# anibali/dsnt-pose2d

Hardware: AMD Instinct MI355X
Metric: images/sec (train step, 256x256, 16 joints) (higher is better)
Workload: dtype f32; 1 GPU; hg2 + DSNT + JS reg, 256x256 -> 64x64x16, batch 32 per GPU, RMSprop lr 2.5e-4, train step fwd+loss+bwd+optim; global_batch=32, parallelism=dp1, launches_fwd=210

## Files before the change

### dsnt-pose2d_amd/csrc/api.cpp

```cpp
#include "common.h"
#include <string.h>

static thread_local char g_err[512] = "";

int dsnt_set_error(int code, const char* fmt, ...) {
    va_list ap;
    va_start(ap, fmt);
    vsnprintf(g_err, sizeof(g_err), fmt, ap);
    va_end(ap);
    return code;
}

int dsnt_device_id(void) {
    int d = 0;
    if (hipGetDevice(&d) != hipSuccess || d < 0) d = 0;
    return d < DSNT_MAX_DEVICES ? d : DSNT_MAX_DEVICES - 1;
}

int dsnt_device_cus(void) {
    static std::atomic<int> cus[DSNT_MAX_DEVICES];
    const int d = dsnt_device_id();
    int c = cus[d].load(std::memory_order_acquire);
    if (!c) {
        hipDeviceProp_t prop;
        int dev = 0;
        c = (hipGetDevice(&dev) == hipSuccess && hipGetDeviceProperties(&prop, dev) == hipSuccess && prop.multiProcessorCount > 0)
                ? prop.multiProcessorCount : 256;
        cus[d].store(c, std::memory_order_release);
    }
    return c;
}

extern "C" int dsnt_version(void) { return 132; }
extern "C" const char* dsnt_last_error(void) { return g_err; }

#include <vector>
#include <new>

struct dsnt_list {
    struct Entry {
        int kind;
        int lane, src, dst;
        mutable hipEvent_t ev;
        std::function<void(hipStream_t)> fn;
    };
    std::vector<Entry> entries;
    std::vector<size_t> seg_start;
    dsnt_list() { seg_start.push_back(0); }
};

static thread_local dsnt_list* g_rec = nullptr;

dsnt_list* dsnt_recording(void) { return g_rec; }

void dsnt_record_launch(dsnt_list* l, int lane, std::function<void(hipStream_t)>&& fn) {
    dsnt_list::Entry e;
    e.kind = 0; e.lane = lane; e.src = e.dst = 0; e.ev = nullptr; e.fn = std::move(fn);
    l->entries.push_back(std::move(e));
}

extern "C" dsnt_list* dsnt_list_create(void) { return new (std::nothrow) dsnt_list(); }

extern "C" void dsnt_list_destroy(dsnt_list* l) {
    if (!l) return;
    if (g_rec == l) g_rec = nullptr;
    for (auto& e : l->entries)
        if (e.ev) (void)hipEventDestroy(e.ev);
    delete l;
}

extern "C" int dsnt_list_begin(dsnt_list* l) {
    DSNT_REQUIRE(l && !g_rec, DSNT_ERR_ARG, "dsnt_list_begin: null list, or this thread is already recording");
    g_rec = l;
    return DSNT_OK;
}

extern "C" int dsnt_list_end(void) {
    DSNT_REQUIRE(g_rec, DSNT_ERR_ARG, "dsnt_list_end: this thread is not recording");
    g_rec = nullptr;
    return DSNT_OK;
}

extern "C" int dsnt_list_sync(dsnt_list* l, int src_lane, int dst_lane) {
    DSNT_REQUIRE(l && src_lane >= 0 && dst_lane >= 0 && src_lane < DSNT_MAX_LANES && dst_lane < DSNT_MAX_LANES, DSNT_ERR_ARG,
                 "dsnt_list_sync: bad argument");
    dsnt_list::Entry e;
    e.kind = 1; e.lane = 0; e.src = src_lane; e.dst = dst_lane; e.ev = nullptr;
    l->entries.push_back(std::move(e));
    return DSNT_OK;
}

extern "C" int dsnt_list_mark(dsnt_list* l) {
    DSNT_REQUIRE(l, DSNT_ERR_ARG, "dsnt_list_mark: null list");
    l->seg_start.push_back(l->entries.size());
    return (int)l->seg_start.size() - 1;
}

extern "C" int dsnt_list_segments(const dsnt_list* l) { return l ? (int)l->seg_start.size() : 0; }
extern "C" int dsnt_list_size(const dsnt_list* l) { return l ? (int)l->entries.size() : 0; }

extern "C" int dsnt_list_replay(const dsnt_list* l, int segment, void* const* streams, int nstreams) {
    DSNT_REQUIRE(l && streams && nstreams > 0 && nstreams <= DSNT_MAX_LANES, DSNT_ERR_ARG, "dsnt_list_replay: bad argument");
    DSNT_REQUIRE(!g_rec, DSNT_ERR_ARG, "dsnt_list_replay: this thread is recording");
    const int nseg = (int)l->seg_start.size();
    DSNT_REQUIRE(segment >= -1 && segment < nseg, DSNT_ERR_ARG, "dsnt_list_replay: segment %d of %d", segment, nseg);
    const size_t a = segment < 0 ? 0 : l->seg_start[segment];
    const size_t b = (segment < 0 || segment + 1 == nseg) ? l->entries.size() : l->seg_start[segment + 1];
    for (size_t i = a; i < b; ++i) {
        const dsnt_list::Entry& e = l->entries[i];
        if (e.kind == 0) {
            DSNT_REQUIRE(e.lane >= 0 && e.lane < nstreams, DSNT_ERR_ARG, "dsnt_list_replay: entry %zu wants lane %d of %d", i, e.lane, nstreams);
            e.fn((hipStream_t)streams[e.lane]);
        } else {
            DSNT_REQUIRE(e.src < nstreams && e.dst < nstreams, DSNT_ERR_ARG, "dsnt_list_replay: lane out of range");
            if (!e.ev && hipEventCreateWithFlags(&e.ev, hipEventDisableTiming) != hipSuccess)
                return dsnt_set_error(DSNT_ERR_HIP, "dsnt_list_replay: hipEventCreate");
            if (hipEventRecord(e.ev, (hipStream_t)streams[e.src]) != hipSuccess ||
                hipStreamWaitEvent((hipStream_t)streams[e.dst], e.ev, 0) != hipSuccess)
                return dsnt_set_error(DSNT_ERR_HIP, "dsnt_list_replay: event record / wait failed");
        }
    }
    hipError_t e_ = hipGetLastError();
    if (e_ != hipSuccess) return dsnt_set_error(DSNT_ERR_HIP, "dsnt_list_replay: %s", hipGetErrorString(e_));
    return DSNT_OK;
}
```

### dsnt-pose2d_amd/csrc/bn.hip

```cpp
#include "common.h"
#include <string.h>
#include "bn_pro.h"
#include "ew_bodies.h"

template <int MODE>
__global__ __launch_bounds__(256) void tile_reduce_kernel(
    const float* __restrict__ a, const float* __restrict__ x, const float* __restrict__ scale,
    const float* __restrict__ shift, const float* __restrict__ mean,
    const float* __restrict__ invstd, int relu, float* __restrict__ partial, long M, int C, int cgs,
    const float* __restrict__ ymask = nullptr, float* __restrict__ dz_out = nullptr) {
    __shared__ float red[256 * 8];
    const int tid = threadIdx.x;
    const int C4 = C >> 2;
    const int rpar = 256 / cgs;
    const int cg_l = tid % cgs, rl = tid / cgs;
    const bool active = rl < rpar;
    const long row0 = (long)blockIdx.x * TILE_ROWS;
    const long row1 = row0 + TILE_ROWS < M ? row0 + TILE_ROWS : M;
    for (int cg0 = blockIdx.y * cgs; cg0 < C4; cg0 += cgs * gridDim.y) {
        const int cg = cg0 + cg_l;
        float4 s1 = make_float4(0.f, 0.f, 0.f, 0.f), s2 = s1;
        if (active && cg < C4) {
            float4 sc, sh, mu, is;
            if (MODE == 1) {
                sc = reinterpret_cast<const float4*>(scale)[cg];
                sh = reinterpret_cast<const float4*>(shift)[cg];
            }
            if (MODE >= 1) {
                mu = reinterpret_cast<const float4*>(mean)[cg];
                is = reinterpret_cast<const float4*>(invstd)[cg];
            }
            for (long r = row0 + rl; r < row1; r += rpar) {
                const float4 v = reinterpret_cast<const float4*>(a + r * C)[cg];
                if (MODE == 0) {
                    s1.x += v.x; s1.y += v.y; s1.z += v.z; s1.w += v.w;
                    s2.x = fmaf(v.x, v.x, s2.x); s2.y = fmaf(v.y, v.y, s2.y);
                    s2.z = fmaf(v.z, v.z, s2.z); s2.w = fmaf(v.w, v.w, s2.w);
                } else {
                    const float4 xv = reinterpret_cast<const float4*>(x + r * C)[cg];
                    float4 dz = v;
                    if (MODE == 2) {
                        if (relu) {
                            const float4 yv = reinterpret_cast<const float4*>(ymask + r * C)[cg];
                            if (yv.x <= 0.f) dz.x = 0.f;
                            if (yv.y <= 0.f) dz.y = 0.f;
                            if (yv.z <= 0.f) dz.z = 0.f;
                            if (yv.w <= 0.f) dz.w = 0.f;
                        }
                        reinterpret_cast<float4*>(dz_out + r * C)[cg] = dz;
                    } else if (relu) {
                        if (fmaf(xv.x, sc.x, sh.x) <= 0.f) dz.x = 0.f;
                        if (fmaf(xv.y, sc.y, sh.y) <= 0.f) dz.y = 0.f;
                        if (fmaf(xv.z, sc.z, sh.z) <= 0.f) dz.z = 0.f;
                        if (fmaf(xv.w, sc.w, sh.w) <= 0.f) dz.w = 0.f;
                    }
                    s1.x += dz.x; s1.y += dz.y; s1.z += dz.z; s1.w += dz.w;
                    s2.x = fmaf(dz.x, (xv.x - mu.x) * is.x, s2.x);
                    s2.y = fmaf(dz.y, (xv.y - mu.y) * is.y, s2.y);
                    s2.z = fmaf(dz.z, (xv.z - mu.z) * is.z, s2.z);
                    s2.w = fmaf(dz.w, (xv.w - mu.w) * is.w, s2.w);
                }
            }
        }
        __syncthreads();
        float* mine = red + tid * 8;
        mine[0] = s1.x; mine[1] = s1.y; mine[2] = s1.z; mine[3] = s1.w;
        mine[4] = s2.x; mine[5] = s2.y; mine[6] = s2.z; mine[7] = s2.w;
        __syncthreads();
        if (tid < cgs && cg0 + tid < C4) {
            float acc[8] = {0, 0, 0, 0, 0, 0, 0, 0};
            for (int j = 0; j < rpar; ++j)
#pragma unroll
                for (int e = 0; e < 8; ++e) acc[e] += red[(j * cgs + tid) * 8 + e];
            float* p0 = partial + ((size_t)blockIdx.x * 2 + 0) * C + (size_t)(cg0 + tid) * 4;
            float* p1 = partial + ((size_t)blockIdx.x * 2 + 1) * C + (size_t)(cg0 + tid) * 4;
            *reinterpret_cast<float4*>(p0) = make_float4(acc[0], acc[1], acc[2], acc[3]);
            *reinterpret_cast<float4*>(p1) = make_float4(acc[4], acc[5], acc[6], acc[7]);
        }
    }
}

extern "C" int dsnt_bn_stats(const float* x, float* partial, int64_t M, int C, void* stream) {
    DSNT_REQUIRE(x && partial && M > 0 && C > 0, DSNT_ERR_ARG, "dsnt_bn_stats: bad argument");
    DSNT_REQUIRE(C % 4 == 0 && dsnt_aligned16(x) && dsnt_aligned16(partial), DSNT_ERR_ALIGN,
                 "dsnt_bn_stats: C %% 4 and 16-byte alignment required");
    const int tiles = (int)((M + TILE_ROWS - 1) / TILE_ROWS);
    DSNT_LAUNCH(tile_reduce_kernel<0>, dim3(tiles, tile_grid_y(tiles, C / 4)), dim3(256), 0, (hipStream_t)stream, x,
                       nullptr, nullptr, nullptr, nullptr, nullptr, 0, partial, (long)M, C, tile_cgs(tiles, C / 4));
    DSNT_CHECK_LAUNCH("dsnt_bn_stats");
}

extern "C" int dsnt_bn_act_fwd_stats(const float* x, const float* scale, const float* shift, int relu, float* y,
                                     float* partial, int64_t M, int C, const dsnt_out_bounds* g_tail, void* stream) {
    OutBoundsP tail;
    if (int e = out_bounds_fill(tail, g_tail, "dsnt_bn_act_fwd_stats")) return e;
    DSNT_REQUIRE(x && scale && shift && y && M > 0 && C > 0, DSNT_ERR_ARG, "dsnt_bn_act_fwd_stats: bad argument");
    DSNT_REQUIRE(C % 4 == 0 && dsnt_aligned16(x) && dsnt_aligned16(y) && dsnt_aligned16(scale) && dsnt_aligned16(shift) &&
                 dsnt_aligned16(partial), DSNT_ERR_ALIGN, "dsnt_bn_act_fwd_stats: alignment");
    const long tiles = ((long)M + TILE_ROWS - 1) / TILE_ROWS;
    DSNT_REQUIRE(M < (1ll << 31), DSNT_ERR_SHAPE, "dsnt_bn_act_fwd_stats: M too large");
    const TileOpP q{x, nullptr, y, nullptr, partial, 1, 1, (int)M, C, tile_cgs(tiles, C / 4), tail, scale, shift, relu};
    DSNT_LAUNCH(tile_op_stats_kernel<2>, dim3((unsigned)tiles, tile_grid_y(tiles, C / 4)), dim3(256), 0, stream, q);
    DSNT_CHECK_LAUNCH("dsnt_bn_act_fwd_stats");
}

extern "C" int dsnt_bn_act_bwd_reduce(const float* da, const float* x, const float* scale,
                                      const float* shift, const float* mean, const float* invstd,
                                      int relu, float* partial, int64_t M, int C, void* stream) {
    DSNT_REQUIRE(da && x && scale && shift && mean && invstd && partial && M > 0 && C > 0,
                 DSNT_ERR_ARG, "dsnt_bn_act_bwd_reduce: bad argument");
    DSNT_REQUIRE(C % 4 == 0 && dsnt_aligned16(x) && dsnt_aligned16(da) && dsnt_aligned16(partial) &&
                 dsnt_aligned16(scale) && dsnt_aligned16(shift) && dsnt_aligned16(mean) &&
                 dsnt_aligned16(invstd), DSNT_ERR_ALIGN,
                 "dsnt_bn_act_bwd_reduce: C %% 4 and 16-byte alignment required");
    const int tiles = (int)((M + TILE_ROWS - 1) / TILE_ROWS);
    DSNT_LAUNCH(tile_reduce_kernel<1>, dim3(tiles, tile_grid_y(tiles, C / 4)), dim3(256), 0, (hipStream_t)stream, da, x,
                       scale, shift, mean, invstd, relu, partial, (long)M, C, tile_cgs(tiles, C / 4));
    DSNT_CHECK_LAUNCH("dsnt_bn_act_bwd_reduce");
}

extern "C" int dsnt_bn_add_act_bwd_reduce(const float* da, const float* y, const float* x, const float* mean, const float* invstd,
                                          int relu, float* dz, float* partial, int64_t M, int C, void* stream) {
    DSNT_REQUIRE(da && y && x && mean && invstd && dz && partial && M > 0 && C > 0, DSNT_ERR_ARG, "dsnt_bn_add_act_bwd_reduce: bad argument");
    DSNT_REQUIRE(C % 4 == 0 && dsnt_aligned16(x) && dsnt_aligned16(da) && dsnt_aligned16(y) && dsnt_aligned16(dz) && dsnt_aligned16(partial) &&
                 dsnt_aligned16(mean) && dsnt_aligned16(invstd), DSNT_ERR_ALIGN, "dsnt_bn_add_act_bwd_reduce: C %% 4 and 16-byte alignment required");
    const int tiles = (int)((M + TILE_ROWS - 1) / TILE_ROWS);
    DSNT_LAUNCH(tile_reduce_kernel<2>, dim3(tiles, tile_grid_y(tiles, C / 4)), dim3(256), 0, (hipStream_t)stream, da, x,
                       nullptr, nullptr, mean, invstd, relu, partial, (long)M, C, tile_cgs(tiles, C / 4), y, dz);
    DSNT_CHECK_LAUNCH("dsnt_bn_add_act_bwd_reduce");
}

#define FIN_T 1024
#define FIN_P (FIN_T / 16)
struct BnBoundP { const float* scale; const float* dz_amax; float sqrtM; unsigned* out; };
struct BnFinP {
    const float* partial; int ntiles; double invM, unbias; int C;
    const float* gamma; const float* beta; float* running_mean; float* running_var;
    float momentum, eps; int training; float* o0; float* o1; float* o2; float* o3; int accumulate; BnBoundP bp;
};
template <int MODE>
__global__ __launch_bounds__(FIN_T) void bn_finalize_kernel(BnFinP q) {
    __shared__ double r0[256], r1[256];
    const float* __restrict__ partial = q.partial; const int ntiles = q.ntiles; const double invM = q.invM, unbias = q.unbias;
    const int C = q.C; const float* __restrict__ gamma = q.gamma; const float* __restrict__ beta = q.beta;
    float* running_mean = q.running_mean; float* running_var = q.running_var; const float momentum = q.momentum, eps = q.eps;
    const int training = q.training; float* o0 = q.o0; float* o1 = q.o1; float* o2 = q.o2; float* o3 = q.o3;
    const int accumulate = q.accumulate; const BnBoundP bp = q.bp;
    const int tid = threadIdx.x, cl = tid & 15;
    const int wg = blockIdx.x;
    const int c = wg * 16 + cl;
    const bool lead = tid < 16 && c < C;
    float pg = 1.f, pb = 0.f, prm = 0.f, prv = 0.f, po0 = 0.f, po1 = 0.f, psc = 0.f, pdz = 0.f;
    if (MODE == 0 && lead) {
        if (gamma) pg = gamma[c];
        if (beta) pb = beta[c];
        if (running_mean) { prm = running_mean[c]; prv = running_var[c]; }
    }
    if (MODE == 1) {
        if (lead && accumulate) { if (o0) po0 = o0[c]; if (o1) po1 = o1[c]; }
        if (bp.out) { pdz = bp.dz_amax[tid & 63]; if (lead) psc = bp.scale[c]; }
    }
    constexpr int VP = 1;
    double a0[VP], a1[VP];
#pragma unroll
    for (int v = 0; v < VP; ++v) {
        a0[v] = 0.0; a1[v] = 0.0;
        const int part = (tid + v * FIN_T) >> 4;
        if (c < C && (MODE == 1 || training)) {
#pragma unroll 4
            for (int t = part; t < ntiles; t += FIN_P) {
                a0[v] += (double)partial[((size_t)t * 2 + 0) * C + c];
                a1[v] += (double)partial[((size_t)t * 2 + 1) * C + c];
            }
        }
    }
#pragma unroll
    for (int v = 0; v < VP; ++v) {
        a0[v] += __shfl_xor(a0[v], 16, 64); a1[v] += __shfl_xor(a1[v], 16, 64);
        a0[v] += __shfl_xor(a0[v], 32, 64); a1[v] += __shfl_xor(a1[v], 32, 64);
        if ((tid & 63) < 16) { r0[((tid + v * FIN_T) >> 6) * 16 + cl] = a0[v]; r1[((tid + v * FIN_T) >> 6) * 16 + cl] = a1[v]; }
    }
    __syncthreads();
    double s0 = 0.0, s1 = 0.0;
    if (tid < 16) {
#pragma unroll
        for (int w = 0; w < FIN_T / 64; ++w) { s0 += r0[w * 16 + cl]; s1 += r1[w * 16 + cl]; }
    }
    if (tid < 16 && c < C) {
        if (MODE == 0) {
            double mean, var;
            if (training) {
                mean = s0 * invM;
                var = s1 * invM - mean * mean;
                if (var < 0.0) var = 0.0;
                if (running_mean) {
                    running_mean[c] = (float)((1.0 - momentum) * prm + momentum * mean);
                    running_var[c] = (float)((1.0 - momentum) * prv + momentum * var * unbias);
                }
            } else {
                mean = prm;
                var = prv;
            }
            const float is = (float)(1.0 / sqrt(var + (double)eps));
            const float mu = (float)mean;
            const float sc = gamma ? pg * is : is;
            o0[c] = mu; o1[c] = is; o2[c] = sc;
            o3[c] = (beta ? pb : 0.f) - mu * sc;
        } else {
            const float sdz = (float)s0, sdzx = (float)s1;
            if (o0) o0[c] = accumulate ? po0 + sdzx : sdzx;
            if (o1) o1[c] = accumulate ? po1 + sdz : sdz;
            o2[c] = (float)(s0 * invM);
            o2[C + c] = (float)(s1 * invM);
        }
    }
    if (MODE == 1 && bp.out) {
        float dzmax = pdz;
#pragma unroll
        for (int o = 32; o > 0; o >>= 1) dzmax = fmaxf(dzmax, __shfl_xor(dzmax, o, 64));
        float b = 0.f;
        if (tid < 16 && c < C)
            b = fabsf(psc) * (dzmax + fabsf((float)(s0 * invM)) + fabsf((float)(s1 * invM)) * bp.sqrtM);
#pragma unroll
        for (int o = 8; o > 0; o >>= 1) b = fmaxf(b, __shfl_xor(b, o, 64));
        if (tid == 0 && b > 0.f) atomicMax(bp.out + (wg & 63), __float_as_uint(b));
    }
}

extern "C" int dsnt_bn_finalize(const float* partial, int ntiles, int64_t M, int C,
                                const float* gamma, const float* beta, float* running_mean,
                                float* running_var, float momentum, float eps, int training,
                                float* mean, float* invstd, float* scale, float* shift,
                                void* stream) {
    DSNT_REQUIRE(mean && invstd && scale && shift && C > 0 && M > 0, DSNT_ERR_ARG,
                 "dsnt_bn_finalize: bad argument");
    DSNT_REQUIRE(training ? (partial != nullptr && ntiles > 0) : (running_mean && running_var),
                 DSNT_ERR_ARG, "dsnt_bn_finalize: missing statistics source");
    DSNT_REQUIRE((running_mean == nullptr) == (running_var == nullptr), DSNT_ERR_ARG,
                 "dsnt_bn_finalize: running_mean/var must be given together");
    const double unbias = M > 1 ? (double)M / (double)(M - 1) : 1.0;
    const BnFinP q{partial, ntiles, 1.0 / (double)M, unbias, C, gamma, beta, running_mean, running_var, momentum, eps, training,
                   mean, invstd, scale, shift, 0, BnBoundP{nullptr, nullptr, 0.f, nullptr}};
    DSNT_LAUNCH(bn_finalize_kernel<0>, dim3((C + 15) / 16), dim3(FIN_T), 0, stream, q);
    DSNT_CHECK_LAUNCH("dsnt_bn_finalize");
}

__global__ __launch_bounds__(256) void bn_eval_prep_kernel(const long long* __restrict__ table) {
    const long long* t = table + (size_t)blockIdx.x * 10;
    const float* gamma = reinterpret_cast<const float*>(t[0]);
    const float* beta = reinterpret_cast<const float*>(t[1]);
    const float* rm = reinterpret_cast<const float*>(t[2]);
    const float* rv = reinterpret_cast<const float*>(t[3]);
    float* mean = reinterpret_cast<float*>(t[4]);
    float* invstd = reinterpret_cast<float*>(t[5]);
    float* scale = reinterpret_cast<float*>(t[6]);
    float* shift = reinterpret_cast<float*>(t[7]);
    const int C = (int)t[8];
    const float eps = __uint_as_float((unsigned)t[9]);
    for (int c = threadIdx.x; c < C; c += 256) {
        const double var = rv[c];
        const float is = (float)(1.0 / sqrt(var + (double)eps));
        const float mu = rm[c];
        const float sc = gamma ? gamma[c] * is : is;
        mean[c] = mu; invstd[c] = is; scale[c] = sc;
        shift[c] = (beta ? beta[c] : 0.f) - mu * sc;
    }
}

extern "C" int dsnt_bn_eval_prep(const int64_t* table, int rows, void* stream) {
    DSNT_REQUIRE(table && rows > 0, DSNT_ERR_ARG, "dsnt_bn_eval_prep: bad argument");
    DSNT_LAUNCH(bn_eval_prep_kernel, dim3(rows), dim3(256), 0, (hipStream_t)stream, (const long long*)table);
    DSNT_CHECK_LAUNCH("dsnt_bn_eval_prep");
}

extern "C" int dsnt_bn_bwd_finalize(const float* partial, int ntiles, int64_t M, int C,
                                    float* dgamma, float* dbeta, int accumulate, float* coef,
                                    void* stream) {
    DSNT_REQUIRE(partial && coef && ntiles > 0 && C > 0 && M > 0, DSNT_ERR_ARG,
                 "dsnt_bn_bwd_finalize: bad argument");
    const double invM = (accumulate & DSNT_BN_FROZEN) ? 0.0 : 1.0 / (double)M;
    const BnFinP q{partial, ntiles, invM, 1.0, C, nullptr, nullptr, nullptr, nullptr, 0.f, 0.f, 1, dgamma, dbeta, coef, nullptr,
                   accumulate & 1, BnBoundP{nullptr, nullptr, 0.f, nullptr}};
    DSNT_LAUNCH(bn_finalize_kernel<1>, dim3((C + 15) / 16), dim3(FIN_T), 0, stream, q);
    DSNT_CHECK_LAUNCH("dsnt_bn_bwd_finalize");
}

extern "C" int dsnt_bn_bwd_finalize_bound(const float* partial, int ntiles, int64_t M, int C, float* dgamma, float* dbeta,
                                          int accumulate, float* coef, const float* scale, const float* dz_amax,
                                          float* bound_out, void* stream) {
    DSNT_REQUIRE(partial && coef && scale && dz_amax && bound_out && ntiles > 0 && C > 0 && M > 0, DSNT_ERR_ARG,
                 "dsnt_bn_bwd_finalize_bound: bad argument");
    DSNT_REQUIRE(!(accumulate & DSNT_BN_FROZEN), DSNT_ERR_ARG, "dsnt_bn_bwd_finalize_bound: DSNT_BN_FROZEN has no bound form");
    const BnFinP q{partial, ntiles, 1.0 / (double)M, 1.0, C, nullptr, nullptr, nullptr, nullptr, 0.f, 0.f, 1, dgamma, dbeta, coef, nullptr,
                   accumulate & 1, BnBoundP{scale, dz_amax, sqrtf((float)M), reinterpret_cast<unsigned*>(bound_out)}};
    DSNT_LAUNCH(bn_finalize_kernel<1>, dim3((C + 15) / 16), dim3(FIN_T), 0, stream, q);
    DSNT_CHECK_LAUNCH("dsnt_bn_bwd_finalize_bound");
}

__global__ void bn_act_fwd_kernel(const float4* __restrict__ x, const float4* __restrict__ scale,
                                  const float4* __restrict__ shift, int relu, float4* __restrict__ y,
                                  long n4, int C4) {
    for (long i = (long)blockIdx.x * blockDim.x + threadIdx.x; i < n4;
         i += (long)gridDim.x * blockDim.x) {
        const int cg = (int)(i % C4);
        const float4 v = x[i], sc = scale[cg], sh = shift[cg];
        float4 o = make_float4(fmaf(v.x, sc.x, sh.x), fmaf(v.y, sc.y, sh.y), fmaf(v.z, sc.z, sh.z),
                               fmaf(v.w, sc.w, sh.w));
        if (relu) { o.x = fmaxf(o.x, 0.f); o.y = fmaxf(o.y, 0.f); o.z = fmaxf(o.z, 0.f); o.w = fmaxf(o.w, 0.f); }
        y[i] = o;
    }
}

extern "C" int dsnt_bn_act_fwd(const float* x, const float* scale, const float* shift, int relu,
                               float* y, int64_t M, int C, void* stream) {
    DSNT_REQUIRE(x && scale && shift && y && M > 0 && C > 0, DSNT_ERR_ARG, "dsnt_bn_act_fwd: bad argument");
    DSNT_REQUIRE(C % 4 == 0 && dsnt_aligned16(x) && dsnt_aligned16(y) && dsnt_aligned16(scale) &&
                 dsnt_aligned16(shift), DSNT_ERR_ALIGN, "dsnt_bn_act_fwd: alignment");
    const long n4 = (long)M * C / 4;
    DSNT_LAUNCH(bn_act_fwd_kernel, dim3(flat_grid(n4, 256)), dim3(256), 0, (hipStream_t)stream,
                       (const float4*)x, (const float4*)scale, (const float4*)shift, relu, (float4*)y,
                       n4, C / 4);
    DSNT_CHECK_LAUNCH("dsnt_bn_act_fwd");
}

__global__ void bn_add_act_fwd_kernel(const float4* __restrict__ x, const float4* __restrict__ scale,
                                      const float4* __restrict__ shift, const float4* __restrict__ res, int relu,
                                      float4* __restrict__ y, long n4, int C4) {
    for (long i = (long)blockIdx.x * blockDim.x + threadIdx.x; i < n4; i += (long)gridDim.x * blockDim.x) {
        const int cg = (int)(i % C4);
        const float4 v = x[i], sc = scale[cg], sh = shift[cg], r = res[i];
        float4 o = make_float4(fmaf(v.x, sc.x, sh.x) + r.x, fmaf(v.y, sc.y, sh.y) + r.y, fmaf(v.z, sc.z, sh.z) + r.z,
                               fmaf(v.w, sc.w, sh.w) + r.w);
        if (relu) { o.x = fmaxf(o.x, 0.f); o.y = fmaxf(o.y, 0.f); o.z = fmaxf(o.z, 0.f); o.w = fmaxf(o.w, 0.f); }
        y[i] = o;
    }
}

extern "C" int dsnt_bn_add_act_fwd(const float* x, const float* scale, const float* shift, const float* res,
                                   int relu, float* y, int64_t M, int C, void* stream) {
    DSNT_REQUIRE(x && scale && shift && res && y && M > 0 && C > 0, DSNT_ERR_ARG, "dsnt_bn_add_act_fwd: bad argument");
    DSNT_REQUIRE(C % 4 == 0 && dsnt_aligned16(x) && dsnt_aligned16(y) && dsnt_aligned16(res) && dsnt_aligned16(scale) &&
                 dsnt_aligned16(shift), DSNT_ERR_ALIGN, "dsnt_bn_add_act_fwd: alignment");
    const long n4 = (long)M * C / 4;
    DSNT_LAUNCH(bn_add_act_fwd_kernel, dim3(flat_grid(n4, 256)), dim3(256), 0, (hipStream_t)stream,
                       (const float4*)x, (const float4*)scale, (const float4*)shift, (const float4*)res, relu,
                       (float4*)y, n4, C / 4);
    DSNT_CHECK_LAUNCH("dsnt_bn_add_act_fwd");
}

__global__ void relu_bwd_kernel(const float4* __restrict__ dy, const float4* __restrict__ y, float4* __restrict__ dz,
                                long n4) {
    for (long i = (long)blockIdx.x * blockDim.x + threadIdx.x; i < n4; i += (long)gridDim.x * blockDim.x) {
        const float4 g = dy[i], v = y[i];
        dz[i] = make_float4(v.x > 0.f ? g.x : 0.f, v.y > 0.f ? g.y : 0.f, v.z > 0.f ? g.z : 0.f, v.w > 0.f ? g.w : 0.f);
    }
}

extern "C" int dsnt_relu_bwd(const float* dy, const float* y, float* dz, int64_t n, void* stream) {
    DSNT_REQUIRE(dy && y && dz && n > 0 && n % 4 == 0, DSNT_ERR_ARG, "dsnt_relu_bwd: bad argument");
    DSNT_REQUIRE(dsnt_aligned16(dy) && dsnt_aligned16(y) && dsnt_aligned16(dz), DSNT_ERR_ALIGN, "dsnt_relu_bwd: alignment");
    DSNT_LAUNCH(relu_bwd_kernel, dim3(flat_grid(n / 4, 256)), dim3(256), 0, (hipStream_t)stream,
                       (const float4*)dy, (const float4*)y, (float4*)dz, (long)(n / 4));
    DSNT_CHECK_LAUNCH("dsnt_relu_bwd");
}

struct BnApplyVec { float4 sc, sh, mu, is, c0, c1; };
__device__ __forceinline__ float4 bn_apply_one(const float4 g, const float4 xv, const BnApplyVec& v, int relu) {
    float4 dz = g;
    if (relu) {
        if (fmaf(xv.x, v.sc.x, v.sh.x) <= 0.f) dz.x = 0.f;
        if (fmaf(xv.y, v.sc.y, v.sh.y) <= 0.f) dz.y = 0.f;
        if (fmaf(xv.z, v.sc.z, v.sh.z) <= 0.f) dz.z = 0.f;
        if (fmaf(xv.w, v.sc.w, v.sh.w) <= 0.f) dz.w = 0.f;
    }
    float4 o;
    o.x = v.sc.x * (dz.x - v.c0.x - (xv.x - v.mu.x) * v.is.x * v.c1.x);
    o.y = v.sc.y * (dz.y - v.c0.y - (xv.y - v.mu.y) * v.is.y * v.c1.y);
    o.z = v.sc.z * (dz.z - v.c0.z - (xv.z - v.mu.z) * v.is.z * v.c1.z);
    o.w = v.sc.w * (dz.w - v.c0.w - (xv.w - v.mu.w) * v.is.w * v.c1.w);
    return o;
}
struct BnApplyP {
    const float4* da; const float4* x; const float4* scale; const float4* shift; const float4* mean; const float4* invstd;
    const float4* coef; int relu; float4* dx; const float4* base; long n4; int C4; unsigned* amax; BnBwdProP pro;
};
template <bool FIXED>
__global__ void bn_act_bwd_apply_kernel(BnApplyP q) {
    __shared__ double pro_sh[512];
    const float4* __restrict__ da = q.da; const float4* __restrict__ x = q.x; const float4* __restrict__ scale = q.scale;
    const float4* __restrict__ shift = q.shift; const float4* __restrict__ mean = q.mean; const float4* __restrict__ invstd = q.invstd;
    const float4* coef = q.coef; const int relu = q.relu; float4* dx = q.dx; const float4* base = q.base;
    const long n4 = q.n4; const int C4 = q.C4; unsigned* __restrict__ amax = q.amax; const BnBwdProP pro = q.pro;
    const bool accumulate = base != nullptr;
    const int wg = blockIdx.x, nwg = gridDim.x;
    if (pro.partial) {
        bn_pro_backward<256>(pro, pro_sh, wg == 0);
        __syncthreads();
    }
    float am = 0.f;
    const long stride = (long)nwg * 256;
    long i = threadIdx.x < 256 ? (long)wg * 256 + threadIdx.x : n4;
    auto vec = [&](int cg) {
        BnApplyVec v;
        v.sc = scale[cg]; v.sh = shift[cg]; v.mu = mean[cg]; v.is = invstd[cg]; v.c0 = coef[cg]; v.c1 = coef[C4 + cg];
        return v;
    };
    auto amx = [&](const float4 o) { am = fmaxf(fmaxf(fmaxf(fabsf(o.x), fabsf(o.y)), fmaxf(fabsf(o.z), fabsf(o.w))), am); };
    if (FIXED) {
        const BnApplyVec v = vec((int)((i < n4 ? i : 0) % C4));
        for (; i + stride < n4; i += 2 * stride) {
            const float4 g0 = da[i], x0 = x[i], g1 = da[i + stride], x1 = x[i + stride];
            float4 p0 = make_float4(0.f, 0.f, 0.f, 0.f), p1 = p0;
            if (accumulate) { p0 = base[i]; p1 = base[i + stride]; }
            float4 o0 = bn_apply_one(g0, x0, v, relu), o1 = bn_apply_one(g1, x1, v, relu);
            if (accumulate) {
                o0.x += p0.x; o0.y += p0.y; o0.z += p0.z; o0.w += p0.w;
                o1.x += p1.x; o1.y += p1.y; o1.z += p1.z; o1.w += p1.w;
            }
            dx[i] = o0; dx[i + stride] = o1;
            amx(o0); amx(o1);
        }
        if (i < n4) {
            float4 o = bn_apply_one(da[i], x[i], v, relu);
            if (accumulate) { const float4 p = base[i]; o.x += p.x; o.y += p.y; o.z += p.z; o.w += p.w; }
            dx[i] = o;
            amx(o);
        }
    } else {
        for (; i < n4; i += stride) {
            float4 o = bn_apply_one(da[i], x[i], vec((int)(i % C4)), relu);
            if (accumulate) { const float4 p = base[i]; o.x += p.x; o.y += p.y; o.z += p.z; o.w += p.w; }
            dx[i] = o;
            amx(o);
        }
    }
    if (amax) amax_commit(am, amax);
}

static int bn_act_bwd_apply_impl(const float* da, const float* x, const float* scale, const float* shift,
                                 const float* mean, const float* invstd, const float* coef, int relu, float* dx,
                                 int accumulate, int64_t M, int C, float* amax, void* stream, const BnBwdProP* pro, const float* base) {
    DSNT_REQUIRE(da && x && scale && shift && mean && invstd && coef && dx && M > 0 && C > 0,
                 DSNT_ERR_ARG, "dsnt_bn_act_bwd_apply: bad argument");
    DSNT_REQUIRE(C % 4 == 0 && dsnt_aligned16(da) && dsnt_aligned16(x) && dsnt_aligned16(dx) &&
                 dsnt_aligned16(coef) && dsnt_aligned16(base), DSNT_ERR_ALIGN, "dsnt_bn_act_bwd_apply: alignment");
    if (!base && accumulate) base = dx;
    const long n4 = (long)M * C / 4;
    int grid = flat_grid(n4, 256);
    BnBwdProP q;
    memset(&q, 0, sizeof(q));
    if (pro) {
        q = *pro;
        if (grid > 128) grid = 128;
    }
    const BnApplyP ap{(const float4*)da, (const float4*)x, (const float4*)scale, (const float4*)shift, (const float4*)mean,
                      (const float4*)invstd, (const float4*)coef, relu, (float4*)dx, (const float4*)base, n4, C / 4, (unsigned*)amax, q};
    if (((long)grid * 256) % (C / 4) == 0)
        DSNT_LAUNCH(bn_act_bwd_apply_kernel<true>, dim3(grid), dim3(256), 0, stream, ap);
    else
        DSNT_LAUNCH(bn_act_bwd_apply_kernel<false>, dim3(grid), dim3(256), 0, stream, ap);
    DSNT_CHECK_LAUNCH("dsnt_bn_act_bwd_apply");
}

extern "C" int dsnt_bn_act_bwd_apply_amax(const float* da, const float* x, const float* scale,
                                          const float* shift, const float* mean, const float* invstd,
                                          const float* coef, int relu, float* dx, int accumulate,
                                          int64_t M, int C, float* amax, void* stream) {
    return bn_act_bwd_apply_impl(da, x, scale, shift, mean, invstd, coef, relu, dx, accumulate, M, C, amax, stream, nullptr, nullptr);
}

extern "C" int dsnt_bn_act_bwd_apply(const float* da, const float* x, const float* scale,
                                     const float* shift, const float* mean, const float* invstd,
                                     const float* coef, int relu, float* dx, int accumulate,
                                     int64_t M, int C, void* stream) {
    return bn_act_bwd_apply_impl(da, x, scale, shift, mean, invstd, coef, relu, dx, accumulate, M, C, nullptr, stream, nullptr, nullptr);
}

static int bn_bwd_pro_fill(BnBwdProP& q, const char* who, const float* partial, int ntiles, float* dgamma, float* dbeta,
                           int accumulate_params, float* coef, int64_t M, int C) {
    DSNT_REQUIRE(partial && ntiles > 0 && coef && C <= 256 && (long)ntiles * C <= 16384, DSNT_ERR_ARG,
                 "%s: needs partial sums of at most 256 channels / 128 KB and a coef buffer", who);
    q.partial = partial; q.tiles = ntiles; q.C = C; q.invM = 1.0 / (double)M;
    q.dgamma = dgamma; q.dbeta = dbeta; q.accumulate = accumulate_params; q.coef = coef;
    return DSNT_OK;
}

extern "C" int dsnt_bn_act_bwd_apply_pro(const float* da, const float* x, const float* scale, const float* shift,
                                         const float* mean, const float* invstd, const float* partial, int ntiles,
                                         float* dgamma, float* dbeta, int accumulate_params, float* coef, int relu,
                                         float* dx, int accumulate, int64_t M, int C, float* amax, void* stream) {
    BnBwdProP q;
    if (int e = bn_bwd_pro_fill(q, "dsnt_bn_act_bwd_apply_pro", partial, ntiles, dgamma, dbeta, accumulate_params, coef, M, C)) return e;
    return bn_act_bwd_apply_impl(da, x, scale, shift, mean, invstd, coef, relu, dx, accumulate, M, C, amax, stream, &q, nullptr);
}
extern "C" int dsnt_bn_act_bwd_apply_base(const float* da, const float* x, const float* scale, const float* shift,
                                          const float* mean, const float* invstd, const float* coef, int relu,
                                          const float* base, float* dx, int64_t M, int C, float* amax, void* stream) {
    DSNT_REQUIRE(base && base != dx, DSNT_ERR_ARG, "dsnt_bn_act_bwd_apply_base: `base` must be a second tensor");
    return bn_act_bwd_apply_impl(da, x, scale, shift, mean, invstd, coef, relu, dx, 1, M, C, amax, stream, nullptr, base);
}
extern "C" int dsnt_bn_act_bwd_apply_pro_base(const float* da, const float* x, const float* scale, const float* shift,
                                              const float* mean, const float* invstd, const float* partial, int ntiles,
                                              float* dgamma, float* dbeta, int accumulate_params, float* coef, int relu,
                                              const float* base, float* dx, int64_t M, int C, float* amax, void* stream) {
    DSNT_REQUIRE(base && base != dx, DSNT_ERR_ARG, "dsnt_bn_act_bwd_apply_pro_base: `base` must be a second tensor");
    BnBwdProP q;
    if (int e = bn_bwd_pro_fill(q, "dsnt_bn_act_bwd_apply_pro_base", partial, ntiles, dgamma, dbeta, accumulate_params, coef, M, C)) return e;
    return bn_act_bwd_apply_impl(da, x, scale, shift, mean, invstd, coef, relu, dx, 1, M, C, amax, stream, &q, base);
}
```

### dsnt-pose2d_amd/csrc/bn_pro.h

```cpp
#pragma once
#include "common.h"

struct OutBoundsP {
    unsigned* amax;
    unsigned* amax_bn;
    const float* amax_scale;
    const float* amax_shift;
    int amax_relu, pad_;
};

__device__ __forceinline__ void tail_store(float* p, float v) { *p = v; }

struct BnProP {
    const float* partial; int tiles, C;
    double invM, unbias;
    const float* gamma; const float* beta; float* rmean; float* rvar;
    float momentum, eps;
    float* mean; float* invstd; float* scale; float* shift;
};
struct BnBwdProP {
    const float* partial; int tiles, C;
    double invM;
    float* dgamma; float* dbeta; int accumulate;
    float* coef;
};

template <int NT>
__device__ __forceinline__ void bn_pro_sums(const float* __restrict__ partial, int tiles, int C, double* sh, double& a0, double& a1) {
    const int tid = threadIdx.x;
    const int ncol = 2 * C;
    a0 = 0.0; a1 = 0.0;
    for (int cb = 0; cb < ncol; cb += NT) {
        const int nc = ncol - cb < NT ? ncol - cb : NT;
        const int L = NT / nc;
        const int col = tid % nc, lane = tid / nc;
        double a = 0.0;
        if (lane < L) {
            const float* q = partial + cb + col;
            for (int r0 = lane; r0 < tiles; r0 += 16 * L) {
                float v[16];
#pragma unroll
                for (int u = 0; u < 16; ++u) {
                    const int r = r0 + u * L;
                    v[u] = r < tiles ? q[(size_t)r * ncol] : 0.f;
                }
#pragma unroll
                for (int u = 0; u < 16; ++u) a += (double)v[u];
            }
        }
        __syncthreads();
        sh[tid] = a;
        __syncthreads();
        for (int st = 0; st < 2; ++st) {
            const int c = st * C + tid - cb;
            if (tid < C && c >= 0 && c < nc) {
                double t = 0.0;
                for (int l = 0; l < L; ++l) t += sh[l * nc + c];
                if (st == 0) a0 = t; else a1 = t;
            }
        }
    }
}

template <int NT>
__device__ __forceinline__ void bn_pro_forward(const BnProP& q, double* sh, bool writer) {
    const int c = threadIdx.x;
    float pg = 1.f, pb = 0.f, prm = 0.f, prv = 0.f;
    if (c < q.C) {
        if (q.gamma) pg = q.gamma[c];
        if (q.beta) pb = q.beta[c];
        if (writer && q.rmean) { prm = q.rmean[c]; prv = q.rvar[c]; }
    }
    double a0, a1;
    bn_pro_sums<NT>(q.partial, q.tiles, q.C, sh, a0, a1);
    if (c < q.C) {
        const double mean = a0 * q.invM;
        double var = a1 * q.invM - mean * mean;
        if (var < 0.0) var = 0.0;
        if (writer && q.rmean) {
            q.rmean[c] = (float)((1.0 - q.momentum) * prm + q.momentum * mean);
            q.rvar[c] = (float)((1.0 - q.momentum) * prv + q.momentum * var * q.unbias);
        }
        const float is = (float)(1.0 / sqrt(var + (double)q.eps));
        const float mu = (float)mean;
        const float sc = q.gamma ? pg * is : is;
        q.mean[c] = mu; q.invstd[c] = is; q.scale[c] = sc;
        q.shift[c] = (q.beta ? pb : 0.f) - mu * sc;
    }
    __builtin_amdgcn_fence(__ATOMIC_RELEASE, "workgroup");
}
template <int NT>
__device__ __forceinline__ void bn_pro_backward(const BnBwdProP& q, double* sh, bool writer) {
    const int c = threadIdx.x;
    float pdg = 0.f, pdb = 0.f;
    if (c < q.C && writer && q.accumulate) { if (q.dgamma) pdg = q.dgamma[c]; if (q.dbeta) pdb = q.dbeta[c]; }
    double a0, a1;
    bn_pro_sums<NT>(q.partial, q.tiles, q.C, sh, a0, a1);
    if (c < q.C) {
        if (writer) {
            const float sdz = (float)a0, sdzx = (float)a1;
            if (q.dgamma) q.dgamma[c] = q.accumulate ? pdg + sdzx : sdzx;
            if (q.dbeta) q.dbeta[c] = q.accumulate ? pdb + sdz : sdz;
        }
        q.coef[c] = (float)(a0 * q.invM);
        q.coef[q.C + c] = (float)(a1 * q.invM);
    }
    __builtin_amdgcn_fence(__ATOMIC_RELEASE, "workgroup");
}

static inline int out_bounds_fill(OutBoundsP& out, const dsnt_out_bounds* in, const char* who) {
    static_assert(sizeof(OutBoundsP) == sizeof(dsnt_out_bounds), "dsnt_out_bounds layout");
    out.amax = in ? reinterpret_cast<unsigned*>(in->amax) : nullptr;
    out.amax_bn = in ? reinterpret_cast<unsigned*>(in->amax_bn) : nullptr;
    out.amax_scale = in ? in->amax_scale : nullptr; out.amax_shift = in ? in->amax_shift : nullptr;
    out.amax_relu = in ? in->amax_relu : 0; out.pad_ = 0;
    DSNT_REQUIRE(!out.amax_bn || (out.amax_scale && out.amax_shift && dsnt_aligned16(out.amax_scale) && dsnt_aligned16(out.amax_shift)),
                 DSNT_ERR_ARG, "%s: dsnt_out_bounds.amax_bn needs 16-byte aligned amax_scale / amax_shift", who);
    return DSNT_OK;
}
```

### dsnt-pose2d_amd/csrc/conv_f32.hip

```cpp
#include "conv_epilogue.h"
#include <string.h>
#include <stdlib.h>

#define BK 32
#define PITCH 36

template <int WM, int WN, int TM, int TN, bool PRO, bool FAST>
__global__ __launch_bounds__(512, 4) void conv_fwd_kernel(ConvP p) {
    constexpr int BM = WM * TM * 32, BN = WN * TN * 32;
    constexpr int APASS = BM / 32, BPASS = BN / 32;
    extern __shared__ __attribute__((aligned(16))) float smem[];
    float* As = smem;
    float* Bs = smem + 2 * BM * PITCH;

    int tile;
    xcd_remap(blockIdx.x, p.mtiles * p.ntiles, tile);
    const int ntile = tile % p.ntiles, mtile = tile / p.ntiles;

    const int tid = threadIdx.x, lane = tid & 63;
    const int wave = __builtin_amdgcn_readfirstlane(tid >> 6);
    const int nsteps = (p.K + BK - 1) / BK;
    const int lr = lane & 31, lh = lane >> 5;
    const int cw = wave & 3;
    const int wm = cw / WN, wn = cw % WN;
    if (PRO && p.pro.partial) {
        bn_pro_forward<512>(p.pro, reinterpret_cast<double*>(smem), blockIdx.x == 0);
        __syncthreads();
    }

    f32x16 acc[TM][TN];
#pragma unroll
    for (int a = 0; a < TM; ++a)
#pragma unroll
        for (int b = 0; b < TN; ++b)
#pragma unroll
            for (int e = 0; e < 16; ++e) acc[a][b][e] = 0.f;

    if (FAST && wave >= 4) {
        typedef unsigned u32x4 __attribute__((ext_vector_type(4)));
        const int ltid = tid - 256;
        const int lrow = ltid >> 3, kc = ltid & 7;
        const int HoWo = p.Ho * p.Wo;
        const int RS = p.R * p.S;
        unsigned apix[APASS];
        unsigned long long vmask = 0ull;
#pragma unroll
        for (int i = 0; i < APASS; ++i) {
            const int m = mtile * BM + lrow + 32 * i;
            const bool vm = m < p.M;
            const int mm = vm ? m : 0;
            const int n = mm / HoWo, rem = mm - n * HoWo;
            const int oh = rem / p.Wo, ow = rem - oh * p.Wo;
            const int ih0 = oh * p.stride - p.pad, iw0 = ow * p.stride - p.pad;
            apix[i] = (unsigned)(((n * p.H + ih0) * p.W + iw0) * p.Cin + kc * 4) * 4u;
            for (int t = 0; t < RS; ++t) {
                const int r = t / p.S, s_ = t - r * p.S;
                const int ih = ih0 + r * p.dil, iw = iw0 + s_ * p.dil;
                if (vm && ih >= 0 && ih < p.H && iw >= 0 && iw < p.W)
                    vmask |= 1ull << (t * APASS + i);
            }
        }
        unsigned bpix[BPASS];
#pragma unroll
        for (int j = 0; j < BPASS; ++j) {
            const int n = ntile * BN + lrow + 32 * j;
            bpix[j] = n < p.Cout ? (unsigned)(n * p.K + kc * 4) * 4u : 0xF0000000u;
        }
        const __amdgpu_buffer_rsrc_t xr = __builtin_amdgcn_make_buffer_rsrc(
            const_cast<float*>(p.x), 0, (int)((size_t)p.N * p.H * p.W * p.Cin * 4u), 0x00020000);
        const __amdgpu_buffer_rsrc_t wr = __builtin_amdgcn_make_buffer_rsrc(
            const_cast<float*>(p.w), 0, (int)((size_t)p.Cout * p.K * 4u), 0x00020000);
        struct Stage {
            u32x4 ra[APASS], rb[BPASS];
            float4 sc, sh;
            unsigned ok;
        };
        Stage S0, S1;
        auto gload = [&](Stage& st, int step) {
            const int kb = step * BK;
            const int tap = kb / p.Cin, cb = kb - tap * p.Cin;
            const int r = tap / p.S, s_ = tap - r * p.S;
            const unsigned toff = (unsigned)(((r * p.dil) * p.W + s_ * p.dil) * p.Cin + cb) * 4u;
            if (PRO) {
                st.sc = *reinterpret_cast<const float4*>(p.in_scale + cb + kc * 4);
                st.sh = *reinterpret_cast<const float4*>(p.in_shift + cb + kc * 4);
            }
            st.ok = (unsigned)(vmask >> (tap * APASS));
#pragma unroll
            for (int i = 0; i < APASS; ++i)
                st.ra[i] = __builtin_amdgcn_raw_buffer_load_b128(xr, apix[i] + toff, 0, 0);
            const unsigned koff = (unsigned)kb * 4u;
#pragma unroll
            for (int j = 0; j < BPASS; ++j)
                st.rb[j] = __builtin_amdgcn_raw_buffer_load_b128(wr, bpix[j] + koff, 0, 0);
        };
        auto lstore = [&](const Stage& st, int buf) {
#pragma unroll
            for (int i = 0; i < APASS; ++i) {
                float4 v = make_float4(__uint_as_float(st.ra[i].x), __uint_as_float(st.ra[i].y),
                                       __uint_as_float(st.ra[i].z), __uint_as_float(st.ra[i].w));
                float* dst = As + (buf * BM + lrow + 32 * i) * PITCH + kc * 4;
                if (PRO) {
                    v.x = fmaf(v.x, st.sc.x, st.sh.x); v.y = fmaf(v.y, st.sc.y, st.sh.y);
                    v.z = fmaf(v.z, st.sc.z, st.sh.z); v.w = fmaf(v.w, st.sc.w, st.sh.w);
                    if (p.in_relu) {
                        v.x = fmaxf(v.x, 0.f); v.y = fmaxf(v.y, 0.f);
                        v.z = fmaxf(v.z, 0.f); v.w = fmaxf(v.w, 0.f);
                    }
                }
                const bool ok = (st.ok >> i) & 1u;
                v.x = ok ? v.x : 0.f; v.y = ok ? v.y : 0.f; v.z = ok ? v.z : 0.f; v.w = ok ? v.w : 0.f;
                *reinterpret_cast<float4*>(dst) = v;
            }
#pragma unroll
            for (int j = 0; j < BPASS; ++j)
                *reinterpret_cast<u32x4*>(Bs + (buf * BN + lrow + 32 * j) * PITCH + kc * 4) = st.rb[j];
        };
        const int last = nsteps - 1;
        gload(S0, 0);
        gload(S1, min(1, last));
        lstore(S0, 0);
        gload(S0, min(2, last));
        __syncthreads();
        int s = 0;
        for (; s + 1 < nsteps; s += 2) {
            lstore(S1, 1);
            gload(S1, min(s + 3, last));
            __syncthreads();
            lstore(S0, 0);
            gload(S0, min(s + 4, last));
            __syncthreads();
        }
        if (s < nsteps) __syncthreads();
    } else if (wave >= 4) {
        const int ltid = tid - 256;
        const int lrow = ltid >> 3, kc = ltid & 7;
        int abase[APASS], aih0[APASS], aiw0[APASS];
        const int HoWo = p.Ho * p.Wo;
#pragma unroll
        for (int i = 0; i < APASS; ++i) {
            const int m = mtile * BM + lrow + 32 * i;
            if (m < p.M) {
                const int n = m / HoWo, rem = m - n * HoWo;
                const int oh = rem / p.Wo, ow = rem - oh * p.Wo;
                abase[i] = n * p.H * p.W * p.Cin;
                aih0[i] = oh * p.stride - p.pad;
                aiw0[i] = ow * p.stride - p.pad;
            } else {
                abase[i] = 0; aih0[i] = -(1 << 28); aiw0[i] = 0;
            }
        }
        int boff[BPASS];
        bool bok[BPASS];
#pragma unroll
        for (int j = 0; j < BPASS; ++j) {
            const int n = ntile * BN + lrow + 32 * j;
            bok[j] = n < p.Cout;
            boff[j] = bok[j] ? n * p.K : 0;
        }
        struct Stage {
            float4 ra[APASS], rb[BPASS];
            float4 sc, sh;
            unsigned okmask;
        };
        Stage S0, S1;
        auto gload = [&](Stage& st, int step) {
            const int k0 = step * BK + kc * 4;
            const bool vk = k0 < p.K;
            const int tap = k0 / p.Cin, c = k0 - tap * p.Cin;
            const int r = tap / p.S, s = tap - r * p.S;
            const int dh = r * p.dil, dw = s * p.dil;
            if (PRO) {
                const int cc = vk ? c : 0;
                st.sc = *reinterpret_cast<const float4*>(p.in_scale + cc);
                st.sh = *reinterpret_cast<const float4*>(p.in_shift + cc);
            }
            st.okmask = 0;
#pragma unroll
            for (int i = 0; i < APASS; ++i) {
                const int ih = aih0[i] + dh, iw = aiw0[i] + dw;
                const bool ok = vk && ih >= 0 && ih < p.H && iw >= 0 && iw < p.W;
                const int off = ok ? abase[i] + (ih * p.W + iw) * p.Cin + c : 0;
                st.ra[i] = *reinterpret_cast<const float4*>(p.x + off);
                st.okmask |= (ok ? 1u : 0u) << i;
            }
#pragma unroll
            for (int j = 0; j < BPASS; ++j) {
                const bool ok = vk && bok[j];
                st.rb[j] = *reinterpret_cast<const float4*>(p.w + (ok ? boff[j] + k0 : 0));
                st.okmask |= (ok ? 1u : 0u) << (8 + j);
            }
        };
        auto lstore = [&](const Stage& st, int buf) {
#pragma unroll
            for (int i = 0; i < APASS; ++i) {
                float4 v = st.ra[i];
                if (PRO) {
                    v.x = fmaf(v.x, st.sc.x, st.sh.x); v.y = fmaf(v.y, st.sc.y, st.sh.y);
                    v.z = fmaf(v.z, st.sc.z, st.sh.z); v.w = fmaf(v.w, st.sc.w, st.sh.w);
                    if (p.in_relu) {
                        v.x = fmaxf(v.x, 0.f); v.y = fmaxf(v.y, 0.f);
                        v.z = fmaxf(v.z, 0.f); v.w = fmaxf(v.w, 0.f);
                    }
                }
                if (!((st.okmask >> i) & 1u)) v = make_float4(0.f, 0.f, 0.f, 0.f);
                *reinterpret_cast<float4*>(As + (buf * BM + lrow + 32 * i) * PITCH + kc * 4) = v;
            }
#pragma unroll
            for (int j = 0; j < BPASS; ++j) {
                float4 v = st.rb[j];
                if (!((st.okmask >> (8 + j)) & 1u)) v = make_float4(0.f, 0.f, 0.f, 0.f);
                *reinterpret_cast<float4*>(Bs + (buf * BN + lrow + 32 * j) * PITCH + kc * 4) = v;
            }
        };
        const int last = nsteps - 1;
        gload(S0, 0);
        gload(S1, min(1, last));
        lstore(S0, 0);
        gload(S0, min(2, last));
        __syncthreads();
        int s = 0;
        for (; s + 1 < nsteps; s += 2) {
            lstore(S1, 1);
            gload(S1, min(s + 3, last));
            __syncthreads();
            lstore(S0, 0);
            gload(S0, min(s + 4, last));
            __syncthreads();
        }
        if (s < nsteps) __syncthreads();
    } else {
        __builtin_amdgcn_s_setprio(1);
        struct Frag { float4 a[TM], b[TN]; };
        Frag F0, F1;
        auto rd = [&](Frag& f, int buf, int ks) {
            const float* Ab = As + (buf * BM + (wm * TM) * 32 + lr) * PITCH + 4 * lh + ks * 8;
            const float* Bb = Bs + (buf * BN + (wn * TN) * 32 + lr) * PITCH + 4 * lh + ks * 8;
#pragma unroll
            for (int a = 0; a < TM; ++a) f.a[a] = *reinterpret_cast<const float4*>(Ab + a * 32 * PITCH);
#pragma unroll
            for (int b = 0; b < TN; ++b) f.b[b] = *reinterpret_cast<const float4*>(Bb + b * 32 * PITCH);
        };
        auto mm = [&](const Frag& f) {
#pragma unroll
            for (int a = 0; a < TM; ++a)
#pragma unroll
                for (int b = 0; b < TN; ++b) {
                    acc[a][b] = __builtin_amdgcn_mfma_f32_32x32x2f32(f.a[a].x, f.b[b].x, acc[a][b], 0, 0, 0);
                    acc[a][b] = __builtin_amdgcn_mfma_f32_32x32x2f32(f.a[a].y, f.b[b].y, acc[a][b], 0, 0, 0);
                    acc[a][b] = __builtin_amdgcn_mfma_f32_32x32x2f32(f.a[a].z, f.b[b].z, acc[a][b], 0, 0, 0);
                    acc[a][b] = __builtin_amdgcn_mfma_f32_32x32x2f32(f.a[a].w, f.b[b].w, acc[a][b], 0, 0, 0);
                }
        };
        __syncthreads();
        rd(F0, 0, 0);
        for (int s = 0; s < nsteps; ++s) {
            const int buf = s & 1;
            rd(F1, buf, 1);
            __builtin_amdgcn_sched_barrier(0);
            mm(F0);
            __builtin_amdgcn_sched_barrier(0);
            rd(F0, buf, 2);
            __builtin_amdgcn_sched_barrier(0);
            mm(F1);
            __builtin_amdgcn_sched_barrier(0);
            rd(F1, buf, 3);
            __builtin_amdgcn_sched_barrier(0);
            mm(F0);
            __builtin_amdgcn_sched_barrier(0);
            __syncthreads();
            if (s + 1 < nsteps) rd(F0, buf ^ 1, 0);
            __builtin_amdgcn_sched_barrier(0);
            mm(F1);
            __builtin_amdgcn_sched_barrier(0);
        }
        __builtin_amdgcn_s_setprio(0);
    }

    conv_epilogue<WM, WN, TM, TN>(p, acc, smem, mtile, ntile, tid, wave, lane);
}

static void pick_cfg(const dsnt_conv_geom* g, int& BM, int& BN) {
    const long M = (long)g->N * g->Ho * g->Wo;
    if (g->Cout <= 32) { BM = 128; BN = 32; }
    else if (g->Cout <= 64) { BM = 128; BN = 64; }
    else { BM = 128; BN = 128; }
    const long tiles = ((M + BM - 1) / BM) * ((g->Cout + BN - 1) / BN);
    if (tiles < 256 && g->Cout >= 128) { BM = 32; BN = 128; }
}

extern "C" int dsnt_conv_fwd_bm(const dsnt_conv_geom* g) {
    int BM, BN;
    pick_cfg(g, BM, BN);
    return BM;
}

template <int WM, int WN, int TM, int TN>
static int launch_fwd(const ConvP& p, bool pro, hipStream_t st) {
    constexpr int BM = WM * TM * 32, BN = WN * TN * 32;
    const size_t lds = (size_t)2 * (BM + BN) * PITCH * sizeof(float);
    const int grid = p.mtiles * p.ntiles;
    if (lds > 65536) {
        DSNT_SET_MAX_LDS((conv_fwd_kernel<WM, WN, TM, TN, true, true>), lds);
        DSNT_SET_MAX_LDS((conv_fwd_kernel<WM, WN, TM, TN, false, true>), lds);
        DSNT_SET_MAX_LDS((conv_fwd_kernel<WM, WN, TM, TN, true, false>), lds);
        DSNT_SET_MAX_LDS((conv_fwd_kernel<WM, WN, TM, TN, false, false>), lds);
    }
    const bool fast = (p.Cin % BK == 0) && (p.R * p.S * (BM / 32) <= 64) &&
                      ((size_t)p.N * p.H * p.W * p.Cin * 4u < (1ull << 31)) &&
                      ((size_t)p.Cout * p.K * 4u < (1ull << 31));
    dim3 gr(grid), bl(512);
    if (pro && fast) DSNT_LAUNCH((conv_fwd_kernel<WM, WN, TM, TN, true, true>), gr, bl, lds, st, p);
    else if (pro) DSNT_LAUNCH((conv_fwd_kernel<WM, WN, TM, TN, true, false>), gr, bl, lds, st, p);
    else if (fast) DSNT_LAUNCH((conv_fwd_kernel<WM, WN, TM, TN, false, true>), gr, bl, lds, st, p);
    else DSNT_LAUNCH((conv_fwd_kernel<WM, WN, TM, TN, false, false>), gr, bl, lds, st, p);
    return 0;
}

int conv_check_geom(const dsnt_conv_geom* g, const char* who) {
    DSNT_REQUIRE(g != nullptr, DSNT_ERR_ARG, "%s: null geometry", who);
    DSNT_REQUIRE(g->N > 0 && g->H > 0 && g->W > 0 && g->Cin > 0 && g->Cout > 0 && g->R > 0 &&
                 g->S > 0 && g->stride > 0 && g->dil > 0 && g->pad >= 0, DSNT_ERR_SHAPE,
                 "%s: non-positive dimension", who);
    DSNT_REQUIRE(g->Cin % 4 == 0, DSNT_ERR_ALIGN, "%s: Cin=%d must be a multiple of 4", who, g->Cin);
    DSNT_REQUIRE(g->Cout % 4 == 0, DSNT_ERR_ALIGN, "%s: Cout=%d must be a multiple of 4", who, g->Cout);
    const int ho = (g->H + 2 * g->pad - g->dil * (g->R - 1) - 1) / g->stride + 1;
    const int wo = (g->W + 2 * g->pad - g->dil * (g->S - 1) - 1) / g->stride + 1;
    DSNT_REQUIRE(ho == g->Ho && wo == g->Wo, DSNT_ERR_SHAPE,
                 "%s: output %dx%d inconsistent with input/filter (expected %dx%d)", who, g->Ho,
                 g->Wo, ho, wo);
    DSNT_REQUIRE((long)g->N * g->H * g->W * g->Cin < (1L << 31) &&
                 (long)g->N * g->Ho * g->Wo * g->Cout < (1L << 31), DSNT_ERR_SHAPE,
                 "%s: tensor exceeds 2^31 elements", who);
    return DSNT_OK;
}

template <bool PRO, int CW>
__device__ __forceinline__ void conv_ksplit_body(const ConvP& p, float (*part)[32][33]) {
    typedef unsigned u32x4 __attribute__((ext_vector_type(4)));
    constexpr int NL = CW / 8;
    const int nt32 = (p.Cout + 31) >> 5;
    const int tile = blockIdx.x;
    const int ntile = tile % nt32, mtile = tile / nt32;
    const int tid = threadIdx.x, lane = tid & 63;
    const int wave = __builtin_amdgcn_readfirstlane(tid >> 6);
    const int i = lane & 31, h = lane >> 5;
    const unsigned OOB = 0xF0000000u;
    if (PRO && p.pro.partial) {
        bn_pro_forward<512>(p.pro, reinterpret_cast<double*>(&part[0][0][0]), tile == 0);
        __syncthreads();
    }
    float* const ssc = &part[0][0][0];
    if (PRO) {
        for (int c = tid; c < p.Cin; c += 512) { ssc[c] = p.in_scale[c]; ssc[p.Cin + c] = p.in_shift[c]; }
        __syncthreads();
    }
    const int m = mtile * 32 + i;
    const bool vm = m < p.M;
    const int HoWo = p.Ho * p.Wo;
    const int mm = vm ? m : 0;
    const int img = mm / HoWo, rem = mm - img * HoWo;
    const int oh = rem / p.Wo, ow = rem - oh * p.Wo;
    const int ih0 = oh * p.stride - p.pad, iw0 = ow * p.stride - p.pad;
    const int nb = ntile * 32 + i;
    const int kl = (CW / 2) * h;
    const unsigned boff = nb < p.Cout ? (unsigned)((size_t)nb * p.K + kl) * 4u : OOB;
    const __amdgpu_buffer_rsrc_t xr = __builtin_amdgcn_make_buffer_rsrc(
        const_cast<float*>(p.x), 0, (int)((size_t)p.N * p.H * p.W * p.Cin * 4u), 0x00020000);
    const __amdgpu_buffer_rsrc_t wr = __builtin_amdgcn_make_buffer_rsrc(
        const_cast<float*>(p.w), 0, (int)((size_t)p.Cout * p.K * 4u), 0x00020000);
    const int nch = p.K / CW;
    const int c0 = wave * nch / 8, c1 = (wave + 1) * nch / 8;
    const float lo_valid = p.in_relu ? 0.f : -__builtin_inff();
    struct Frag { u32x4 a[NL], b[NL]; bool ok; int cb; };
    int pos = c0, pr, ps, pcb;
    {
        const int kb = c0 * CW, tap = kb / p.Cin;
        pcb = kb - tap * p.Cin; pr = tap / p.S; ps = tap - pr * p.S;
    }
    auto load_next = [&]() {
        Frag f;
        const int ih = ih0 + pr * p.dil, iw = iw0 + ps * p.dil;
        f.ok = vm && (unsigned)ih < (unsigned)p.H && (unsigned)iw < (unsigned)p.W;
        f.cb = pcb;
        const unsigned aoff = f.ok ? (unsigned)(((img * p.H + ih) * p.W + iw) * p.Cin + pcb + kl) * 4u : OOB;
        const int kb4 = ((pr * p.S + ps) * p.Cin + pcb) * 4;
#pragma unroll
        for (int q = 0; q < NL; ++q) f.a[q] = __builtin_amdgcn_raw_buffer_load_b128(xr, aoff + 16u * q, 0, 0);
#pragma unroll
        for (int q = 0; q < NL; ++q) f.b[q] = __builtin_amdgcn_raw_buffer_load_b128(wr, boff + 16u * q, kb4, 0);
        if (pos < c1 - 1) {
            ++pos;
            pcb += CW;
            if (pcb == p.Cin) { pcb = 0; if (++ps == p.S) { ps = 0; ++pr; } }
        }
        return f;
    };
    f32x16 acc;
#pragma unroll
    for (int e = 0; e < 16; ++e) acc[e] = 0.f;
    auto mma = [&](const Frag& f) {
        const float lo = f.ok ? lo_valid : 0.f, hi = f.ok ? __builtin_inff() : 0.f;
#pragma unroll
        for (int q = 0; q < NL; ++q) {
            float4 a = make_float4(__uint_as_float(f.a[q].x), __uint_as_float(f.a[q].y), __uint_as_float(f.a[q].z),
                                   __uint_as_float(f.a[q].w));
            if (PRO) {
                const float4 sc = *reinterpret_cast<const float4*>(ssc + f.cb + kl + 4 * q);
                const float4 sh = *reinterpret_cast<const float4*>(ssc + p.Cin + f.cb + kl + 4 * q);
                a.x = __builtin_amdgcn_fmed3f(fmaf(a.x, sc.x, sh.x), lo, hi);
                a.y = __builtin_amdgcn_fmed3f(fmaf(a.y, sc.y, sh.y), lo, hi);
                a.z = __builtin_amdgcn_fmed3f(fmaf(a.z, sc.z, sh.z), lo, hi);
                a.w = __builtin_amdgcn_fmed3f(fmaf(a.w, sc.w, sh.w), lo, hi);
            }
            acc = __builtin_amdgcn_mfma_f32_32x32x2f32(a.x, __uint_as_float(f.b[q].x), acc, 0, 0, 0);
            acc = __builtin_amdgcn_mfma_f32_32x32x2f32(a.y, __uint_as_float(f.b[q].y), acc, 0, 0, 0);
            acc = __builtin_amdgcn_mfma_f32_32x32x2f32(a.z, __uint_as_float(f.b[q].z), acc, 0, 0, 0);
            acc = __builtin_amdgcn_mfma_f32_32x32x2f32(a.w, __uint_as_float(f.b[q].w), acc, 0, 0, 0);
        }
    };
    const int col = tid & 31, rg = tid >> 5;
    const int n = ntile * 32 + col;
    const bool vn = n < p.Cout;
    const bool bnb = p.bnb_scale != nullptr;
    float bias = 0.f, bsc = 0.f, bsh = 0.f, bmu = 0.f, bis = 0.f;
    if (!PRO) {
        bias = (p.bias && vn) ? p.bias[n] : 0.f;
        if (bnb && vn) { bsc = p.bnb_scale[n]; bsh = p.bnb_shift[n]; bmu = p.bnb_mean[n]; bis = p.bnb_invstd[n]; }
    }
    float r1v[2] = {0.f, 0.f};
    if (!PRO) {
#pragma unroll
        for (int j = 0; j < 2; ++j) {
            const int mo = mtile * 32 + rg + 16 * j;
            if (vn && mo < p.M && p.res1) r1v[j] = p.res1[(size_t)mo * p.Cout + n];
        }
    }
    if (c0 < c1) {
        Frag f0 = load_next(), f1 = load_next(), f2;
        for (int ch = c0;;) {
            f2 = load_next(); mma(f0); if (++ch >= c1) break;
            f0 = load_next(); mma(f1); if (++ch >= c1) break;
            f1 = load_next(); mma(f2); if (++ch >= c1) break;
        }
    }
    if (PRO) __syncthreads();
#pragma unroll
    for (int e = 0; e < 16; ++e) part[wave][(e & 3) + 8 * (e >> 2) + 4 * h][i] = acc[e];
    __syncthreads();
    if (PRO) {
        bias = (p.bias && vn) ? p.bias[n] : 0.f;
        if (bnb && vn) { bsc = p.bnb_scale[n]; bsh = p.bnb_shift[n]; bmu = p.bnb_mean[n]; bis = p.bnb_invstd[n]; }
    }
    float s1 = 0.f, s2 = 0.f;
#pragma unroll
    for (int j = 0; j < 2; ++j) {
        const int row = rg + 16 * j;
        const int mo = mtile * 32 + row;
        float v = 0.f;
#pragma unroll
        for (int w = 0; w < 8; ++w) v += part[w][row][col];
        if (vn && mo < p.M) {
            const size_t o = (size_t)mo * p.Cout + n;
            if (bnb) {
                const float xv = PRO ? p.res1[o] : r1v[j];
                if (p.bnb_relu && fmaf(xv, bsc, bsh) <= 0.f) v = 0.f;
                p.y[o] = v;
                s1 += v;
                s2 = fmaf(v, (xv - bmu) * bis, s2);
            } else {
                v += bias + (PRO ? (p.res1 ? p.res1[o] : 0.f) : r1v[j]) + (p.res2 ? p.res2[o] : 0.f);
                p.y[o] = v;
                s1 += v;
                s2 = fmaf(v, v, s2);
            }
        }
    }
    if (p.stats) {
        __syncthreads();
        float* red = &part[0][0][0];
        red[(rg * 32 + col) * 2 + 0] = s1;
        red[(rg * 32 + col) * 2 + 1] = s2;
        __syncthreads();
        if (tid < 32 && vn) {
            float a0 = 0.f, a1 = 0.f;
#pragma unroll
            for (int w = 0; w < 16; ++w) { a0 += red[(w * 32 + tid) * 2 + 0]; a1 += red[(w * 32 + tid) * 2 + 1]; }
            tail_store(p.stats + ((size_t)mtile * 2 + 0) * p.Cout + n, a0);
            tail_store(p.stats + ((size_t)mtile * 2 + 1) * p.Cout + n, a1);
        }
    }
}

template <bool PRO, int CW>
__global__ __launch_bounds__(512) void conv_ksplit_kernel(ConvP p) {
    __shared__ __attribute__((aligned(16))) float part[8][32][33];
    conv_ksplit_body<PRO, CW>(p, part);
}

static long ksplit_rows() {
    static long v = -1;
    if (v < 0) {
        const char* e = getenv("DSNT_X_KSPLIT_ROWS");
        v = e ? atol(e) : 2048;
    }
    return v;
}

static bool conv_fwd_pro_ok(const dsnt_conv_geom* g, int tiles, int C) {
    return g && C == g->Cin && C <= 256 && C % 4 == 0 && tiles > 0 && (long)tiles * C <= 16384;
}
extern "C" int dsnt_conv_fwd_pro_ok(const dsnt_conv_geom* g, int tiles, int C) { return conv_fwd_pro_ok(g, tiles, C) ? 1 : 0; }

int conv_fill(ConvP& p, const char* who, const float* x, const void* w, bool planes, int64_t plane_stride, const float* bias,
              float* y, const float* in_scale, const float* in_shift, int in_relu, const float* res1, const float* res2,
              float* stats_partial, const dsnt_conv_geom* g, const dsnt_bn_bwd_epilogue* bnb, const dsnt_out_bounds* tail) {
    if (int e = conv_check_geom(g, who)) return e;
    char who_ex[64];
    snprintf(who_ex, sizeof(who_ex), "%s_ex", who);
    DSNT_REQUIRE(!bnb || (bnb->x && bnb->scale && bnb->shift && bnb->mean && bnb->invstd &&
                          stats_partial && !res1 && !res2 && !bias), DSNT_ERR_ARG,
                 "%s: the batch-norm-backward epilogue needs x/scale/shift/mean/invstd and "
                 "stats_partial, and excludes bias/residuals", who_ex);
    DSNT_REQUIRE(x && w && y, DSNT_ERR_ARG, "%s: null tensor", who);
    DSNT_REQUIRE((in_scale == nullptr) == (in_shift == nullptr), DSNT_ERR_ARG,
                 "%s: in_scale/in_shift must be given together", who);
    DSNT_REQUIRE(!planes || dsnt_conv_bf16x6_ok(g), DSNT_ERR_SHAPE,
                 "%s: geometry not supported (need Cin %% 16 == 0, <= 16 taps, < 2 GiB)", who);
    DSNT_REQUIRE(dsnt_aligned16(x) && dsnt_aligned16(w) && (!in_scale || dsnt_aligned16(in_scale)) &&
                 (!in_shift || dsnt_aligned16(in_shift)), DSNT_ERR_ALIGN,
                 "%s: x/w/scale/shift must be 16-byte aligned", who);
    DSNT_REQUIRE(!planes || (plane_stride >= (int64_t)g->Cout * g->R * g->S * g->Cin && plane_stride % 8 == 0 &&
                             (2 * plane_stride + (int64_t)g->Cout * g->R * g->S * g->Cin) * 2 < (1LL << 31)), DSNT_ERR_SHAPE,
                 "%s: bad plane stride %lld", who, (long long)plane_stride);
    p.x = x; p.bias = bias; p.y = y; p.in_scale = in_scale; p.in_shift = in_shift;
    p.w = planes ? nullptr : (const float*)w;
    p.wq = planes ? (const unsigned short*)w : nullptr; p.wq_stride = planes ? plane_stride : 0;
    p.res1 = res1; p.res2 = res2; p.stats = stats_partial; p.in_relu = in_relu;
    p.bnb_scale = p.bnb_shift = p.bnb_mean = p.bnb_invstd = nullptr; p.bnb_relu = 0;
    p.a_bound = p.w_bound = nullptr;
    p.ap_y = p.ap_scale = p.ap_mean = p.ap_invstd = p.ap_coef = nullptr; p.ap_out = nullptr;
    if (bnb) {
        p.res1 = bnb->x; p.bnb_scale = bnb->scale; p.bnb_shift = bnb->shift;
        p.bnb_mean = bnb->mean; p.bnb_invstd = bnb->invstd; p.bnb_relu = bnb->relu;
    }
    if (int e = out_bounds_fill(p.tail, tail, who_ex)) return e;
    DSNT_REQUIRE(!(p.tail.amax_bn && bnb), DSNT_ERR_ARG, "%s: dsnt_out_bounds.amax_bn excludes the batch-norm-backward epilogue", who_ex);
    memset(&p.pro, 0, sizeof(p.pro));
    conv_geom_fill(p, g);
    return DSNT_OK;
}

static int conv_fwd_impl(const float* x, const float* w, const float* bias, float* y,
                         const float* in_scale, const float* in_shift, int in_relu,
                         const float* res1, const float* res2, float* stats_partial,
                         const dsnt_conv_geom* g, const dsnt_bn_bwd_epilogue* g_bnb, const dsnt_out_bounds* g_tail,
                         void* stream, const dsnt_bn_prologue* g_pro = nullptr) {
    ConvP p;
    if (int e = conv_fill(p, "dsnt_conv_fwd", x, w, false, 0, bias, y, in_scale, in_shift, in_relu, res1, res2, stats_partial, g,
                          g_bnb, g_tail)) return e;
    if (g_pro) {
        DSNT_REQUIRE(g_pro->partial && g_pro->mean && g_pro->invstd && g_pro->scale && g_pro->shift && g_pro->M > 0 &&
                     conv_fwd_pro_ok(g, g_pro->tiles, g_pro->C), DSNT_ERR_ARG,
                     "dsnt_conv_fwd_pro: incomplete dsnt_bn_prologue, or more than 256 channels / 128 KB of partial sums");
        DSNT_REQUIRE((g_pro->running_mean == nullptr) == (g_pro->running_var == nullptr), DSNT_ERR_ARG,
                     "dsnt_conv_fwd_pro: running_mean/var must be given together");
        DSNT_REQUIRE(dsnt_aligned16(g_pro->scale) && dsnt_aligned16(g_pro->shift), DSNT_ERR_ALIGN, "dsnt_conv_fwd_pro: alignment");
        p.pro.partial = g_pro->partial; p.pro.tiles = g_pro->tiles; p.pro.C = g_pro->C;
        p.pro.invM = 1.0 / (double)g_pro->M;
        p.pro.unbias = g_pro->M > 1 ? (double)g_pro->M / (double)(g_pro->M - 1) : 1.0;
        p.pro.gamma = g_pro->gamma; p.pro.beta = g_pro->beta; p.pro.rmean = g_pro->running_mean; p.pro.rvar = g_pro->running_var;
        p.pro.momentum = g_pro->momentum; p.pro.eps = g_pro->eps;
        p.pro.mean = g_pro->mean; p.pro.invstd = g_pro->invstd; p.pro.scale = g_pro->scale; p.pro.shift = g_pro->shift;
    }
    int BM, BN;
    pick_cfg(g, BM, BN);
    p.mtiles = (p.M + BM - 1) / BM; p.ntiles = (p.Cout + BN - 1) / BN;
    hipStream_t st = (hipStream_t)stream;
    const bool pro = in_scale != nullptr;
    if (BM == 32 && p.M <= ksplit_rows() && p.Cin % 8 == 0 && (size_t)p.N * p.H * p.W * p.Cin * 4u < (1ull << 31) &&
        (size_t)p.Cout * p.K * 4u < (1ull << 31) && !p.tail.amax && !p.tail.amax_bn &&
        (!pro || p.Cin <= 4096)) {
        const int grid = p.mtiles * ((p.Cout + 31) / 32);
#ifndef KS_CW
#define KS_CW 16
#endif
        if (p.Cin % KS_CW == 0) {
            if (pro) DSNT_LAUNCH((conv_ksplit_kernel<true, KS_CW>), dim3(grid), dim3(512), 0, st, p);
            else DSNT_LAUNCH((conv_ksplit_kernel<false, KS_CW>), dim3(grid), dim3(512), 0, st, p);
        } else if (pro) DSNT_LAUNCH((conv_ksplit_kernel<true, 8>), dim3(grid), dim3(512), 0, st, p);
        else DSNT_LAUNCH((conv_ksplit_kernel<false, 8>), dim3(grid), dim3(512), 0, st, p);
    } else if (BM == 128 && BN == 128) launch_fwd<2, 2, 2, 2>(p, pro, st);
    else if (BM == 128 && BN == 64) launch_fwd<2, 2, 2, 1>(p, pro, st);
    else if (BM == 128 && BN == 32) launch_fwd<4, 1, 1, 1>(p, pro, st);
    else launch_fwd<1, 4, 1, 1>(p, pro, st);
    DSNT_CHECK_LAUNCH("dsnt_conv_fwd");
}

extern "C" int dsnt_conv_fwd(const float* x, const float* w, const float* bias, float* y,
                             const float* in_scale, const float* in_shift, int in_relu,
                             const float* res1, const float* res2, float* stats_partial,
                             const dsnt_conv_geom* g, void* stream) {
    return conv_fwd_impl(x, w, bias, y, in_scale, in_shift, in_relu, res1, res2, stats_partial, g, nullptr, nullptr, stream);
}

extern "C" int dsnt_conv_fwd_ex(const float* x, const float* w, const float* bias, float* y,
                                const float* in_scale, const float* in_shift, int in_relu,
                                const float* res1, const float* res2, float* stats_partial,
                                const dsnt_conv_geom* g, const dsnt_bn_bwd_epilogue* bnb, const dsnt_out_bounds* tail,
                                void* stream) {
    return conv_fwd_impl(x, w, bias, y, in_scale, in_shift, in_relu, res1, res2, stats_partial, g, bnb, tail, stream);
}

extern "C" int dsnt_conv_fwd_pro(const float* x, const float* w, const float* bias, float* y, const dsnt_bn_prologue* pro,
                                 int in_relu, const float* res1, const float* res2, float* stats_partial,
                                 const dsnt_conv_geom* g, const dsnt_out_bounds* tail, void* stream) {
    DSNT_REQUIRE(pro, DSNT_ERR_ARG, "dsnt_conv_fwd_pro: null dsnt_bn_prologue");
    return conv_fwd_impl(x, w, bias, y, pro->scale, pro->shift, in_relu, res1, res2, stats_partial, g, nullptr, tail, stream, pro);
}
```

### dsnt-pose2d_amd/dsnt/_lib.py

```python
import ctypes as C
import os

import torch

_HERE = os.path.dirname(os.path.abspath(__file__))
LIB_PATH = os.environ.get('DSNT_HIP_LIB') or os.path.join(os.path.dirname(_HERE), 'csrc', 'libdsnt_hip.so')

P = C.c_void_p
I = C.c_int
L = C.c_int64
F = C.c_float
D = C.c_double


class ConvGeom(C.Structure):
    _fields_ = [(n, C.c_int) for n in
                ('N', 'H', 'W', 'Cin', 'Ho', 'Wo', 'Cout', 'R', 'S', 'stride', 'pad', 'dil')]


GP = C.POINTER(ConvGeom)


class BnBwdEpilogue(C.Structure):
    _fields_ = [('x', C.c_void_p), ('scale', C.c_void_p), ('shift', C.c_void_p), ('mean', C.c_void_p),
                ('invstd', C.c_void_p), ('relu', C.c_int)]


BP = C.POINTER(BnBwdEpilogue)


class BnPrologue(C.Structure):
    _fields_ = [('partial', C.c_void_p), ('tiles', C.c_int), ('C', C.c_int), ('M', C.c_int64),
                ('gamma', C.c_void_p), ('beta', C.c_void_p), ('running_mean', C.c_void_p), ('running_var', C.c_void_p),
                ('momentum', C.c_float), ('eps', C.c_float),
                ('mean', C.c_void_p), ('invstd', C.c_void_p), ('scale', C.c_void_p), ('shift', C.c_void_p)]


PP = C.POINTER(BnPrologue)


class BnTail(C.Structure):
    _fields_ = [('amax', C.c_void_p), ('amax_bn', C.c_void_p), ('amax_scale', C.c_void_p), ('amax_shift', C.c_void_p),
                ('amax_relu', C.c_int), ('reserved', C.c_int)]


TP = C.POINTER(BnTail)


class BnBwdApply(C.Structure):
    _fields_ = [('y', C.c_void_p), ('scale', C.c_void_p), ('mean', C.c_void_p), ('invstd', C.c_void_p),
                ('coef', C.c_void_p)]


AP = C.POINTER(BnBwdApply)

SIGNATURES = {
    'dsnt_preact_fwd': [P, P, L, I, I, F, F, P],
    'dsnt_preact_bwd': [P, P, P, P, L, I, I, F, F, P],
    'dsnt_expect_fwd': [P, P, L, I, I, P],
    'dsnt_expect_bwd': [P, P, L, I, I, P],
    'dsnt_make_gauss': [P, P, L, I, I, F, P],
    'dsnt_make_gauss_bwd': [P, P, P, L, I, I, F, P],
    'dsnt_encode_heatmaps': [P, P, L, I, I, F, P],
    'dsnt_heatmap_mse_fwd': [P, P, P, L, I, I, F, P],
    'dsnt_heatmap_mse_bwd': [P, P, P, P, L, I, I, F, P],
    'dsnt_decode_heatmaps': [P, P, L, I, I, I, P],
    'dsnt_fc2_fwd': [P, P, P, P, L, I, P],
    'dsnt_fc2_bwd': [P, P, P, P, P, P, L, I, P],
    'dsnt_reg_fwd': [P, P, P, L, I, I, F, I, P],
    'dsnt_reg_bwd': [P, P, P, P, L, I, I, F, I, P],
    'dsnt_reg_bwd_mu': [P, P, P, P, L, I, I, F, I, P],
    'dsnt_euclid_fwd': [P, P, P, L, I, P],
    'dsnt_euclid_bwd': [P, P, P, P, P, L, I, P],
    'dsnt_masked_avg_fwd': [P, P, P, L, P],
    'dsnt_masked_avg_bwd': [P, P, P, P, L, P],
    'dsnt_head_fwd': [P, P, P, L, I, I, P],
    'dsnt_flip_merge_head': [P, L, I, I, I, P, I, I, F, F, P, P, P, P, P, P],
    'dsnt_flip_merge_head_stats': [P, L, I, I, I, P, I, I, F, F, P, P, P, P, P, P, P, P, P],
    'dsnt_heatmap_stats': [P, L, I, I, P, P, P],
    'dsnt_head_loss_rows': [P, P, P, P, P, L, I, I, F, I, P],
    'dsnt_head_bwd': [P, P, P, P, P, P, P, L, I, I, F, I, P],
    'dsnt_head_loss_grad': [P, P, P, P, P, P, P, P, L, I, I, F, I, F, P],
    'dsnt_mask_denom': [P, P, L, P],
    'dsnt_head_loss_reduce': [P, P, P, P, F, P, P, L, P],
    'dsnt_scale_by_scalar': [P, P, L, P],
    'dsnt_conv_fwd': [P, P, P, P, P, P, I, P, P, P, GP, P],
    'dsnt_conv_fwd_ex': [P, P, P, P, P, P, I, P, P, P, GP, BP, TP, P],
    'dsnt_conv_fwd_bf16x6_ex': [P, P, L, P, P, P, P, I, P, P, P, GP, BP, TP, P],
    'dsnt_conv_pack_dgrad': [P, P, I, I, I, I, P],
    'dsnt_conv_pack_dgrad_all': [P, I, P, P, P, L, P],
    'dsnt_conv_fwd_bf16x6': [P, P, L, P, P, P, P, I, P, P, P, GP, P],
    'dsnt_split_bf16x3': [P, P, L, P],
    'dsnt_conv_fwd_f16x3_ex': [P, P, L, P, P, P, P, P, P, I, P, P, P, GP, BP, TP, P],
    'dsnt_conv_fwd_f16x3_stream': [P, P, L, P, P, P, P, P, P, I, P, P, P, GP, BP, TP, P],
    'dsnt_amax': [P, L, P, P],
    'dsnt_split_f16x2': [P, P, L, L, P, P],
    'dsnt_f16_prep_weights': [P, I, I, P],
    'dsnt_f16_prep_bn_bounds': [P, I, P],
    'dsnt_conv_wgrad': [P, P, P, I, P, P, P, P, I, GP, P],
    'dsnt_conv_wgrad_bf16x6': [P, P, P, I, P, P, P, P, I, GP, P],
    'dsnt_conv_wgrad_f16x3': [P, P, P, I, P, P, P, P, I, P, P, GP, P],
    'dsnt_conv1x1_fwd_f16x3': [P, P, L, P, P, P, P, P, P, I, P, P, GP, TP, P],
    'dsnt_conv1x1_bwd_f16x3': [BP, P, AP, P, L, P, P, P, P, P, P, P, I, GP, P],
    'dsnt_conv1x1_fwd_ds_f16x3': [P, P, P, P, L, P, P, P, P, P, P, P, P, P, I, P, GP, GP, TP, P],
    'dsnt_conv_dgrad_f16x3_stream_apply': [P, AP, P, P, L, P, P, P, P, I, GP, BP, TP, P],
    'dsnt_wgrad_reduce_all': [P, I, I, P],
    'dsnt_conv_wgrad_group': [P, I, I, P],
    'dsnt_bn_stats': [P, P, L, I, P],
    'dsnt_bn_finalize': [P, I, L, I, P, P, P, P, F, F, I, P, P, P, P, P],
    'dsnt_bn_act_fwd': [P, P, P, I, P, L, I, P],
    'dsnt_bn_act_bwd_reduce': [P, P, P, P, P, P, I, P, L, I, P],
    'dsnt_bn_bwd_finalize': [P, I, L, I, P, P, I, P, P],
    'dsnt_bn_bwd_finalize_bound': [P, I, L, I, P, P, I, P, P, P, P, P],
    'dsnt_bn_eval_prep': [P, I, P],
    'dsnt_bn_act_bwd_apply': [P, P, P, P, P, P, P, I, P, I, L, I, P],
    'dsnt_bn_act_bwd_apply_amax': [P, P, P, P, P, P, P, I, P, I, L, I, P, P],
    'dsnt_bn_act_bwd_apply_pro': [P, P, P, P, P, P, P, I, P, P, I, P, I, P, I, L, I, P, P],
    'dsnt_stem4_fwd_f16x3': [P, P, L, P, P, P, P, P, GP, TP, P],
    'dsnt_bn_add_act_bwd_reduce': [P, P, P, P, P, I, P, P, L, I, P],
    'dsnt_bn_act_bwd_apply_base': [P, P, P, P, P, P, P, I, P, P, L, I, P, P],
    'dsnt_bn_act_bwd_apply_pro_base': [P, P, P, P, P, P, P, I, P, P, I, P, I, P, P, L, I, P, P],
    'dsnt_conv_fwd_pro': [P, P, P, P, PP, I, P, P, P, GP, TP, P],
    'dsnt_fill_zero': [P, L, P],
    'dsnt_axpy_amax': [P, P, F, I, L, P, P],
    'dsnt_maxpool2_bwd_amax': [P, P, P, I, I, I, I, I, P, P],
    'dsnt_maxpool2_bwd_add': [P, P, P, I, P, I, I, I, I, P, P],
    'dsnt_upsample2_bwd_amax': [P, P, I, I, I, I, I, P, P],
    'dsnt_maxpool2_fwd': [P, P, P, I, I, I, I, P],
    'dsnt_maxpool2_bwd': [P, P, P, I, I, I, I, I, P],
    'dsnt_maxpool2_fwd_stats': [P, P, P, P, I, I, I, I, TP, P],
    'dsnt_upsample2_add_fwd_stats': [P, P, P, P, I, I, I, I, TP, P],
    'dsnt_bn_act_fwd_stats': [P, P, P, I, P, P, L, I, TP, P],
    'dsnt_s2d_input': [P, P, I, I, I, I, TP, P],
    'dsnt_s2d_weights': [P, P, I, I, P],
    'dsnt_s2d_weights_prep': [P, P, P, P, P, I, P],
    'dsnt_maxpool3s2_fwd': [P, P, P, I, I, I, I, P],
    'dsnt_maxpool3s2_bwd': [P, P, P, I, I, I, I, I, P],
    'dsnt_bn_add_act_fwd': [P, P, P, P, I, P, L, I, P],
    'dsnt_relu_bwd': [P, P, P, L, P],
    'dsnt_zero_insert': [P, P, I, I, I, I, I, I, I, P],
    'dsnt_conv_dgrad_strided': [P, P, P, P, P, GP, BP, TP, P],
    'dsnt_upsample2_add_fwd': [P, P, P, I, I, I, I, P],
    'dsnt_upsample2_bwd': [P, P, I, I, I, I, I, P],
    'dsnt_axpy': [P, P, F, I, L, P],
    'dsnt_nchw_to_nhwc': [P, P, I, I, I, I, P],
    'dsnt_nhwc_to_nchw': [P, P, I, I, I, I, P],
    'dsnt_rmsprop_step': [P, P, P, L, F, F, F, F, F, P],
    'dsnt_sgd_step': [P, P, P, L, F, F, F, F, I, P],
    'dsnt_rmsprop_step_guarded': [P, P, P, L, F, F, F, F, F, P, P],
    'dsnt_sgd_step_guarded': [P, P, P, L, F, F, F, F, I, P, P],
    'dsnt_nonfinite_flag': [P, L, P, I, P],
    'dsnt_pckh': [P, P, P, P, P, P, F, P, P, I, I, P],
    'dsnt_pckh_hist': [P, P, P, P, P, P, P, I, P, P, I, I, P],
    'dsnt_error_field': [P, P, P, P, P, P, F, P, I, P, P, I, I, P],
    'dsnt_score_hist': [P, P, P, P, P, P, P, P, I, P, I, P, I, I, P],
    'dsnt_score_lookup': [P, P, I, P, I, P, L, I, P],
    'dsnt_pckh_boot': [P, P, P, P, P, P, P, P, I, C.c_uint64, I, P, I, I, P],
    'dsnt_joint_confusion': [P, P, P, P, P, P, F, P, P, P, I, I, P],
    'dsnt_target_mass': [P, P, P, P, P, P, F, P, P, I, I, I, I, P],
    'dsnt_map_modes': [P, L, I, I, I, I, I, P, P, P, P, P, P, P],
    'dsnt_augment_fwd': [P, I, I, I, P, P, P, P, I, C.c_uint64, C.c_uint64, P, P, P, P],
    'dsnt_augment_fwd_pair': [P, I, I, I, P, P, P, P, I, C.c_uint64, C.c_uint64, P, P, P, P],
    'dsnt_augment_keypoints': [P, P, P, I, I, P, P, P, P, I, P, P, P, P, P],
    'dsnt_pool_normalize': [P, I, I, I, I, I, P, P, P, P],
    'dsnt_augment_fwd_gather': [P, L, P, I, I, I, P, P, P, P, I, C.c_uint64, C.c_uint64, C.c_uint32, P, P, P, P],
    'dsnt_augment_fwd_pair_gather': [P, L, P, I, I, I, P, P, P, P, I, C.c_uint64, C.c_uint64, C.c_uint32, P, P, P, P],
    'dsnt_augment_keypoints_gather': [P, P, P, P, L, P, I, I, P, P, P, P, I, P, P, P, P, P, P],
    'dsnt_epoch_indices': [L, C.c_uint64, C.c_uint64, L, L, I, P, P],
    'dsnt_sample_cdf': [P, L, P, P, P],
    'dsnt_sample_indices': [P, L, C.c_uint64, C.c_uint64, L, L, P, P],
    'dsnt_example_scores': [P, P, P, P, P, P, P, L, C.c_uint32, P, P, I, I, P],
    'dsnt_occlude': [P, P, I, I, I, I, I, C.c_uint32, I, I, P, P, P, P, P, I, P, P, P, I, C.c_uint64, C.c_uint64, C.c_uint32, P],
    'dsnt_crop_affine': [P, L, P, P, L, P, P, I, I, P, P, P],
    'dsnt_render_pose': [P, I, P, P, I, I, I, I, P, I, I, P, L, P, F, P, P, I, P, P, I, F, F, P, P],
}
PLAIN = {
    'dsnt_version': (I, []),
    'dsnt_last_error': (C.c_char_p, []),
    'dsnt_conv_fwd_bm': (I, [GP]),
    'dsnt_list_create': (P, []),
    'dsnt_list_destroy': (None, [P]),
    'dsnt_list_begin': (I, [P]),
    'dsnt_list_end': (I, []),
    'dsnt_list_sync': (I, [P, I, I]),
    'dsnt_list_mark': (I, [P]),
    'dsnt_list_segments': (I, [P]),
    'dsnt_list_size': (I, [P]),
    'dsnt_list_replay': (I, [P, I, C.POINTER(C.c_void_p), I]),
    'dsnt_conv_bf16x6_ok': (I, [GP]),
    'dsnt_conv_wgrad_bf16x6_ok': (I, [GP]),
    'dsnt_conv_wgrad_splits': (I, [GP]),
    'dsnt_conv_wgrad_halo_ok': (I, [GP]),
    'dsnt_conv_f16x3_route': (I, [GP, I]),
    'dsnt_conv_fwd_stream_ok': (I, [GP]),
    'dsnt_conv_fwd_stream_form': (I, [GP, I]),
    'dsnt_conv_dgrad_strided_ok': (I, [GP]),
    'dsnt_conv_dgrad_strided_tiles': (I, [GP]),
    'dsnt_conv_fwd_pro_ok': (I, [GP, I, I]),
    'dsnt_conv_wgrad_f16x3_splits': (I, [GP, I]),
    'dsnt_conv_wgrad_f16x3_ws_floats': (L, [GP, I]),
    'dsnt_conv_wgrad_ws_floats': (L, [GP]),
    'dsnt_conv1x1_fwd_ok': (I, [GP]),
    'dsnt_conv1x1_fwd_stats_rows': (I, [GP, I]),
    'dsnt_stem4_fwd_ok': (I, [GP]),
    'dsnt_stem4_fwd_stats_rows': (I, [GP]),
    'dsnt_conv1x1_bwd_ok': (I, [GP]),
    'dsnt_conv1x1_bwd_splits': (I, [GP, I]),
    'dsnt_conv1x1_bwd_ws_floats': (L, [GP, I]),
    'dsnt_conv_wgrad_desc_bytes': (I, []),
    'dsnt_conv_wgrad_desc': (I, [P, P, P, I, P, P, GP, P]),
    'dsnt_conv_wgrad_desc_f16x3': (I, [P, P, P, I, P, P, P, P, GP, P]),
}

_lib = None


def load():
    global _lib
    if _lib is None:
        if not os.path.exists(LIB_PATH):
            raise RuntimeError(
                'libdsnt_hip.so not found at %s — build it with `python dsnt-pose2d_amd/build.py` '
                '(there is no CPU fallback for the dsnt hot path)' % LIB_PATH)
        lib = C.CDLL(LIB_PATH)
        for name, argtypes in SIGNATURES.items():
            fn = getattr(lib, name)
            fn.argtypes = argtypes
            fn.restype = I
        for name, (res, argtypes) in PLAIN.items():
            fn = getattr(lib, name)
            fn.argtypes = argtypes
            fn.restype = res
        _lib = lib
    return _lib


def fn(name):
    return getattr(load(), name)


def stream_ptr():
    return torch.cuda.current_stream().cuda_stream


def call(name, *args):
    lib = load()
    rc = getattr(lib, name)(*args, stream_ptr())
    if rc != 0:
        raise RuntimeError('%s failed (%d): %s' % (name, rc, lib.dsnt_last_error().decode()))


def ptr(t):
    if t is None:
        return None
    if not t.is_cuda:
        raise RuntimeError('dsnt: tensor is on %s; the dsnt hot path runs on the HIP device only '
                           '(no CPU fallback)' % t.device)
    if not t.is_contiguous():
        raise RuntimeError('dsnt: tensor must be contiguous')
    return t.data_ptr()


def f32(t):
    if t.dtype != torch.float32:
        raise RuntimeError('dsnt: expected float32, got %s (the HIP path computes in fp32)' % t.dtype)
    return t
```

### dsnt-pose2d_amd/dsnt/convop.py

```python
import ctypes as C

import torch

from . import _lib
from ._lib import ConvGeom, BnBwdEpilogue, BnTail, BnPrologue, BnBwdApply


def use6(tape, g):
    return (tape.use_bf16x6 and g.N * g.Ho * g.Wo >= tape.bf16x6_min_rows and
            bool(tape.lib.dsnt_conv_bf16x6_ok(C.byref(g))))


def stream_ok(tape, p, g, res2):
    return (tape.conv3s and p.R == 3 and p.S == 3 and res2 is None and
            bool(tape.lib.dsnt_conv_fwd_stream_ok(C.byref(g))))


def share(tape, persistent=True):
    return 2 if (persistent and tape.lane != 0) else 0


def stats_tiles(tape, g, big):
    bm = 128 if big else tape.lib.dsnt_conv_fwd_bm(C.byref(g))
    return (g.N * g.Ho * g.Wo + bm - 1) // bm


def tail_at(slot):
    tl = BnTail()
    tl.amax = slot.data_ptr()
    return tl


def bn_epilogue(x, n):
    vectors = (n.scale, n.shift, n.mean, n.invstd) if n is not None else (None,) * 4
    return BnBwdEpilogue(_lib.ptr(x.buf), *(_lib.ptr(v) for v in vectors), 1 if (n is not None and n.relu) else 0)


def bn_apply(y, ap):
    n = ap.n
    return (BnBwdApply(_lib.ptr(y.buf), _lib.ptr(n.scale), _lib.ptr(n.mean), _lib.ptr(n.invstd), _lib.ptr(ap.coef)),
            dict(dz=ap.dz, y=y.buf, scale=n.scale, mean=n.mean, invstd=n.invstd, coef=ap.coef))


def ds_fuse_ok(tape, x, p_ds, p3):
    if not (tape.ds_fuse and tape.training and tape.record and tape.use_f16x3 and tape.fwd1):
        return False
    if not (p_ds.R == 1 and p_ds.S == 1 and p_ds.stride == 1 and p3.R == 1 and p3.S == 1 and p3.stride == 1 and
            (p_ds.Cin, p_ds.Cout) == (p3.Cin, p3.Cout) and (p3.Cin, p3.Cout) in ((64, 128), (128, 256)) and
            x.M >= tape.ds_fuse_rows and p_ds.post_reduce is None and p3.post_reduce is None):
        return False
    if any(p.wq is None or p.wq16 is None for p in (p_ds, p3)) or p_ds.wq_stride != p3.wq_stride:
        return False
    g = tape.geom(x, p_ds)
    if not (use6(tape, g) and tape.lib.dsnt_conv1x1_fwd_ok(C.byref(g))):
        return False
    return tape.bounds.operand_amax(x) is not None


class _Dgrad:
    __slots__ = ('native', 'gd', 'gsrc', 'wd', 'wq', 'wq_stride', 'wq16', 'wbd', 'g_amax', 'd6', 'd16', 'd_stream')

    def __init__(self, native, gd, gsrc, wd, wq, wq_stride, d6, g_amax, d16, d_stream, wq16, wbd):
        self.native, self.gd, self.gsrc = native, gd, gsrc
        self.wd, self.wq, self.wq_stride, self.d6 = wd, wq, wq_stride, d6
        self.g_amax, self.d16, self.d_stream, self.wq16, self.wbd = g_amax, d16, d_stream, wq16, wbd


class ConvOp:
    __slots__ = ('tape', 'src', 'x', 'y', 'p', 'g', 'res1', 'res2', 'name', 'normed', 'sc', 'sh', 'relu', 'need_input_grad', 'bucket',
                 'x_amax', 'use6', 'use16', 'slot', 'slot_k', 'fuse1', 'fold3_ok', 'gd')

    def __init__(self, tape, src, p, res1, res2, name, need_input_grad):
        from .engine import Normed
        self.tape, self.src, self.p, self.res1, self.res2, self.name = tape, src, p, res1, res2, name
        self.need_input_grad = need_input_grad
        self.normed = isinstance(src, Normed)
        self.x = src.x if self.normed else src
        self.g = tape.geom(self.x, p)
        self.sc, self.sh, self.relu = (src.scale, src.shift, 1 if src.relu else 0) if self.normed else (None, None, 0)
        self.bucket = tape.cur_bucket
        self.y = None
        self.x_amax, self.use6, self.use16 = None, False, False
        self.slot, self.slot_k, self.fuse1, self.fold3_ok, self.gd = None, None, False, False, None

    def operand_bound(self):
        bd = self.tape.bounds
        return bd.operand_amax_bn(self.src) if self.normed else bd.operand_amax(self.x)

    def dz_buffer(self, private):
        t, n = self.tape, self.x.M * self.x.C
        return t.empty(n) if private else t.scratch('da', n).view(-1)[:n]

    def a_operand(self, a_bound):
        return dict(x=self.x.buf, sc=self.sc, sh=self.sh, relu=self.relu, a_bound=a_bound)

    def use(self, e, kind, **operands):
        u = dict(kind=kind, name=self.name, **operands)
        if e is not None:
            self.tape.f16_uses.append((e, u))
        return u

    def forward(self, want_stats):
        t, lib, bd = self.tape, self.tape.lib, self.tape.bounds
        src, x, y, p, g, normed, res2 = self.src, self.x, self.y, self.p, self.g, self.normed, self.res2
        sc, sh, relu = self.sc, self.sh, self.relu
        if normed:
            t.check_lane(src)
        part, tail = None, None
        big = self.use6 = use6(t, g) and p.wq is not None
        can16 = big and p.wq16 is not None
        early = can16 and p.R == 1 and res2 is None and t.fwd1
        x_amax = self.operand_bound() if early else None
        f1 = bool(early and t.use_f16x3 and ((t.training and normed) or x_amax is not None) and
                  lib.dsnt_conv1x1_fwd_ok(C.byref(g)))
        f1_shr = share(t, f1)
        s4 = bool(can16 and t.use_f16x3 and t.stem4 and not normed and self.res1 is None and res2 is None and
                  lib.dsnt_stem4_fwd_ok(C.byref(g)))
        if want_stats and t.training:
            tiles = (lib.dsnt_conv1x1_fwd_stats_rows(C.byref(g), f1_shr) if f1 else
                     lib.dsnt_stem4_fwd_stats_rows(C.byref(g)) if s4 else stats_tiles(t, g, big))
            part = t.empty(tiles, 2, p.Cout)
            y.stats = (part, tiles)
        if big and t.use_f16x3:
            y.amax_tail = tail = BnTail()
        r1 = self.res1.buf if self.res1 is not None else None
        r2 = res2.buf if res2 is not None else None
        if t.use_f16x3 and t.training and normed:
            bd.f16_bn_bound(src)
        if can16 and not early:
            x_amax = self.operand_bound()
        self.x_amax = x_amax
        use16 = self.use16 = can16 and t.use_f16x3 and ((t.training and normed) or x_amax is not None)
        if normed and (use16 or big):
            t.materialize(src)
        if use16:
            st = stream_ok(t, p, g, res2)
            bd.f16_weights(p, stream=st)
            ab = bd.f16_bn_bound(src) if (normed and t.training) else x_amax
            if f1:
                e = t.f('dsnt_conv1x1_fwd_f16x3', x.buf, p.wq16, p.wq_stride, p.wb, ab, p.b, y.buf, sc, sh, relu | f1_shr, r1,
                        part, g, tail)
            elif s4:
                e = t.f('dsnt_stem4_fwd_f16x3', x.buf, p.wq16, p.wq_stride, p.wb, ab, p.b, y.buf, part, g, tail)
            else:
                e = t.f('dsnt_conv_fwd_f16x3_stream' if st else 'dsnt_conv_fwd_f16x3_ex', x.buf, p.wq16, p.wq_stride, p.wb, ab,
                        p.b, y.buf, sc, sh, relu | share(t, st or p.R == 1), r1, r2, part, g, None, tail)
            self.use(e, 'fwd', **self.a_operand(ab), w=p.w, w_bound=p.wb)
        elif big:
            t.f('dsnt_conv_fwd_bf16x6_ex', x.buf, p.wq, p.wq_stride, p.b, y.buf, sc, sh, relu, r1, r2, part, g,
                None, tail)
        elif normed and src.pending is not None and lib.dsnt_conv_fwd_pro_ok(C.byref(g), src.pending[1], src.bn.C):
            spart, stiles = src.pending
            src.pending = None
            bn = src.bn
            pro = BnPrologue(_lib.ptr(spart), stiles, bn.C, x.M, _lib.ptr(bn.gamma), _lib.ptr(bn.beta), _lib.ptr(bn.rmean),
                             _lib.ptr(bn.rvar), bn.momentum, bn.eps, _lib.ptr(src.mean), _lib.ptr(src.invstd),
                             _lib.ptr(src.scale), _lib.ptr(src.shift))
            t._keep.extend((spart, src.mean, src.invstd, src.scale, src.shift))
            t.f('dsnt_conv_fwd_pro', x.buf, p.w, p.b, y.buf, pro, relu, r1, r2, part, g, tail)
        else:
            if normed:
                t.materialize(src)
            t.f('dsnt_conv_fwd_ex', x.buf, p.w, p.b, y.buf, sc, sh, relu, r1, r2, part, g, None, tail)

    def forward_ds(self, cd, want_stats):
        t, bd = self.tape, self.tape.bounds
        src, x, y, p, g = self.src, self.x, self.y, self.p, self.g
        t.check_lane(src)
        self.use6 = cd.use6 = True
        self.use16 = cd.use16 = True
        shr = share(t)
        part = None
        if want_stats:
            tiles = t.lib.dsnt_conv1x1_fwd_stats_rows(C.byref(g), shr)
            part = t.empty(tiles, 2, p.Cout)
            y.stats = (part, tiles)
        y.amax_tail = tail = BnTail()
        ab = bd.f16_bn_bound(src)
        self.x_amax, cd.x_amax = None, bd.operand_amax(cd.x)
        t.materialize(src)
        for q in (p, cd.p):
            bd.f16_weights(q, stream=False)
        e = t.f('dsnt_conv1x1_fwd_ds_f16x3', x.buf, cd.x.buf, p.wq16, cd.p.wq16, p.wq_stride, p.wb, cd.p.wb, ab, cd.x_amax,
                p.b, cd.p.b, y.buf, self.sc, self.sh, self.relu | shr, part, g, cd.g, tail)
        self.use(e, 'fwd', **self.a_operand(ab), w=p.w, w_bound=p.wb)
        cd.use(e, 'fwd', **cd.a_operand(cd.x_amax), w=cd.p.w, w_bound=cd.p.wb)

    def plan_backward(self):
        t, x, y, p, g = self.tape, self.x, self.y, self.p, self.g
        if self.need_input_grad and t.param_arena is not None:
            self.slot, self.slot_k = t.bounds.dgrad_slot(p)
        one_pass = t.bwd1 and t.use_f16x3 and t.defer_reduce and self.slot is not None
        self.fuse1 = bool(one_pass and (self.normed or self.x_amax is not None) and p.R == 1 and p.S == 1 and
                          p.post_reduce is None and t.lib.dsnt_conv1x1_bwd_ok(C.byref(g)))
        plain = self.normed and self.res1 is None and self.res2 is None
        if p.stride == 1:
            self.gd = ConvGeom(x.N, g.Ho, g.Wo, p.Cout, x.H, x.W, p.Cin, p.R, p.S, 1, p.dil * (p.R - 1) - p.pad, p.dil)
        self.fold3_ok = bool(t.fold3 and one_pass and plain and t.training and p.R == 3 and p.S == 3 and self.gd is not None and
                             self.use16 and y.M >= t.fold3_rows and use6(t, self.gd) and stream_ok(t, p, self.gd, None))
        y.fold_ok = bool(self.fuse1 and plain) or self.fold3_ok

    def backward(self):
        t, y = self.tape, self.y
        gy, ap = y.grad, y.pending_apply
        fused = self.fuse1 and t.bounds.dgrad_planes16 is not None
        fold3 = bool(self.fold3_ok and ap is not None and gy is None and t.bounds.dgrad_planes16 is not None and
                     self.need_input_grad and ap.bound is not None)
        if ap is not None and (not fused or gy is not None) and not fold3:
            t.materialize_apply(y)
            ap, gy = None, y.grad
        assert gy is not None or ap is not None, 'no gradient reached conv output ' + self.name
        if fused and ap is None and y.grad_amax is None:
            fused = False
        wl, defer_res = t.lane, False
        if fused:
            self.backward_fused1(ap, gy)
        elif fold3:
            gy = y._grad = t.empty(y.N, y.H, y.W, y.C)
            y.grad_amax, y.pending_apply = ap.bound, None
            self.dgrad(gy, ap)
            wl, defer_res = self.wgrad(gy)
        else:
            wl, defer_res = self.wgrad(gy)
            self.dgrad(gy, None)
        self.residual_grads(gy, wl, defer_res)

    def backward_ds(self, cd):
        y = self.y
        if y.pending_apply is not None:
            self.tape.materialize_apply(y)
        assert y.grad is not None, 'no gradient reached conv output ' + self.name
        self.backward()
        cd.backward()

    def backward_fused1(self, ap, gy):
        t, lib, bd = self.tape, self.tape.lib, self.tape.bounds
        src, x, y, p, g, name = self.src, self.x, self.y, self.p, self.g, 'dsnt_conv1x1_bwd_f16x3'
        nw = p.w.numel()
        shr = share(t)
        nsp = lib.dsnt_conv1x1_bwd_splits(C.byref(g), shr)
        ws = t.wgrads.slab(p, lib.dsnt_conv1x1_bwd_ws_floats(C.byref(g), shr), nsp)
        wd, wq16, wbd = bd.dgrad_f16(self.slot, self.slot_k, nw)
        total = bd.dgrad_total
        if ap is not None:
            aps, applied = bn_apply(y, ap)
            dy, gb = ap.dz, ap.bound
            y.pending_apply = None
            grad = dict(g_apply=applied, g_bound=gb)
        else:
            aps, dy, gb = None, gy, y.grad_amax
            grad = dict(g=dy, g_bound=gb)
        if self.normed:
            ab = bd.f16_bn_bound_bwd(src)
            fold = t.fold_ok(src)
            dz = self.dz_buffer(fold)
            dz_amax = bd.amax_slot() if fold else None
            part = t.scratch('bnpart', nsp * 2 * x.C).view(-1)
            e = t.b(name, bn_epilogue(x, src), dy, aps, wq16, total, wbd, ab, gb, dz, part, ws, dz_amax, shr, g)
        else:
            ab = self.x_amax
            buf, acc = t.grad_target(x, amax=True)
            e = t.b(name, bn_epilogue(x, None), dy, None, wq16, total, wbd, ab, gb, buf, None, ws,
                    x.grad_amax, shr | acc, g)
        t.bwd.count(name, 4 * (x.buf.numel() + (y.buf.numel() if ap is not None else 0)))
        self.use(e, 'bwd1', **self.a_operand(ab), w=wd, w_bound=wbd, **grad)
        if self.normed:
            t._norm_backward(src, dz, reduced=(part, nsp), finalised=False, dz_amax=dz_amax)

    def wgrad(self, gy):
        t, p, g = self.tape, self.p, self.g
        cur = t.lane
        w6 = t.use_bf16x6 and bool(t.lib.dsnt_conv_wgrad_bf16x6_ok(C.byref(g)))
        defer_res = False
        with t.wgrads.placed(self, gy) as (wl, shr):
            if t.defer_reduce:
                defer_res = self.wgrad_slab(gy, shr, w6, wl == cur)
            else:
                ws = t.scratch('wgrad', t.lib.dsnt_conv_wgrad_ws_floats(C.byref(g)))
                t.b('dsnt_conv_wgrad_bf16x6' if w6 else 'dsnt_conv_wgrad', self.x.buf, self.sc, self.sh, self.relu, gy, ws, p.gw, p.gb, 0, g)
                if p.post_reduce is not None:
                    t.b(p.post_reduce[0], *p.post_reduce[1])
        return wl, defer_res

    def wgrad_slab(self, gy, shr, w6, on_chain):
        t, lib = self.tape, self.tape.lib
        x, y, p, g, normed, sc, sh, relu = self.x, self.y, self.p, self.g, self.normed, self.sc, self.sh, self.relu
        groupable = (w6 and (normed or t.share_grads) and on_chain and not y.grad_shared and
                     0 < g.N * g.Ho * g.Wo <= t.group_rows)
        residuals = [r for r in (self.res1, self.res2) if r is not None]
        defer_res = bool(groupable and residuals and t.share_grads and t.defer_res and all(r.untouched for r in residuals))
        grouped = groupable and (not residuals or defer_res)
        w16 = w6 and t.use_f16x3 and (normed or self.x_amax is not None) and y.grad_amax is not None
        ab = (t.bounds.f16_bn_bound_bwd(self.src) if normed else self.x_amax) if w16 else None
        if w16 and not grouped:
            nws = lib.dsnt_conv_wgrad_f16x3_ws_floats(C.byref(g), shr)
            splits = lib.dsnt_conv_wgrad_f16x3_splits(C.byref(g), shr)
        else:
            nws, splits = lib.dsnt_conv_wgrad_ws_floats(C.byref(g)), lib.dsnt_conv_wgrad_splits(C.byref(g))
        ws = t.wgrads.slab(p, nws, splits)
        if grouped:
            desc = C.create_string_buffer(lib.dsnt_conv_wgrad_desc_bytes())
            gsc, gsh = (sc, sh) if normed else t.identity_bn(x.C)
            if w16:
                nblk = lib.dsnt_conv_wgrad_desc_f16x3(_lib.ptr(x.buf), _lib.ptr(gsc), _lib.ptr(gsh), relu, _lib.ptr(gy),
                                                      _lib.ptr(ws), _lib.ptr(ab), _lib.ptr(y.grad_amax), C.byref(g), desc)
            else:
                nblk = lib.dsnt_conv_wgrad_desc(_lib.ptr(x.buf), _lib.ptr(gsc), _lib.ptr(gsh), relu, _lib.ptr(gy),
                                                _lib.ptr(ws), C.byref(g), desc)
            if nblk <= 0:
                raise RuntimeError('dsnt_conv_wgrad_desc failed: %s' % lib.dsnt_last_error().decode())
            t.wgrads.group(desc.raw, nblk, self.use(None, 'wgrad', **self.a_operand(ab), g=gy, g_bound=y.grad_amax) if w16 else None)
        elif w16:
            e = t.b('dsnt_conv_wgrad_f16x3', x.buf, sc, sh, relu, gy, ws, None, None, shr, ab, y.grad_amax, g)
            self.use(e, 'wgrad', **self.a_operand(ab), g=gy, g_bound=y.grad_amax)
        else:
            t.b('dsnt_conv_wgrad_bf16x6' if w6 else 'dsnt_conv_wgrad', x.buf, sc, sh, relu, gy, ws, None, None,
                shr if w6 else 0, g)
        return defer_res

    def dgrad_operands(self, gy):
        t, x, p, g, bd = self.tape, self.x, self.p, self.g, self.tape.bounds
        nw = p.w.numel()
        pad_d = p.dil * (p.R - 1) - p.pad
        assert pad_d >= 0, 'data gradient needs pad <= dil * (R - 1)'
        native = p.stride != 1 and self.slot is not None and t.lib.dsnt_conv_dgrad_strided_ok(C.byref(g))
        gd, gsrc = self.gd, gy
        if p.stride != 1 and not native:
            Hs, Ws = x.H + 2 * p.pad - p.dil * (p.R - 1), x.W + 2 * p.pad - p.dil * (p.S - 1)
            gsrc = t.scratch('stuffed', x.N * Hs * Ws * p.Cout).view(-1)[:x.N * Hs * Ws * p.Cout]
            t.b('dsnt_zero_insert', gy, gsrc, x.N, g.Ho, g.Wo, p.Cout, Hs, Ws, p.stride)
            gd = ConvGeom(x.N, Hs, Ws, p.Cout, x.H, x.W, p.Cin, p.R, p.S, 1, pad_d, p.dil)
        wq = wq_stride = None
        if self.slot is not None:
            wd = bd.dgrad_f32[self.slot:self.slot + nw]
            wq, wq_stride = bd.dgrad_planes[self.slot:self.slot + nw], bd.dgrad_total
            d6 = gd is not None and use6(t, gd)
        else:
            wd = t.scratch('wdgrad', nw)
            t.b('dsnt_conv_pack_dgrad', p.w, wd, p.Cout, p.R, p.S, p.Cin)
            d6 = use6(t, gd) and nw % 8 == 0
            if d6:
                wq, wq_stride = t.scratch('wdgrad6', 3 * nw, torch.bfloat16, 8), nw
                t.b('dsnt_split_bf16x3', wd, wq, nw)
        g_amax = self.y.grad_amax if (t.use_f16x3 and p.stride == 1) else None
        d16 = d6 and g_amax is not None and self.slot is not None and bd.dgrad_planes16 is not None
        d_stream = wq16 = wbd = None
        if d16:
            d_stream = stream_ok(t, p, gd, None)
            _, wq16, wbd = bd.dgrad_f16(self.slot, self.slot_k, nw, (p.Cin, p.Cout) if d_stream else (0, 0))
        return _Dgrad(native, gd, gsrc, wd, wq, wq_stride, d6, g_amax, d16, d_stream, wq16, wbd)

    def dgrad_launch(self, d, out, res, part=None, bnb=None, tail=None):
        t = self.tape
        if d.native:
            t.b('dsnt_conv_dgrad_strided', d.gsrc, d.wd, out, res, part, self.g, bnb, tail)
        elif d.d16:
            e = t.b('dsnt_conv_fwd_f16x3_stream' if d.d_stream else 'dsnt_conv_fwd_f16x3_ex', d.gsrc, d.wq16, t.bounds.dgrad_total,
                    d.wbd, d.g_amax, None, out, None, None, share(t, d.d_stream or self.p.R == 1), res, None, part, d.gd, bnb, tail)
            self.use(e, 'dgrad', g=d.gsrc, g_bound=d.g_amax, w=d.wd, w_bound=d.wbd)
        elif d.d6:
            t.b('dsnt_conv_fwd_bf16x6_ex', d.gsrc, d.wq, d.wq_stride, None, out, None, None, 0, res, None, part, d.gd, bnb, tail)
        else:
            t.b('dsnt_conv_fwd_ex', d.gsrc, d.wd, None, out, None, None, 0, res, None, part, d.gd, bnb, tail)

    def dgrad(self, gy, ap):
        if not self.need_input_grad:
            return
        t, src, x, y = self.tape, self.src, self.x, self.y
        d = self.dgrad_operands(gy)
        if not self.normed:
            buf, acc, base = t.grad_target_base(x, amax=bool(d.d6 or d.native))
            tl = tail_at(x.grad_amax) if x.grad_amax is not None else None
            self.dgrad_launch(d, buf, base if base is not None else (buf if acc else None), tail=tl)
            return
        fold = not d.native and t.fold_ok(src)
        dz = self.dz_buffer(fold)
        tiles = t.lib.dsnt_conv_dgrad_strided_tiles(C.byref(self.g)) if d.native else stats_tiles(t, d.gd, d.d6)
        part = t.scratch('bnpart', tiles * 2 * x.C).view(-1)
        bnb = bn_epilogue(x, src)
        tl, dz_amax = None, None
        if fold:
            dz_amax = t.bounds.amax_slot()
            tl = tail_at(dz_amax)
        if ap is not None:
            assert d.d16 and d.d_stream and not d.native
            name = 'dsnt_conv_dgrad_f16x3_stream_apply'
            aps, applied = bn_apply(y, ap)
            e = t.b(name, ap.dz, aps, gy, d.wq16, t.bounds.dgrad_total, d.wbd, ap.bound, dz, part, share(t), d.gd, bnb, tl)
            t.bwd.count(name, 4 * y.buf.numel())
            self.use(e, 'dgrad', w=d.wd, w_bound=d.wbd, g_bound=ap.bound, g_apply=applied)
        else:
            self.dgrad_launch(d, dz, None, part, bnb, tl)
        t._norm_backward(src, dz, reduced=(part, tiles), dz_amax=dz_amax)

    def residual_grads(self, gy, wl, defer_res):
        t, y = self.tape, self.y
        if self.res1 is not None or self.res2 is not None:
            t.sync_bwd(wl, t.lane)
        donated = False
        for r in (self.res1, self.res2):
            if r is None:
                continue
            if defer_res:
                r.base, r.base_amax = gy, y.grad_amax
            elif (donated and t.share_grads and r.grad is None and r.pending_apply is None and r.uses == 1 and
                    not r.gives_away and not r.is_branch):
                r.grad, r.grad_amax, r.grad_shared = gy, y.grad_amax, True
            else:
                donated = t.grad_identity(r, gy, donate=not donated, g_amax=y.grad_amax) or donated
```

### dsnt-pose2d_amd/dsnt/engine.py

```python
import os

import torch

from . import _lib, convop
from ._lib import ConvGeom, BnTail
from .bounds import Bounds
from .launchlist import Lanes, LaunchList
from .wgrad_queue import WgradQueue

BN_EPS = 1e-5
BN_MOMENTUM = 0.1


class Act:
    __slots__ = ('buf', 'N', 'H', 'W', 'C', '_grad', 'stats', 'name', 'grad_amax', 'amax_tail', 'fold_ok',
                 'pending_apply', 'uses', 'gives_away', 'is_branch', 'grad_shared', 'pending_add', 'base', 'base_amax')

    def __init__(self, buf, name=''):
        self.buf = buf
        self.N, self.H, self.W, self.C = buf.shape
        self._grad = None
        self.base, self.base_amax = None, None
        self.stats = None
        self.amax_tail = None
        self.grad_amax = None
        self.fold_ok = False
        self.pending_apply = None
        self.uses = 0
        self.gives_away = False
        self.is_branch = False
        self.grad_shared = False
        self.pending_add = None
        self.name = name

    @property
    def M(self):
        return self.N * self.H * self.W

    @property
    def untouched(self):
        return self._grad is None and self.base is None and self.pending_apply is None and self.pending_add is None

    @property
    def grad(self):
        if self._grad is None and self.base is not None:
            self._grad, self.grad_amax, self.grad_shared = self.base, self.base_amax, True
        return self._grad

    @grad.setter
    def grad(self, g):
        self._grad = g


class ConvParams:
    __slots__ = ('w', 'b', 'gw', 'gb', 'Cout', 'R', 'S', 'Cin', 'stride', 'pad', 'dil', 'wq', 'wq_stride', 'wq16', 'wb',
                 'post_reduce')

    def __init__(self, w, b, gw, gb, stride=1, pad=0, dil=1):
        self.w, self.b, self.gw, self.gb = w, b, gw, gb
        self.wq, self.wq_stride = None, 0
        self.wq16, self.wb = None, None
        self.post_reduce = None
        self.Cout, self.R, self.S, self.Cin = w.shape
        self.stride, self.pad, self.dil = stride, pad, dil


class BnParams:
    __slots__ = ('gamma', 'beta', 'ggamma', 'gbeta', 'rmean', 'rvar', 'C', 'uses', 'momentum', 'eps')

    def __init__(self, gamma, beta, ggamma, gbeta, rmean, rvar, momentum=BN_MOMENTUM, eps=BN_EPS):
        self.gamma, self.beta, self.ggamma, self.gbeta = gamma, beta, ggamma, gbeta
        self.rmean, self.rvar = rmean, rvar
        self.momentum, self.eps = float(momentum), float(eps)
        self.C = gamma.numel()
        self.uses = 0


class Normed:
    __slots__ = ('x', 'bn', 'mean', 'invstd', 'scale', 'shift', 'relu', 'abound', 'pending', 'lane')


class PendingApply:
    __slots__ = ('dz', 'n', 'coef', 'bound', 'dz_amax')

    def __init__(self, dz, n, coef, bound, dz_amax):
        self.dz, self.n, self.coef, self.bound, self.dz_amax = dz, n, coef, bound, dz_amax


class Tape:
    def __init__(self, device, training, record=None, want_input_grad=False):
        self.device = device
        self.training = training
        self.record = training if record is None else bool(record)
        self.want_input_grad = want_input_grad
        self._bwd_emitters = []
        self._scratch = {}
        self._keep = []
        self.lib = _lib.load()
        self.nbytes = 0
        self._read_switches()
        lanes = Lanes(self.use_lanes, self.n_lanes)
        self.fwd, self.bwd = (LaunchList(self.lib, lanes, self._keep) for _ in range(2))
        self.bounds = Bounds(self)
        self.wgrads = WgradQueue(self)
        self.lane = 0
        self.cur_bucket = 0
        self._ident = None
        self.acts = []
        self.param_arena = None
        self._planar_src = {}
        self.f16_uses = []

    def _read_switches(self):
        self.use_bf16x6 = os.environ.get('DSNT_MFMA', 'bf16x6') != 'f32'
        self.bf16x6_min_rows = int(os.environ.get('DSNT_BF16X6_MIN_ROWS', '4096'))
        self.use_lanes = os.environ.get('DSNT_LANES', '1') != '0'
        self.side_lanes = (1, 3)
        self.n_lanes = 3 + len(self.side_lanes) - 1
        self.chain_lanes = (0,) + self.side_lanes
        self.wgrad_lane = 2 if (self.use_lanes and os.environ.get('DSNT_WGRAD_LANE', '1') != '0') else None
        self.wgrad_lane_rows = int(os.environ.get('DSNT_X_WGRAD_LANE_ROWS', '16000'))
        self.release_rows = int(os.environ.get('DSNT_X_RELEASE_ROWS', '4096'))
        off = set(os.environ.get('DSNT_OFF', '').replace('+', ',').split(','))
        self.conv3s = 'conv3s' not in off
        self.bwd1 = 'bwd1' not in off
        self.fwd1 = 'fwd1' not in off
        self.fold3 = 'fold3' not in off
        self.fold3_rows = int(os.environ.get('DSNT_X_FOLD3_ROWS', '16384'))
        self.stem4 = 'stem4' not in off
        self.ds_fuse = 'dsfuse' not in off
        self.ds_fuse_rows = int(os.environ.get('DSNT_X_DS_FUSE_ROWS', '65536'))
        self._x = dict(kv.split('=') for kv in os.environ.get('DSNT_X', '').split(',') if '=' in kv)
        self.wgrad_narrow = self._x.get('wgrad_narrow', '1')
        self.share_grads = self._x.get('share_grads', '1') != '0'
        self.defer_res = self._x.get('defer_res', '1') != '0'
        self.flush_points = self._x.get('flush_points', '1') != '0'
        self.prep_split = self._x.get('prep_split', '1') != '0'
        self.defer_reduce = os.environ.get('DSNT_DEFER_REDUCE', '1') != '0'
        self.group_rows = int(os.environ.get('DSNT_X_GROUP_ROWS', '8192')) if self.defer_reduce else 0
        self.fuse_finalize = os.environ.get('DSNT_FUSE_FINALIZE', '1') != '0'
        self.fuse_finalize_max = int(os.environ.get('DSNT_X_FUSE_FINALIZE_MAX', '2048'))
        self.use_f16x3 = self.use_bf16x6 and os.environ.get('DSNT_SPLIT', 'f16x3') == 'f16x3'
        if self.record and not self.training:
            self.use_f16x3 = False
        self.no_relu = bool(os.environ.get('DSNT_DEBUG_NO_RELU'))

    def empty(self, *shape, dtype=torch.float32):
        t = torch.empty(*shape, device=self.device, dtype=dtype)
        self.nbytes += t.numel() * t.element_size()
        self._keep.append(t)
        return t

    def scratch(self, key, numel, dtype=torch.float32, least=1):
        key = (key, self.lane)
        t = self._scratch.get(key)
        if t is None or t.numel() < numel:
            if t is not None:
                self._keep.append(t)
            t = torch.empty(max(numel, least), device=self.device, dtype=dtype)
            self.nbytes += t.numel() * t.element_size()
            self._scratch[key] = t
        return t

    def upload(self, rows, dtype=torch.int64):
        t = torch.tensor(rows, dtype=dtype).to(self.device)
        self._keep.append(t)
        return t

    def act(self, N, H, W, Cc, name=''):
        a = Act(self.empty(N, H, W, Cc), name)
        self.acts.append(a)
        return a

    def f(self, name, *args):
        return self.fwd.emit(self.lane, name, *args)

    def b(self, name, *args):
        return self.bwd.emit(self.lane, name, *args)

    def b_amax(self, name, *args, amax):
        return self.b(name, *args) if amax is None else self.b(name + '_amax', *args, amax)

    bytes_fwd = property(lambda self: self.fwd.nbytes)
    bytes_bwd = property(lambda self: self.bwd.nbytes)

    @property
    def bytes_by_name(self):
        both = dict(self.fwd.bytes_by_name)
        for name, nb in self.bwd.bytes_by_name.items():
            both[name] = both.get(name, 0) + nb
        return both

    def on_backward(self, fn):
        lane = self.lane

        def emit():
            saved, self.lane = self.lane, lane
            try:
                fn()
            finally:
                self.lane = saved
        self._bwd_emitters.append(emit)

    def sync(self, src, dst, bwd=True):
        if not self.use_lanes:
            return
        self.fwd.sync(src, dst)
        if self.record and bwd:
            self._bwd_emitters.append(lambda: self.bwd.sync(dst, src))

    def sync_bwd(self, src, dst):
        if self.use_lanes and src != dst:
            self.bwd.sync(src, dst)

    def branch(self, x, join=True):
        if not self.use_lanes:
            return x
        xb = Act(x.buf, x.name + '/branch')
        xb.stats, xb.amax_tail = x.stats, x.amax_tail
        xb.is_branch = True
        x.uses += 1
        if self.record and join:
            def join_grad():
                if xb.grad is not None:
                    self.grad_identity(x, xb.grad, donate=False, g_amax=xb.grad_amax)
            self.on_backward(join_grad)
        return xb

    def finish(self):
        self.bounds.close_dgrad()
        prep_pos = len(self.bwd)
        self.wgrads.begin_backward()
        for fn in reversed(self._bwd_emitters):
            fn()
        self._bwd_emitters = []
        self.bounds.emit_backward_zero(prep_pos)
        if self.wgrads.pending:
            self.wgrads.flush()

    def mark_bucket(self, k):
        self.cur_bucket = k
        if self.record:
            self.on_backward(lambda: self.wgrads.flush(bucket=k))

    def flush_point(self):
        if self.record and self.defer_reduce and self.flush_points:
            self.on_backward(self.wgrads.flush)

    def run(self, lst, bucket_hook=None, probe=None):
        lst.replay(bucket_hook, probe)

    def add_later(self, a, g, g_amax=None):
        assert a.grad is not None and a.pending_add is None
        a.pending_add = (g, g_amax)

    def _flush_add(self, a):
        (g, g_amax), a.pending_add = a.pending_add, None
        self.grad_identity(a, g, donate=False, g_amax=g_amax)

    def identity_bn(self, Cc):
        if self._ident is None or self._ident[0].numel() < Cc:
            n = max(Cc, 2048)
            self._ident = (torch.ones(n, device=self.device), torch.zeros(n, device=self.device))
        return self._ident

    def grad_target(self, a, amax=False, take_add=False):
        buf, acc, base = self.grad_target_base(a, amax, take_add)
        if base is not None:
            self.b_amax('dsnt_axpy', base, buf, 1.0, 0, base.numel(), amax=a.grad_amax)
            acc = 1
        return buf, acc

    def grad_target_base(self, a, amax=False, take_add=False):
        if a.pending_apply is not None:
            self.materialize_apply(a)
        if a.pending_add is not None and not take_add:
            self._flush_add(a)
        if a.base is not None:
            base, a.base, a.base_amax = a.base, None, None
            a._grad, a.grad_shared = self.empty(a.N, a.H, a.W, a.C), False
            a.grad_amax = self.bounds.amax_slot() if (self.use_f16x3 and amax) else None
            return a._grad, 0, base
        acc = 1
        if a.grad is None:
            a.grad = self.empty(a.N, a.H, a.W, a.C)
            acc = 0
        else:
            self.wgrads.before_write(a.grad)
        if self.use_f16x3 and amax:
            if a.grad_amax is None:
                a.grad_amax = self.bounds.amax_slot()
        else:
            a.grad_amax = None
        return a.grad, acc, None

    def grad_identity(self, a, g, donate, g_amax=None):
        if a.pending_apply is not None:
            self.materialize_apply(a)
        if a.pending_add is not None:
            self._flush_add(a)
        if a.grad is None and donate:
            a.grad = g
            a.grad_amax = g_amax
            return True
        buf, acc = self.grad_target(a, amax=True)
        self.b_amax('dsnt_axpy', g, buf, 1.0, acc, g.numel(), amax=a.grad_amax)
        return False

    def geom(self, x, p):
        Ho = (x.H + 2 * p.pad - p.dil * (p.R - 1) - 1) // p.stride + 1
        Wo = (x.W + 2 * p.pad - p.dil * (p.S - 1) - 1) // p.stride + 1
        assert x.C == p.Cin, (x.C, p.Cin)
        return ConvGeom(x.N, x.H, x.W, p.Cin, Ho, Wo, p.Cout, p.R, p.S, p.stride, p.pad, p.dil)

    def ensure_stats(self, a):
        if a.stats is None:
            tiles = (a.M + 127) // 128
            part = self.empty(tiles, 2, a.C)
            self.f('dsnt_bn_stats', a.buf, part, a.M, a.C)
            a.stats = (part, tiles)
        return a.stats

    def finalize_in_consumer(self, bn, tiles):
        return self.fuse_finalize and bn.C <= 256 and tiles * bn.C <= self.fuse_finalize_max

    def norm(self, x, bn, relu=True):
        if self.no_relu:
            relu = False
        n = Normed()
        n.x, n.bn, n.relu = x, bn, relu
        n.abound = None
        n.mean, n.invstd, n.scale, n.shift = (self.empty(bn.C) for _ in range(4))
        n.pending = None
        n.lane = self.lane
        if self.training:
            n.pending = self.ensure_stats(x)
            if not self.finalize_in_consumer(bn, n.pending[1]):
                self.materialize(n)
        else:
            self.bounds.eval_bn(n)
        return n

    def check_lane(self, n):
        if n.pending is not None:
            n.lane = self.lane
        elif n.lane != self.lane:
            raise RuntimeError('dsnt: BatchNorm vectors finalised on lane %d are read on lane %d without a synchronisation '
                               '(trace norm() and its consumers on one lane, or sync the lanes)' % (n.lane, self.lane))

    def materialize(self, n):
        self.check_lane(n)
        if n.pending is not None:
            part, tiles = n.pending
            n.pending = None
            bn = n.bn
            self.f('dsnt_bn_finalize', part, tiles, n.x.M, bn.C, bn.gamma, bn.beta, bn.rmean, bn.rvar,
                   bn.momentum, bn.eps, 1, n.mean, n.invstd, n.scale, n.shift)

    def fold_ok(self, n):
        x = n.x
        return bool(self.bwd1 and x.fold_ok and x.grad is None and x.pending_apply is None)

    def materialize_apply(self, x):
        ap, x.pending_apply = x.pending_apply, None
        n = ap.n
        buf, acc = self.grad_target(x, amax=True)
        self.b_amax('dsnt_bn_act_bwd_apply', ap.dz, x.buf, n.scale, n.shift, n.mean, n.invstd, ap.coef, 0,
                    buf, acc, x.M, n.bn.C, amax=x.grad_amax)

    def _norm_backward(self, n, da, reduced=None, finalised=False, dz_amax=None):
        x, bn = n.x, n.bn
        coef = self.scratch('bncoef', 2 * bn.C)
        relu = 1 if n.relu else 0
        if reduced is not None:
            part, tiles = reduced
            relu = 0
        else:
            tiles = (x.M + 127) // 128
            part = self.scratch('bnpart', tiles * 2 * bn.C).view(-1)
            self.b('dsnt_bn_act_bwd_reduce', da, x.buf, n.scale, n.shift, n.mean, n.invstd, relu, part,
                   x.M, bn.C)
        if dz_amax is not None:
            assert reduced is not None and not finalised and x.grad is None
            acc_p = 1 if bn.uses > 0 else 0
            bn.uses += 1
            coef = self.empty(2 * bn.C)
            bound = self.bounds.amax_slot()
            self.b('dsnt_bn_bwd_finalize_bound', part, tiles, x.M, bn.C, bn.ggamma, bn.gbeta, acc_p, coef, n.scale,
                   dz_amax, bound)
            x.pending_apply = PendingApply(da, n, coef, bound, dz_amax)
            return
        frozen = not self.training
        fused = (not finalised) and self.finalize_in_consumer(bn, tiles) and not frozen
        assert not (frozen and finalised)
        if not finalised:
            acc_p = 1 if bn.uses > 0 else 0
            bn.uses += 1
            if not fused:
                self.b('dsnt_bn_bwd_finalize', part, tiles, x.M, bn.C, bn.ggamma, bn.gbeta, acc_p | (2 if frozen else 0), coef)
        buf, acc, base = self.grad_target_base(x, amax=True)
        if fused:
            coef = self.empty(2 * bn.C)
            if base is not None:
                self.b('dsnt_bn_act_bwd_apply_pro_base', da, x.buf, n.scale, n.shift, n.mean, n.invstd, part, tiles,
                       bn.ggamma, bn.gbeta, acc_p, coef, relu, base, buf, x.M, bn.C, x.grad_amax)
            else:
                self.b('dsnt_bn_act_bwd_apply_pro', da, x.buf, n.scale, n.shift, n.mean, n.invstd, part, tiles,
                       bn.ggamma, bn.gbeta, acc_p, coef, relu, buf, acc, x.M, bn.C, x.grad_amax)
        elif base is not None:
            self.b('dsnt_bn_act_bwd_apply_base', da, x.buf, n.scale, n.shift, n.mean, n.invstd, coef, relu,
                   base, buf, x.M, bn.C, x.grad_amax)
        else:
            self.b_amax('dsnt_bn_act_bwd_apply', da, x.buf, n.scale, n.shift, n.mean, n.invstd, coef, relu,
                        buf, acc, x.M, bn.C, amax=x.grad_amax)

    def conv(self, src, p, res1=None, res2=None, want_stats=False, need_input_grad=True, name=''):
        c = convop.ConvOp(self, src, p, res1, res2, name, need_input_grad)
        c.y = y = self.act(c.x.N, c.g.Ho, c.g.Wo, p.Cout, name)
        c.x.uses += 1
        for r in (res1, res2):
            if r is not None:
                r.uses += 1
                y.gives_away = True
        c.forward(want_stats)
        if self.record:
            c.plan_backward()
            self.on_backward(c.backward)
        return y

    def ds_fuse_ok(self, x, p_ds, p3):
        return convop.ds_fuse_ok(self, x, p_ds, p3)

    def conv_ds(self, src, p, x_ds, p_ds, want_stats=False, name='', name_ds='ds'):
        c, cd = convop.ConvOp(self, src, p, None, None, name, True), convop.ConvOp(self, x_ds, p_ds, None, None, name_ds, True)
        c.y = cd.y = y = self.act(c.x.N, c.g.Ho, c.g.Wo, p.Cout, name)
        c.x.uses += 1
        x_ds.uses += 1
        c.forward_ds(cd, want_stats)
        cd.plan_backward()
        c.plan_backward()
        y.fold_ok = False
        self.on_backward(lambda: c.backward_ds(cd))
        return y

    def _f_with_stats(self, name, y, tensors, dims):
        part = None
        if self.training:
            tiles = (y.M + 127) // 128
            part = self.empty(tiles, 2, y.C)
            y.stats = (part, tiles)
        if self.use_f16x3 and y.M >= self.bf16x6_min_rows:
            y.amax_tail = BnTail()
        if part is None and y.amax_tail is None:
            self.f(name, *tensors, *dims)
        else:
            self.f(name + '_stats', *tensors, part, *dims, y.amax_tail)

    def bn_act(self, x, bn, relu=True, name=''):
        n = self.norm(x, bn, relu)
        self.materialize(n)
        y = self.act(x.N, x.H, x.W, x.C, name)
        x.uses += 1
        self._f_with_stats('dsnt_bn_act_fwd', y, (x.buf, n.scale, n.shift, 1 if n.relu else 0, y.buf), (x.M, x.C))
        if self.record:
            def backward():
                self._norm_backward(n, y.grad)
            self.on_backward(backward)
        return y

    def maxpool2(self, x, name=''):
        y = self.act(x.N, x.H // 2, x.W // 2, x.C, name)
        x.uses += 1
        idx = self.empty(x.N, x.H // 2, x.W // 2, x.C, dtype=torch.uint8)
        self._f_with_stats('dsnt_maxpool2_fwd', y, (x.buf, y.buf, idx), (x.N, x.H, x.W, x.C))
        if self.record:
            def backward():
                add, x.pending_add = x.pending_add, None
                buf, acc = self.grad_target(x, amax=True, take_add=True)
                if add is not None:
                    assert acc == 1
                    self.b('dsnt_maxpool2_bwd_add', y.grad, idx, buf, acc, add[0], x.N, x.H, x.W, x.C, x.grad_amax)
                else:
                    self.b_amax('dsnt_maxpool2_bwd', y.grad, idx, buf, acc, x.N, x.H, x.W, x.C, amax=x.grad_amax)
            self.on_backward(backward)
        return y

    def maxpool3s2(self, x, name=''):
        Ho, Wo = (x.H - 1) // 2 + 1, (x.W - 1) // 2 + 1
        y = self.act(x.N, Ho, Wo, x.C, name)
        x.uses += 1
        idx = self.empty(x.N, Ho, Wo, x.C, dtype=torch.uint8)
        self.f('dsnt_maxpool3s2_fwd', x.buf, y.buf, idx, x.N, x.H, x.W, x.C)
        if self.record:
            def backward():
                buf, acc = self.grad_target(x)
                self.b('dsnt_maxpool3s2_bwd', y.grad, idx, buf, acc, x.N, x.H, x.W, x.C)
            self.on_backward(backward)
        return y

    def bn_add_act(self, x, bn, skip, relu=True, name=''):
        n = self.norm(x, bn, relu=False)
        y = self.act(x.N, x.H, x.W, x.C, name)
        x.uses += 1
        skip.uses += 1
        if self.no_relu:
            relu = False
        self.materialize(n)
        self.f('dsnt_bn_add_act_fwd', x.buf, n.scale, n.shift, skip.buf, 1 if relu else 0, y.buf, x.M, x.C)
        if self.record:
            def backward():
                share = bool(self.share_grads and skip.untouched)
                if relu:
                    dz = (self.empty(x.M * x.C) if share else self.scratch('dz_tail', x.M * x.C).view(-1)[:x.M * x.C])
                    tiles = (x.M + 127) // 128
                    part = self.scratch('bnpart', tiles * 2 * bn.C).view(-1)
                    self.b('dsnt_bn_add_act_bwd_reduce', y.grad, y.buf, x.buf, n.mean, n.invstd, 1, dz, part, x.M, bn.C)
                    self._norm_backward(n, dz, reduced=(part, tiles))
                else:
                    dz = y.grad
                    self._norm_backward(n, dz)
                if share and skip.untouched:
                    skip.base, skip.base_amax = dz, None
                else:
                    self.grad_identity(skip, dz, donate=False)
            self.on_backward(backward)
        return y

    def upsample2_add(self, up, low, name=''):
        out = self.act(up.N, up.H, up.W, up.C, name)
        up.uses += 1
        low.uses += 1
        out.gives_away = True
        self._f_with_stats('dsnt_upsample2_add_fwd', out, (up.buf, low.buf, out.buf), (up.N, up.H, up.W, up.C))
        if self.record:
            point = self.wgrads.release_point(low.M)

            def backward():
                if point:
                    self.wgrads.pass_release_point()
                buf, acc = self.grad_target(low, amax=True)
                self.b_amax('dsnt_upsample2_bwd', out.grad, buf, acc, up.N, up.H, up.W, up.C, amax=low.grad_amax)
                self.grad_identity(up, out.grad, donate=True, g_amax=out.grad_amax)
            self.on_backward(backward)
        return out

    def to_planar(self, x, C_logical, name='', out=None, gin=None):
        out = self.empty(x.N, C_logical, x.H, x.W) if out is None else out
        x.uses += 1
        if gin is None:
            gin = self.empty(x.N, C_logical, x.H, x.W) if self.record else None
        self.f('dsnt_nhwc_to_nchw', x.buf, out, x.N, C_logical, x.H * x.W, x.C)
        if self.record:
            def backward():
                assert x.grad is None, 'planar output must be the first gradient writer'
                buf, _ = self.grad_target(x)
                self.b('dsnt_nchw_to_nhwc', gin, buf, x.N, C_logical, x.H * x.W, x.C)
            self.on_backward(backward)
        return out, gin

    def from_planar(self, src_nchw, Cpad, name=''):
        N, Cc, H, W = src_nchw.shape
        a = self.act(N, H, W, Cpad, name)
        e = self.f('dsnt_nchw_to_nhwc', src_nchw, a.buf, N, Cc, H * W, Cpad)
        self._planar_src[id(a)] = (src_nchw, e)
        return a

    def stem_s2d(self, x, p, name='stem'):
        got = self._planar_src.get(id(x))
        if (got is None or not self.use_f16x3 or p.R != 7 or p.S != 7 or p.stride != 2 or p.pad != 3
                or p.dil != 1 or x.C != 4 or x.H % 2 or x.W % 2 or x.N * (x.H // 2) * (x.W // 2) < self.bf16x6_min_rows):
            return None
        src, entry = got
        self.fwd.remove(entry)
        xs = self.act(x.N, x.H // 2 + 1, x.W // 2 + 1, 16, 'input_s2d')
        xs.amax_tail = BnTail()
        self.f('dsnt_s2d_input', src, xs.buf, x.N, src.shape[1], x.H, x.W, xs.amax_tail)
        n = p.Cout * 256
        w2, gw2 = self.empty(p.Cout, 4, 4, 16), self.empty(p.Cout, 4, 4, 16)
        p2 = ConvParams(w2, p.b, gw2, p.gb, 1, 1, 1)
        p2.wq, p2.wq_stride = self.empty(3 * n, dtype=torch.bfloat16), n
        p2.wq16, p2.wb = self.empty(2 * n, dtype=torch.float16), self.empty(64)
        p2.post_reduce = ('dsnt_s2d_weights', (gw2, p.gw, p.Cout, 1))
        self.f('dsnt_s2d_weights_prep', p.w, w2, p2.wq16, p2.wq, p2.wb, p.Cout)
        self.bounds.prepared_elsewhere(p2.wq16)
        mark = len(self.fwd)
        y = self.conv(xs, p2, want_stats=True, need_input_grad=False, name=name)
        self.bounds.exempt(self.fwd[mark:])
        return y
```

### include/dsnt_hip.h

```cpp
#ifndef DSNT_HIP_H
#define DSNT_HIP_H

#include <stdint.h>

#ifdef __cplusplus
extern "C" {
#endif

typedef enum {
    DSNT_OK = 0,
    DSNT_ERR_SHAPE = 1,
    DSNT_ERR_ALIGN = 2,
    DSNT_ERR_ARG = 3,
    DSNT_ERR_HIP = 4
} dsnt_status;

typedef struct {
    float* amax;
    float* amax_bn; const float* amax_scale; const float* amax_shift; int amax_relu, reserved;
} dsnt_out_bounds;

typedef struct dsnt_bn_prologue {
    const float* partial; int tiles, C;
    int64_t M;
    const float* gamma; const float* beta;
    float* running_mean; float* running_var;
    float momentum, eps;
    float* mean; float* invstd; float* scale; float* shift;
} dsnt_bn_prologue;

int dsnt_version(void);
const char* dsnt_last_error(void);


int dsnt_preact_fwd(const float* x, float* y, int64_t rows, int hw, int mode,
                    float threshold, float eps, void* stream);
int dsnt_preact_bwd(const float* x, const float* y, const float* gy, float* gx,
                    int64_t rows, int hw, int mode, float threshold, float eps, void* stream);

int dsnt_expect_fwd(const float* hm, float* coords, int64_t rows, int h, int w, void* stream);
int dsnt_expect_bwd(const float* gcoords, float* ghm, int64_t rows, int h, int w, void* stream);

int dsnt_make_gauss(const float* coords, float* out, int64_t rows, int h, int w, float sigma,
                    void* stream);
int dsnt_make_gauss_bwd(const float* coords, const float* g_out, float* g_coords, int64_t rows, int h, int w,
                        float sigma, void* stream);

int dsnt_fc2_fwd(const float* hm, const float* w, const float* b, float* out, int64_t rows, int hw, void* stream);
int dsnt_fc2_bwd(const float* g, const float* hm, const float* w, float* ghm, float* gw, float* gb, int64_t rows,
                 int hw, void* stream);

int dsnt_reg_fwd(const float* hm, const float* target, float* per_row, int64_t rows, int h, int w,
                 float sigma, int kind, void* stream);
int dsnt_reg_bwd(const float* hm, const float* target, const float* g_row, float* ghm,
                 int64_t rows, int h, int w, float sigma, int kind, void* stream);
int dsnt_reg_bwd_mu(const float* hm, const float* target, const float* g_row, float* gmu,
                    int64_t rows, int h, int w, float sigma, int kind, void* stream);

int dsnt_euclid_fwd(const float* actual, const float* target, float* dist, int64_t n, int d,
                    void* stream);
int dsnt_euclid_bwd(const float* actual, const float* target, const float* dist,
                    const float* g_dist, float* g_actual, int64_t n, int d, void* stream);

int dsnt_masked_avg_fwd(const float* losses, const float* mask, float* out2, int64_t n,
                        void* stream);
int dsnt_masked_avg_bwd(const float* g_out, const float* mask, const float* out2,
                        float* g_losses, int64_t n, void* stream);

int dsnt_head_fwd(const float* logits, float* hm, float* coords, int64_t rows, int h, int w,
                  void* stream);
#define DSNT_FLIP_DSNT 0
#define DSNT_FLIP_GAUSS 1
int dsnt_flip_merge_head(const float* logits, int64_t B, int J, int h, int w, const int* perm, int strategy,
                         int preact, float threshold, float eps, const double* transform_m, const double* transform_b,
                         float* hm, float* coords, double* img, void* stream);
int dsnt_heatmap_stats(const float* hm, int64_t rows, int h, int w, float* stats, int* peak_index, void* stream);
int dsnt_flip_merge_head_stats(const float* logits, int64_t B, int J, int h, int w, const int* perm, int strategy,
                               int preact, float threshold, float eps, const double* transform_m,
                               const double* transform_b, float* hm, float* coords, double* img, float* stats,
                               int* peak_index, double* cov_image, void* stream);
int dsnt_head_loss_rows(const float* hm, const float* coords, const float* target,
                        float* dist, float* reg_row, int64_t rows, int h, int w, float sigma,
                        int reg_kind, void* stream);
int dsnt_mask_denom(const float* mask, float* denom2, int64_t n, void* stream);
int dsnt_head_loss_grad(const float* hm, const float* coords, const float* target, const float* mask,
                        const float* denom2, float* dist, float* reg_row, float* g_logits, int64_t rows, int h, int w,
                        float sigma, int reg_kind, float reg_coeff, void* stream);
int dsnt_head_loss_reduce(const float* dist, const float* reg_row, const float* mask, const float* denom2,
                          float reg_coeff, float* loss, float* e2, int64_t rows, void* stream);
int dsnt_scale_by_scalar(float* x, const float* s, int64_t n, void* stream);
int dsnt_head_bwd(const float* hm, const float* coords, const float* target, const float* dist,
                  const float* g_dist, const float* g_reg, float* g_logits, int64_t rows,
                  int h, int w, float sigma, int reg_kind, void* stream);

typedef struct {
    int N, H, W, Cin;
    int Ho, Wo, Cout;
    int R, S;
    int stride, pad, dil;
} dsnt_conv_geom;

int dsnt_conv_fwd(const float* x, const float* w, const float* bias, float* y,
                  const float* in_scale, const float* in_shift, int in_relu,
                  const float* res1, const float* res2, float* stats_partial,
                  const dsnt_conv_geom* g, void* stream);

typedef struct {
    const float* x;
    const float* scale; const float* shift; const float* mean; const float* invstd;
    int relu;
} dsnt_bn_bwd_epilogue;
int dsnt_conv_fwd_ex(const float* x, const float* w, const float* bias, float* y,
                     const float* in_scale, const float* in_shift, int in_relu,
                     const float* res1, const float* res2, float* stats_partial,
                     const dsnt_conv_geom* g, const dsnt_bn_bwd_epilogue* bnb, const dsnt_out_bounds* tail, void* stream);

int dsnt_conv_fwd_pro_ok(const dsnt_conv_geom* g, int tiles, int C);
int dsnt_conv_fwd_pro(const float* x, const float* w, const float* bias, float* y, const dsnt_bn_prologue* pro,
                      int in_relu, const float* res1, const float* res2, float* stats_partial,
                      const dsnt_conv_geom* g, const dsnt_out_bounds* tail, void* stream);

int dsnt_conv_fwd_bm(const dsnt_conv_geom* g);

int dsnt_conv_bf16x6_ok(const dsnt_conv_geom* g);
int dsnt_split_bf16x3(const float* src, void* dst_planes, int64_t n, void* stream);
int dsnt_conv_fwd_bf16x6(const float* x, const void* w_planes, int64_t plane_stride, const float* bias, float* y,
                         const float* in_scale, const float* in_shift, int in_relu,
                         const float* res1, const float* res2, float* stats_partial,
                         const dsnt_conv_geom* g, void* stream);

int dsnt_conv_fwd_bf16x6_ex(const float* x, const void* w_planes, int64_t plane_stride, const float* bias,
                            float* y, const float* in_scale, const float* in_shift, int in_relu,
                            const float* res1, const float* res2, float* stats_partial,
                            const dsnt_conv_geom* g, const dsnt_bn_bwd_epilogue* bnb, const dsnt_out_bounds* tail,
                            void* stream);

int dsnt_conv_fwd_f16x3_ex(const float* x, const void* w_planes, int64_t plane_stride, const float* w_bound,
                           const float* a_bound, const float* bias, float* y, const float* in_scale,
                           const float* in_shift, int in_relu, const float* res1, const float* res2,
                           float* stats_partial, const dsnt_conv_geom* g, const dsnt_bn_bwd_epilogue* bnb,
                           const dsnt_out_bounds* tail, void* stream);
#define DSNT_CONV_SHARE_CHIP 2
int dsnt_conv_fwd_f16x3_stream(const float* x, const void* w_planes, int64_t plane_stride, const float* w_bound,
                               const float* a_bound, const float* bias, float* y, const float* in_scale,
                               const float* in_shift, int in_relu, const float* res1, const float* res2,
                               float* stats_partial, const dsnt_conv_geom* g, const dsnt_bn_bwd_epilogue* bnb,
                               const dsnt_out_bounds* tail, void* stream);
int dsnt_conv_fwd_stream_ok(const dsnt_conv_geom* g);
int dsnt_conv_fwd_stream_form(const dsnt_conv_geom* g, int mode);
int dsnt_amax(const float* src, int64_t n, float* out, void* stream);
int dsnt_split_f16x2(const float* src, void* dst, int64_t n, int64_t plane_stride, const float* bound, void* stream);
int dsnt_f16_prep_weights(const int64_t* table, int rows, int row_ints, void* stream);
int dsnt_f16_prep_bn_bounds(const int64_t* table, int rows, void* stream);

int dsnt_conv_pack_dgrad(const float* w, float* wd, int Cout, int R, int S, int Cin,
                         void* stream);

int dsnt_conv_pack_dgrad_all(const int* table, int nconv, const float* params, float* out,
                             void* planes, int64_t total, void* stream);

#define DSNT_WGRAD_SHARE_CHIP 2
#define DSNT_WGRAD_NARROW 4
int64_t dsnt_conv_wgrad_ws_floats(const dsnt_conv_geom* g);
int dsnt_conv_wgrad(const float* x, const float* in_scale, const float* in_shift, int in_relu,
                    const float* dy, float* ws, float* dw, float* dbias, int accumulate,
                    const dsnt_conv_geom* g, void* stream);

int dsnt_conv_wgrad_bf16x6_ok(const dsnt_conv_geom* g);
int dsnt_conv_wgrad_bf16x6(const float* x, const float* in_scale, const float* in_shift, int in_relu,
                           const float* dy, float* ws, float* dw, float* dbias, int accumulate,
                           const dsnt_conv_geom* g, void* stream);

int dsnt_conv_wgrad_splits(const dsnt_conv_geom* g);
int dsnt_wgrad_reduce_all(const int64_t* table, int rows, int max_blocks, void* stream);

int dsnt_conv_wgrad_desc_bytes(void);
int dsnt_conv_wgrad_desc(const float* x, const float* in_scale, const float* in_shift, int in_relu,
                         const float* dy, float* ws, const dsnt_conv_geom* g, void* desc_out);
int dsnt_conv_wgrad_group(const void* table, int nconv, int max_blocks, void* stream);

int dsnt_conv_wgrad_f16x3(const float* x, const float* in_scale, const float* in_shift, int in_relu,
                          const float* dy, float* ws, float* dw, float* dbias, int accumulate,
                          const float* a_bound, const float* g_bound, const dsnt_conv_geom* g, void* stream);
int dsnt_conv_wgrad_desc_f16x3(const float* x, const float* in_scale, const float* in_shift, int in_relu,
                               const float* dy, float* ws, const float* a_bound, const float* g_bound,
                               const dsnt_conv_geom* g, void* desc_out);
int dsnt_conv_wgrad_halo_ok(const dsnt_conv_geom* g);
int dsnt_conv_f16x3_route(const dsnt_conv_geom* g, int wgrad);
int dsnt_conv_wgrad_f16x3_splits(const dsnt_conv_geom* g, int accumulate);
int64_t dsnt_conv_wgrad_f16x3_ws_floats(const dsnt_conv_geom* g, int accumulate);

int dsnt_conv1x1_fwd_ok(const dsnt_conv_geom* g);
int dsnt_conv1x1_fwd_stats_rows(const dsnt_conv_geom* g, int in_relu);
int dsnt_conv1x1_fwd_f16x3(const float* x, const void* w_planes, int64_t plane_stride, const float* w_bound,
                           const float* a_bound, const float* bias, float* y, const float* in_scale,
                           const float* in_shift, int in_relu, const float* res1, float* stats_partial,
                           const dsnt_conv_geom* g, const dsnt_out_bounds* tail, void* stream);
int dsnt_conv1x1_fwd_ds_f16x3(const float* x, const float* x_ds, const void* w_planes, const void* w_planes_ds,
                              int64_t plane_stride, const float* w_bound, const float* w_bound_ds, const float* a_bound,
                              const float* a_bound_ds, const float* bias, const float* bias_ds, float* y,
                              const float* in_scale, const float* in_shift, int in_relu, float* stats_partial,
                              const dsnt_conv_geom* g, const dsnt_conv_geom* g_ds, const dsnt_out_bounds* tail, void* stream);
int dsnt_stem4_fwd_ok(const dsnt_conv_geom* g);
int dsnt_stem4_fwd_stats_rows(const dsnt_conv_geom* g);
int dsnt_stem4_fwd_f16x3(const float* x, const void* w_planes, int64_t plane_stride, const float* w_bound,
                         const float* a_bound, const float* bias, float* y, float* stats_partial,
                         const dsnt_conv_geom* g, const dsnt_out_bounds* tail, void* stream);


typedef struct {
    const float* y;
    const float* scale; const float* mean; const float* invstd;
    const float* coef;
} dsnt_bn_bwd_apply;
int dsnt_conv1x1_bwd_ok(const dsnt_conv_geom* g);
int dsnt_conv1x1_bwd_splits(const dsnt_conv_geom* g, int flags);
int64_t dsnt_conv1x1_bwd_ws_floats(const dsnt_conv_geom* g, int flags);
int dsnt_conv1x1_bwd_f16x3(const dsnt_bn_bwd_epilogue* xs, const float* dy, const dsnt_bn_bwd_apply* ap,
                           const void* wd_planes, int64_t plane_stride, const float* w_bound, const float* a_bound,
                           const float* g_bound, float* dz_out, float* stats_partial, float* ws, float* dz_amax,
                           int flags, const dsnt_conv_geom* g, void* stream);
int dsnt_conv_dgrad_f16x3_stream_apply(const float* dz, const dsnt_bn_bwd_apply* ap, float* dy_out,
                                       const void* w_planes, int64_t plane_stride, const float* w_bound,
                                       const float* a_bound, float* dx_dz, float* stats_partial, int flags,
                                       const dsnt_conv_geom* g, const dsnt_bn_bwd_epilogue* bnb,
                                       const dsnt_out_bounds* tail, void* stream);

int dsnt_encode_heatmaps(const float* target, float* out, int64_t rows, int h, int w, float sigma, void* stream);
int dsnt_heatmap_mse_fwd(const float* hm, const float* target, float* per_row, int64_t rows, int h, int w,
                         float sigma, void* stream);
int dsnt_heatmap_mse_bwd(const float* hm, const float* target, const float* gscale, float* dhm, int64_t rows,
                         int h, int w, float sigma, void* stream);
int dsnt_decode_heatmaps(const float* hm, float* coords, int64_t rows, int h, int w, int use_neighbours,
                         void* stream);


int dsnt_bn_stats(const float* x, float* partial, int64_t M, int C, void* stream);

int dsnt_bn_finalize(const float* partial, int ntiles, int64_t M, int C,
                     const float* gamma, const float* beta,
                     float* running_mean, float* running_var, float momentum, float eps,
                     int training, float* mean, float* invstd, float* scale, float* shift,
                     void* stream);

int dsnt_bn_act_fwd(const float* x, const float* scale, const float* shift, int relu,
                    float* y, int64_t M, int C, void* stream);

int dsnt_bn_eval_prep(const int64_t* table, int rows, void* stream);
#define DSNT_BN_FROZEN 2
int dsnt_bn_act_bwd_reduce(const float* da, const float* x, const float* scale,
                           const float* shift, const float* mean, const float* invstd,
                           int relu, float* partial, int64_t M, int C, void* stream);
int dsnt_bn_add_act_bwd_reduce(const float* da, const float* y, const float* x, const float* mean, const float* invstd,
                               int relu, float* dz, float* partial, int64_t M, int C, void* stream);
int dsnt_bn_bwd_finalize(const float* partial, int ntiles, int64_t M, int C,
                         float* dgamma, float* dbeta, int accumulate, float* coef,
                         void* stream);
int dsnt_bn_bwd_finalize_bound(const float* partial, int ntiles, int64_t M, int C, float* dgamma, float* dbeta,
                               int accumulate, float* coef, const float* scale, const float* dz_amax, float* bound_out,
                               void* stream);
int dsnt_bn_act_bwd_apply(const float* da, const float* x, const float* scale,
                          const float* shift, const float* mean, const float* invstd,
                          const float* coef, int relu, float* dx, int accumulate,
                          int64_t M, int C, void* stream);
int dsnt_bn_act_bwd_apply_amax(const float* da, const float* x, const float* scale, const float* shift,
                               const float* mean, const float* invstd, const float* coef, int relu, float* dx,
                               int accumulate, int64_t M, int C, float* amax, void* stream);
int dsnt_bn_act_bwd_apply_pro(const float* da, const float* x, const float* scale, const float* shift,
                              const float* mean, const float* invstd, const float* partial, int ntiles,
                              float* dgamma, float* dbeta, int accumulate_params, float* coef, int relu,
                              float* dx, int accumulate, int64_t M, int C, float* amax, void* stream);
int dsnt_bn_act_bwd_apply_base(const float* da, const float* x, const float* scale, const float* shift,
                               const float* mean, const float* invstd, const float* coef, int relu,
                               const float* base, float* dx, int64_t M, int C, float* amax, void* stream);
int dsnt_bn_act_bwd_apply_pro_base(const float* da, const float* x, const float* scale, const float* shift,
                                   const float* mean, const float* invstd, const float* partial, int ntiles,
                                   float* dgamma, float* dbeta, int accumulate_params, float* coef, int relu,
                                   const float* base, float* dx, int64_t M, int C, float* amax, void* stream);
int dsnt_fill_zero(float* p, int64_t n, void* stream);
int dsnt_axpy_amax(const float* x, float* y, float a, int accumulate, int64_t n, float* amax, void* stream);
int dsnt_maxpool2_bwd_amax(const float* dy, const uint8_t* idx, float* dx, int accumulate, int N, int H, int W, int C,
                           float* amax, void* stream);
int dsnt_maxpool2_bwd_add(const float* dy, const uint8_t* idx, float* dx, int accumulate, const float* extra,
                          int N, int H, int W, int C, float* amax, void* stream);
int dsnt_upsample2_bwd_amax(const float* dout, float* dlow, int accumulate, int N, int H, int W, int C, float* amax,
                            void* stream);

int dsnt_maxpool2_fwd(const float* x, float* y, uint8_t* idx, int N, int H, int W, int C,
                      void* stream);
int dsnt_maxpool2_bwd(const float* dy, const uint8_t* idx, float* dx, int accumulate,
                      int N, int H, int W, int C, void* stream);

int dsnt_maxpool3s2_fwd(const float* x, float* y, uint8_t* idx, int N, int H, int W, int C, void* stream);
int dsnt_maxpool3s2_bwd(const float* dy, const uint8_t* idx, float* dx, int accumulate, int N, int H, int W,
                        int C, void* stream);
int dsnt_bn_add_act_fwd(const float* x, const float* scale, const float* shift, const float* res, int relu,
                        float* y, int64_t M, int C, void* stream);
int dsnt_relu_bwd(const float* dy, const float* y, float* dz, int64_t n, void* stream);
int dsnt_zero_insert(const float* dy, float* out, int N, int Ho, int Wo, int C, int Hs, int Ws, int stride,
                     void* stream);

int dsnt_conv_dgrad_strided(const float* dy, const float* wd, float* dx, const float* res1, float* stats_partial,
                            const dsnt_conv_geom* g, const dsnt_bn_bwd_epilogue* bnb, const dsnt_out_bounds* tail, void* stream);
int dsnt_conv_dgrad_strided_ok(const dsnt_conv_geom* g);
int dsnt_conv_dgrad_strided_tiles(const dsnt_conv_geom* g);

int dsnt_upsample2_add_fwd(const float* up, const float* low, float* out,
                           int N, int H, int W, int C, void* stream);
int dsnt_upsample2_bwd(const float* dout, float* dlow, int accumulate,
                       int N, int H, int W, int C, void* stream);

int dsnt_maxpool2_fwd_stats(const float* x, float* y, uint8_t* idx, float* partial, int N, int H, int W, int C,
                            const dsnt_out_bounds* tail, void* stream);
int dsnt_upsample2_add_fwd_stats(const float* up, const float* low, float* out, float* partial, int N, int H, int W,
                                 int C, const dsnt_out_bounds* tail, void* stream);
int dsnt_bn_act_fwd_stats(const float* x, const float* scale, const float* shift, int relu, float* y, float* partial,
                          int64_t M, int C, const dsnt_out_bounds* tail, void* stream);

int dsnt_s2d_input(const float* src_nchw, float* dst, int N, int C, int H, int W, const dsnt_out_bounds* tail, void* stream);
int dsnt_s2d_weights(const float* w, float* w2, int Cout, int back, void* stream);
int dsnt_s2d_weights_prep(const float* w, float* w2, void* planes16, void* planes_bf16, float* bound, int Cout, void* stream);

int dsnt_axpy(const float* x, float* y, float a, int accumulate, int64_t n, void* stream);

int dsnt_nchw_to_nhwc(const float* src, float* dst, int N, int C, int HW, int Cpad, void* stream);
int dsnt_nhwc_to_nchw(const float* src, float* dst, int N, int C, int HW, int Cpad, void* stream);

int dsnt_rmsprop_step(float* p, const float* g, float* square_avg, int64_t n, float lr,
                      float alpha, float eps, float weight_decay, float grad_scale, void* stream);
int dsnt_sgd_step(float* p, const float* g, float* momentum_buf, int64_t n, float lr,
                  float momentum, float weight_decay, float grad_scale, int first_step,
                  void* stream);
#define DSNT_FLAG_LOSS 1
#define DSNT_FLAG_GRAD 2
int dsnt_rmsprop_step_guarded(float* p, const float* g, float* square_avg, int64_t n, float lr, float alpha,
                              float eps, float weight_decay, float grad_scale, int* flag, void* stream);
int dsnt_sgd_step_guarded(float* p, const float* g, float* momentum_buf, int64_t n, float lr, float momentum,
                          float weight_decay, float grad_scale, int first_step, int* flag, void* stream);
int dsnt_nonfinite_flag(const float* x, int64_t n, int* flag, int code, void* stream);

#define DSNT_MAX_LANES 8
typedef struct dsnt_list dsnt_list;
dsnt_list* dsnt_list_create(void);
void dsnt_list_destroy(dsnt_list* l);
int dsnt_list_begin(dsnt_list* l);
int dsnt_list_end(void);
int dsnt_list_sync(dsnt_list* l, int src_lane, int dst_lane);
int dsnt_list_mark(dsnt_list* l);
int dsnt_list_segments(const dsnt_list* l);
int dsnt_list_size(const dsnt_list* l);
int dsnt_list_replay(const dsnt_list* l, int segment, void* const* streams, int nstreams);

int dsnt_pckh(const float* pred, const float* target, const double* m, const double* b,
              const float* mask, const double* head, float threshold, float* hits,
              float* valid, int B, int J, void* stream);
#define DSNT_PCKH_HIST_MAX_T 64
#define DSNT_PCKH_HIST_LDS_CELLS 4096
#define DSNT_PCKH_HIST_BLOCK 256
#define DSNT_PCKH_HIST_MAX_BLOCKS 64
int dsnt_pckh_hist(const float* pred, const float* target, const double* m, const double* b,
                   const float* mask, const double* head, const double* thresholds, int T,
                   unsigned long long* table, double* dist, int B, int J, void* stream);
#define DSNT_ERROR_FIELD_MAX_BINS 32
#define DSNT_ERROR_FIELD_BLOCK 256
int dsnt_error_field(const float* pred, const float* target, const double* m, const double* b,
                     const float* mask, const double* head, float threshold,
                     const double* edges, int bins, int64_t* counts, double* sums,
                     int B, int J, void* stream);
#define DSNT_SCORE_HIST_MAX_S 64
#define DSNT_SCORE_HIST_LDS_CELLS 8192
int dsnt_score_hist(const float* pred, const float* target, const double* m, const double* b,
                    const float* mask, const double* head, const float* score,
                    const double* score_edges, int S, const double* thresholds, int T,
                    unsigned long long* table, int B, int J, void* stream);
#define DSNT_SCORE_LOOKUP_BLOCK 256
#define DSNT_SCORE_LOOKUP_MAX_BLOCKS 1024
int dsnt_score_lookup(const float* score, const double* score_edges, int S, const float* values,
                      int per_joint, float* out, int64_t n, int J, void* stream);
#define DSNT_PCKH_BOOT_DOMAIN 0x424F4F54u
#define DSNT_PCKH_BOOT_CDF { 1580030168u, 3160060337u, 3950075421u, 4213413783u, 4279248373u, 4292415291u, 4294609777u, 4294923276u, 4294962463u, 4294966817u, 4294967252u, 4294967292u }
#define DSNT_PCKH_BOOT_MAX_B 357913941
#define DSNT_PCKH_BOOT_LDS_CELLS 4096
#define DSNT_PCKH_BOOT_BLOCK 256
#define DSNT_PCKH_BOOT_CHUNK 32
#define DSNT_PCKH_BOOT_SPAN 1024
#define DSNT_PCKH_BOOT_MAX_CHUNK_BLOCKS 1024
#define DSNT_PCKH_BOOT_MAX_SPAN_BLOCKS 16
int dsnt_pckh_boot(const float* pred, const float* target, const double* m, const double* b,
                   const float* mask, const double* head, const int64_t* ids,
                   const double* thresholds, int T, uint64_t seed, int R,
                   unsigned long long* table, int B, int J, void* stream);
#define DSNT_CONFUSION_MAX_J 64
#define DSNT_CONFUSION_BLOCK 256
#define DSNT_CONFUSION_MAX_BLOCKS 64
int dsnt_joint_confusion(const float* pred, const float* target, const double* m, const double* b,
                         const float* mask, const double* head, float threshold, const int* mirror,
                         unsigned long long* table, unsigned long long* mutual, int B, int J, void* stream);
#define DSNT_TARGET_MASS_BLOCK 256
int dsnt_target_mass(const float* heatmaps, const float* target, const double* m, const double* b,
                     const float* mask, const double* head, float threshold, const int* mirror, float* out,
                     int B, int J, int h, int w, void* stream);
#define DSNT_MODES_MAX_RADIUS 8
#define DSNT_MODES_MAX_K 4
#define DSNT_MODES_MAX_PIXELS 8192
int dsnt_map_modes(const float* hm, int64_t rows, int J, int h, int w, int radius, int K,
                   const double* transform_m, const double* transform_b,
                   float* coords, float* mass, int* index, double* image, void* stream);

int dsnt_augment_fwd(const uint8_t* src, int B, int R, int S, float* scale, float* rot_deg, uint8_t* hflip,
                     float* gain, int draw, uint64_t seed, uint64_t step, const float* mean, const float* stdv,
                     float* out, void* stream);
int dsnt_augment_fwd_pair(const uint8_t* src, int B, int R, int S, float* scale, float* rot_deg, uint8_t* hflip,
                          float* gain, int draw, uint64_t seed, uint64_t step, const float* mean, const float* stdv,
                          float* out, void* stream);
int dsnt_augment_keypoints(const double* matrix, const double* keypoints, const float* keypoint_mask, int B, int J,
                           const float* scale, const float* rot_deg, const uint8_t* hflip, const int64_t* flip_idx,
                           int train, float* part_coords, float* part_mask, double* trans_m, double* trans_b,
                           void* stream);
int dsnt_augment_fwd_gather(const uint8_t* pool, int64_t N, const int64_t* idx, int B, int R, int S, float* scale,
                            float* rot_deg, uint8_t* hflip, float* gain, int draw, uint64_t seed, uint64_t step,
                            uint32_t draw_offset, const float* mean, const float* stdv, float* out, void* stream);
int dsnt_augment_fwd_pair_gather(const uint8_t* pool, int64_t N, const int64_t* idx, int B, int R, int S, float* scale,
                                 float* rot_deg, uint8_t* hflip, float* gain, int draw, uint64_t seed, uint64_t step,
                                 uint32_t draw_offset, const float* mean, const float* stdv, float* out, void* stream);
int dsnt_augment_keypoints_gather(const double* matrix_pool, const double* kp_pool, const float* mask_pool,
                                  const double* head_len_pool, int64_t N, const int64_t* idx, int B, int J,
                                  const float* scale, const float* rot_deg, const uint8_t* hflip, const int64_t* flip_idx,
                                  int train, float* part_coords, float* part_mask, double* trans_m, double* trans_b,
                                  double* normalize, void* stream);
int dsnt_epoch_indices(int64_t n, uint64_t seed, uint64_t epoch, int64_t first, int64_t count, int shuffle, int64_t* out,
                       void* stream);
#define DSNT_SAMPLE_MAX_N (1 << 24)
#define DSNT_SAMPLE_TILE 1024
#define DSNT_SAMPLE_CDF_SCRATCH_BYTES(n) (8 * (1 + ((int64_t)(n) + DSNT_SAMPLE_TILE - 1) / DSNT_SAMPLE_TILE))
int dsnt_sample_cdf(const float* weights, int64_t n, uint64_t* cdf, void* scratch, void* stream);
#define DSNT_SAMPLE_DOMAIN 0x57534D50u
int dsnt_sample_indices(const uint64_t* cdf, int64_t n, uint64_t seed, uint64_t epoch, int64_t first, int64_t count,
                        int64_t* out, void* stream);
int dsnt_example_scores(const float* pred, const float* target, const double* m, const double* b, const float* mask,
                        const double* head, const int64_t* idx, int64_t N, uint32_t stamp, unsigned long long* table,
                        float* score, int B, int J, void* stream);
#define DSNT_OCCLUDE_DOMAIN 0x4F43434Cu
#define DSNT_OCCLUDE_MAX_RECTS 8
#define DSNT_OCCLUDE_MAX_JOINTS 256
#define DSNT_OCCLUDE_FILL_VALUE 0
#define DSNT_OCCLUDE_FILL_NOISE 1
#define DSNT_OCCLUDE_FILL_PASTE 2
#define DSNT_OCCLUDE_CENTRE_UNIFORM 0
#define DSNT_OCCLUDE_CENTRE_JOINT 1
int dsnt_occlude(const float* in, float* out, int B, int S, int K, int side_min, int side_max, uint32_t p24, int fill,
                 int centre, const float* fill_value, const float* mean, const float* stdv, const float* coords,
                 const float* mask, int J, int32_t* rects, int32_t* donor, uint8_t* occluded, int draw, uint64_t seed,
                 uint64_t step, uint32_t draw_offset, void* stream);
int dsnt_crop_affine(const uint8_t* pool, int64_t pool_bytes, const int64_t* offset, const int32_t* hw, int64_t N,
                     const int64_t* idx, const double* matrix, int B, int R, uint8_t* out, uint8_t* valid, void* stream);
int dsnt_pool_normalize(const float* x, int N, int C, int H, int W, int S, const float* mean, const float* stdv,
                        float* out, void* stream);

#define DSNT_RENDER_CANVAS_BLACK 0
#define DSNT_RENDER_CANVAS_F32 1
#define DSNT_RENDER_CANVAS_U8 2
#define DSNT_RENDER_MAX_JOINTS 64
#define DSNT_RENDER_MAX_BONES 32
#define DSNT_RENDER_MAX_SIDE 16384
int dsnt_render_pose(const void* canvas, int canvas_kind, const float* mean, const float* stdv, int B, int H, int W, int J,
                     const float* heatmaps, int h, int w, const float* peak, int64_t peak_stride, const float* heat_rgb,
                     float heat_alpha, const float* coords, const float* mask, int pixel_coords,
                     const int32_t* bone_joints, const float* bone_rgb, int nbones, float width, float joint_radius,
                     uint8_t* out, void* stream);

#ifdef __cplusplus
}
#endif
#endif
```

Baseline: 2965 images/sec.

## Fold BatchNorm backward apply into f32 k-split dgrad kernel operand load

Adds an APPLY variant of the f32 k-split dgrad kernel that applies the pending BatchNorm backward transform (and optionally its finalize prologue) to the incoming gradient while loading it. The workgroup that owns the centre filter tap writes the materialized gradient out for wgrad. This removes the separate bn_act_bwd_apply pass and its extra read and write of the activation-sized gradient for eligible convolutions. In exchange, the kernel loads an extra operand (y) per fragment, does more ALU work per MFMA, and pipelines only two fragments deep instead of three. It also redoes the apply arithmetic in every tap and N-tile workgroup.

```diff
diff --git a/dsnt-pose2d_amd/csrc/api.cpp b/dsnt-pose2d_amd/csrc/api.cpp
--- a/dsnt-pose2d_amd/csrc/api.cpp
+++ b/dsnt-pose2d_amd/csrc/api.cpp
@@ -31,7 +31,7 @@
     return c;
 }
 
-extern "C" int dsnt_version(void) { return 132; }
+extern "C" int dsnt_version(void) { return 133; }
 extern "C" const char* dsnt_last_error(void) { return g_err; }
 
 #include <vector>
diff --git a/dsnt-pose2d_amd/csrc/bn.hip b/dsnt-pose2d_amd/csrc/bn.hip
--- a/dsnt-pose2d_amd/csrc/bn.hip
+++ b/dsnt-pose2d_amd/csrc/bn.hip
@@ -364,22 +364,6 @@
     DSNT_CHECK_LAUNCH("dsnt_relu_bwd");
 }
 
-struct BnApplyVec { float4 sc, sh, mu, is, c0, c1; };
-__device__ __forceinline__ float4 bn_apply_one(const float4 g, const float4 xv, const BnApplyVec& v, int relu) {
-    float4 dz = g;
-    if (relu) {
-        if (fmaf(xv.x, v.sc.x, v.sh.x) <= 0.f) dz.x = 0.f;
-        if (fmaf(xv.y, v.sc.y, v.sh.y) <= 0.f) dz.y = 0.f;
-        if (fmaf(xv.z, v.sc.z, v.sh.z) <= 0.f) dz.z = 0.f;
-        if (fmaf(xv.w, v.sc.w, v.sh.w) <= 0.f) dz.w = 0.f;
-    }
-    float4 o;
-    o.x = v.sc.x * (dz.x - v.c0.x - (xv.x - v.mu.x) * v.is.x * v.c1.x);
-    o.y = v.sc.y * (dz.y - v.c0.y - (xv.y - v.mu.y) * v.is.y * v.c1.y);
-    o.z = v.sc.z * (dz.z - v.c0.z - (xv.z - v.mu.z) * v.is.z * v.c1.z);
-    o.w = v.sc.w * (dz.w - v.c0.w - (xv.w - v.mu.w) * v.is.w * v.c1.w);
-    return o;
-}
 struct BnApplyP {
     const float4* da; const float4* x; const float4* scale; const float4* shift; const float4* mean; const float4* invstd;
     const float4* coef; int relu; float4* dx; const float4* base; long n4; int C4; unsigned* amax; BnBwdProP pro;
@@ -476,15 +460,6 @@
     return bn_act_bwd_apply_impl(da, x, scale, shift, mean, invstd, coef, relu, dx, accumulate, M, C, nullptr, stream, nullptr, nullptr);
 }
 
-static int bn_bwd_pro_fill(BnBwdProP& q, const char* who, const float* partial, int ntiles, float* dgamma, float* dbeta,
-                           int accumulate_params, float* coef, int64_t M, int C) {
-    DSNT_REQUIRE(partial && ntiles > 0 && coef && C <= 256 && (long)ntiles * C <= 16384, DSNT_ERR_ARG,
-                 "%s: needs partial sums of at most 256 channels / 128 KB and a coef buffer", who);
-    q.partial = partial; q.tiles = ntiles; q.C = C; q.invM = 1.0 / (double)M;
-    q.dgamma = dgamma; q.dbeta = dbeta; q.accumulate = accumulate_params; q.coef = coef;
-    return DSNT_OK;
-}
-
 extern "C" int dsnt_bn_act_bwd_apply_pro(const float* da, const float* x, const float* scale, const float* shift,
                                          const float* mean, const float* invstd, const float* partial, int ntiles,
                                          float* dgamma, float* dbeta, int accumulate_params, float* coef, int relu,
diff --git a/dsnt-pose2d_amd/csrc/bn_pro.h b/dsnt-pose2d_amd/csrc/bn_pro.h
--- a/dsnt-pose2d_amd/csrc/bn_pro.h
+++ b/dsnt-pose2d_amd/csrc/bn_pro.h
@@ -108,6 +108,23 @@
     __builtin_amdgcn_fence(__ATOMIC_RELEASE, "workgroup");
 }
 
+struct BnApplyVec { float4 sc, sh, mu, is, c0, c1; };
+__device__ __forceinline__ float4 bn_apply_one(const float4 g, const float4 xv, const BnApplyVec& v, int relu) {
+    float4 dz = g;
+    if (relu) {
+        if (fmaf(xv.x, v.sc.x, v.sh.x) <= 0.f) dz.x = 0.f;
+        if (fmaf(xv.y, v.sc.y, v.sh.y) <= 0.f) dz.y = 0.f;
+        if (fmaf(xv.z, v.sc.z, v.sh.z) <= 0.f) dz.z = 0.f;
+        if (fmaf(xv.w, v.sc.w, v.sh.w) <= 0.f) dz.w = 0.f;
+    }
+    float4 o;
+    o.x = v.sc.x * (dz.x - v.c0.x - (xv.x - v.mu.x) * v.is.x * v.c1.x);
+    o.y = v.sc.y * (dz.y - v.c0.y - (xv.y - v.mu.y) * v.is.y * v.c1.y);
+    o.z = v.sc.z * (dz.z - v.c0.z - (xv.z - v.mu.z) * v.is.z * v.c1.z);
+    o.w = v.sc.w * (dz.w - v.c0.w - (xv.w - v.mu.w) * v.is.w * v.c1.w);
+    return o;
+}
+
 static inline int out_bounds_fill(OutBoundsP& out, const dsnt_out_bounds* in, const char* who) {
     static_assert(sizeof(OutBoundsP) == sizeof(dsnt_out_bounds), "dsnt_out_bounds layout");
     out.amax = in ? reinterpret_cast<unsigned*>(in->amax) : nullptr;
@@ -118,3 +135,12 @@
                  DSNT_ERR_ARG, "%s: dsnt_out_bounds.amax_bn needs 16-byte aligned amax_scale / amax_shift", who);
     return DSNT_OK;
 }
+
+static inline int bn_bwd_pro_fill(BnBwdProP& q, const char* who, const float* partial, int ntiles, float* dgamma, float* dbeta,
+                           int accumulate_params, float* coef, int64_t M, int C) {
+    DSNT_REQUIRE(partial && ntiles > 0 && coef && C <= 256 && (long)ntiles * C <= 16384, DSNT_ERR_ARG,
+                 "%s: needs partial sums of at most 256 channels / 128 KB and a coef buffer", who);
+    q.partial = partial; q.tiles = ntiles; q.C = C; q.invM = 1.0 / (double)M;
+    q.dgamma = dgamma; q.dbeta = dbeta; q.accumulate = accumulate_params; q.coef = coef;
+    return DSNT_OK;
+}
diff --git a/dsnt-pose2d_amd/csrc/conv_f32.hip b/dsnt-pose2d_amd/csrc/conv_f32.hip
--- a/dsnt-pose2d_amd/csrc/conv_f32.hip
+++ b/dsnt-pose2d_amd/csrc/conv_f32.hip
@@ -335,8 +335,14 @@
     return DSNT_OK;
 }
 
-template <bool PRO, int CW>
-__device__ __forceinline__ void conv_ksplit_body(const ConvP& p, float (*part)[32][33]) {
+struct KsApplyP {
+    BnBwdProP pro;
+    unsigned* amax;
+    int cr, cs;
+};
+template <bool PRO, int CW, bool APPLY = false>
+__device__ __forceinline__ void conv_ksplit_body(const ConvP& p, float (*part)[32][33], const KsApplyP& ka = KsApplyP()) {
+    static_assert(!(PRO && APPLY), "the APPLY form has no BatchNorm prologue on its operand");
     typedef unsigned u32x4 __attribute__((ext_vector_type(4)));
     constexpr int NL = CW / 8;
     const int nt32 = (p.Cout + 31) >> 5;
@@ -353,6 +359,17 @@
     float* const ssc = &part[0][0][0];
     if (PRO) {
         for (int c = tid; c < p.Cin; c += 512) { ssc[c] = p.in_scale[c]; ssc[p.Cin + c] = p.in_shift[c]; }
+        __syncthreads();
+    }
+    if (APPLY) {
+        if (ka.pro.partial) {
+            bn_pro_backward<256>(ka.pro, reinterpret_cast<double*>(&part[0][0][0]), tile == 0);
+            __syncthreads();
+        }
+        for (int c = tid; c < p.Cin; c += 512) {
+            ssc[c] = p.ap_scale[c]; ssc[p.Cin + c] = p.ap_mean[c]; ssc[2 * p.Cin + c] = p.ap_invstd[c];
+            ssc[3 * p.Cin + c] = p.ap_coef[c]; ssc[4 * p.Cin + c] = p.ap_coef[p.Cin + c];
+        }
         __syncthreads();
     }
     const int m = mtile * 32 + i;
@@ -369,10 +386,16 @@
         const_cast<float*>(p.x), 0, (int)((size_t)p.N * p.H * p.W * p.Cin * 4u), 0x00020000);
     const __amdgpu_buffer_rsrc_t wr = __builtin_amdgcn_make_buffer_rsrc(
         const_cast<float*>(p.w), 0, (int)((size_t)p.Cout * p.K * 4u), 0x00020000);
+    const __amdgpu_buffer_rsrc_t yr = __builtin_amdgcn_make_buffer_rsrc(
+        const_cast<float*>(APPLY ? p.ap_y : p.x), 0, (int)((size_t)p.N * p.H * p.W * p.Cin * 4u), 0x00020000);
+    const __amdgpu_buffer_rsrc_t dor = __builtin_amdgcn_make_buffer_rsrc(
+        APPLY ? p.ap_out : const_cast<float*>(p.x), 0, (int)((size_t)p.N * p.H * p.W * p.Cin * 4u), 0x00020000);
+    const bool writer = APPLY && ntile == 0;
+    float am = 0.f;
     const int nch = p.K / CW;
     const int c0 = wave * nch / 8, c1 = (wave + 1) * nch / 8;
     const float lo_valid = p.in_relu ? 0.f : -__builtin_inff();
-    struct Frag { u32x4 a[NL], b[NL]; bool ok; int cb; };
+    struct Frag { u32x4 a[NL], b[NL], y[APPLY ? NL : 1]; bool ok; int cb; unsigned aoff; bool own; };
     int pos = c0, pr, ps, pcb;
     {
         const int kb = c0 * CW, tap = kb / p.Cin;
@@ -387,6 +410,12 @@
         const int kb4 = ((pr * p.S + ps) * p.Cin + pcb) * 4;
 #pragma unroll
         for (int q = 0; q < NL; ++q) f.a[q] = __builtin_amdgcn_raw_buffer_load_b128(xr, aoff + 16u * q, 0, 0);
+        if (APPLY) {
+#pragma unroll
+            for (int q = 0; q < NL; ++q) f.y[q] = __builtin_amdgcn_raw_buffer_load_b128(yr, aoff + 16u * q, 0, 0);
+            f.aoff = aoff;
+            f.own = writer && pr == ka.cr && ps == ka.cs;
+        }
 #pragma unroll
         for (int q = 0; q < NL; ++q) f.b[q] = __builtin_amdgcn_raw_buffer_load_b128(wr, boff + 16u * q, kb4, 0);
         if (pos < c1 - 1) {
@@ -413,6 +442,25 @@
                 a.z = __builtin_amdgcn_fmed3f(fmaf(a.z, sc.z, sh.z), lo, hi);
                 a.w = __builtin_amdgcn_fmed3f(fmaf(a.w, sc.w, sh.w), lo, hi);
             }
+            if (APPLY) {
+                const int ch = f.cb + kl + 4 * q;
+                BnApplyVec v;
+                v.sc = *reinterpret_cast<const float4*>(ssc + ch);
+                v.mu = *reinterpret_cast<const float4*>(ssc + p.Cin + ch);
+                v.is = *reinterpret_cast<const float4*>(ssc + 2 * p.Cin + ch);
+                v.c0 = *reinterpret_cast<const float4*>(ssc + 3 * p.Cin + ch);
+                v.c1 = *reinterpret_cast<const float4*>(ssc + 4 * p.Cin + ch);
+                v.sh = v.sc;
+                a = bn_apply_one(a, make_float4(__uint_as_float(f.y[q].x), __uint_as_float(f.y[q].y), __uint_as_float(f.y[q].z),
+                                                __uint_as_float(f.y[q].w)), v, 0);
+                a.x = f.ok ? a.x : 0.f; a.y = f.ok ? a.y : 0.f; a.z = f.ok ? a.z : 0.f; a.w = f.ok ? a.w : 0.f;
+                if (f.own) {
+                    u32x4 o;
+                    o.x = __float_as_uint(a.x); o.y = __float_as_uint(a.y); o.z = __float_as_uint(a.z); o.w = __float_as_uint(a.w);
+                    __builtin_amdgcn_raw_buffer_store_b128(o, dor, f.ok ? f.aoff + 16u * q : OOB, 0, 0);
+                    am = fmaxf(fmaxf(fmaxf(fabsf(a.x), fabsf(a.y)), fmaxf(fabsf(a.z), fabsf(a.w))), am);
+                }
+            }
             acc = __builtin_amdgcn_mfma_f32_32x32x2f32(a.x, __uint_as_float(f.b[q].x), acc, 0, 0, 0);
             acc = __builtin_amdgcn_mfma_f32_32x32x2f32(a.y, __uint_as_float(f.b[q].y), acc, 0, 0, 0);
             acc = __builtin_amdgcn_mfma_f32_32x32x2f32(a.z, __uint_as_float(f.b[q].z), acc, 0, 0, 0);
@@ -436,7 +484,13 @@
             if (vn && mo < p.M && p.res1) r1v[j] = p.res1[(size_t)mo * p.Cout + n];
         }
     }
-    if (c0 < c1) {
+    if (APPLY && c0 < c1) {
+        Frag f0 = load_next(), f1;
+        for (int ch = c0;;) {
+            f1 = load_next(); mma(f0); if (++ch >= c1) break;
+            f0 = load_next(); mma(f1); if (++ch >= c1) break;
+        }
+    } else if (c0 < c1) {
         Frag f0 = load_next(), f1 = load_next(), f2;
         for (int ch = c0;;) {
             f2 = load_next(); mma(f0); if (++ch >= c1) break;
@@ -444,7 +498,8 @@
             f1 = load_next(); mma(f2); if (++ch >= c1) break;
         }
     }
-    if (PRO) __syncthreads();
+    if (PRO || APPLY) __syncthreads();
+    if (APPLY && ka.amax && writer) amax_commit(am, ka.amax);
 #pragma unroll
     for (int e = 0; e < 16; ++e) part[wave][(e & 3) + 8 * (e >> 2) + 4 * h][i] = acc[e];
     __syncthreads();
@@ -496,6 +551,11 @@
 __global__ __launch_bounds__(512) void conv_ksplit_kernel(ConvP p) {
     __shared__ __attribute__((aligned(16))) float part[8][32][33];
     conv_ksplit_body<PRO, CW>(p, part);
+}
+template <int CW>
+__global__ __launch_bounds__(512) void conv_ksplit_apply_kernel(ConvP p, KsApplyP q) {
+    __shared__ __attribute__((aligned(16))) float part[8][32][33];
+    conv_ksplit_body<false, CW, true>(p, part, q);
 }
 
 static long ksplit_rows() {
@@ -618,3 +678,52 @@
     DSNT_REQUIRE(pro, DSNT_ERR_ARG, "dsnt_conv_fwd_pro: null dsnt_bn_prologue");
     return conv_fwd_impl(x, w, bias, y, pro->scale, pro->shift, in_relu, res1, res2, stats_partial, g, nullptr, tail, stream, pro);
 }
+
+static bool dgrad_apply_tap(const dsnt_conv_geom* g, int& cr, int& cs) {
+    if (g->stride != 1 || g->dil <= 0 || g->H != g->Ho || g->W != g->Wo || g->pad % g->dil != 0) return false;
+    cr = cs = g->pad / g->dil;
+    return cr < g->R && cs < g->S;
+}
+
+extern "C" int dsnt_conv_dgrad_apply_ok(const dsnt_conv_geom* g) {
+    if (!g || g->N <= 0 || g->H <= 0 || g->W <= 0 || g->Ho <= 0 || g->Wo <= 0 || g->R <= 0 || g->S <= 0 || g->Cin <= 0 || g->Cout <= 0)
+        return 0;
+    if (g->Cin % 8 != 0 || g->Cin > 1024 || g->Cout % 4 != 0) return 0;
+    const long M = (long)g->N * g->Ho * g->Wo;
+    if (M > ksplit_rows()) return 0;
+    if ((size_t)g->N * g->H * g->W * g->Cin * 4u >= (1ull << 31) || (size_t)g->Cout * g->R * g->S * g->Cin * 4u >= (1ull << 31)) return 0;
+    int cr, cs;
+    return dgrad_apply_tap(g, cr, cs) ? 1 : 0;
+}
+
+extern "C" int dsnt_conv_dgrad_apply(const float* dz, const dsnt_bn_bwd_apply* ap, float* dy_out, float* dy_amax,
+                                     const float* partial, int ntiles, float* dgamma, float* dbeta, int accumulate_params,
+                                     const float* wd, float* dx_dz, float* stats_partial, const dsnt_conv_geom* g,
+                                     const dsnt_bn_bwd_epilogue* bnb, void* stream) {
+    const char* who = "dsnt_conv_dgrad_apply";
+    ConvP p;
+    if (int e = conv_fill(p, who, dz, wd, false, 0, nullptr, dx_dz, nullptr, nullptr, 0, nullptr, nullptr, stats_partial, g, bnb, nullptr))
+        return e;
+    DSNT_REQUIRE(dsnt_conv_dgrad_apply_ok(g), DSNT_ERR_SHAPE,
+                 "%s: geometry not supported (stride 1, output as large as the input, a filter tap on the output pixel, "
+                 "Cin %% 8 == 0 and <= 1024, at most %ld rows)", who, ksplit_rows());
+    DSNT_REQUIRE(bnb && ap && ap->y && ap->scale && ap->mean && ap->invstd && ap->coef && dy_out, DSNT_ERR_ARG,
+                 "%s: needs a complete dsnt_bn_bwd_apply, dy_out and the BatchNorm-backward epilogue", who);
+    DSNT_REQUIRE(dsnt_aligned16(ap->y) && dsnt_aligned16(dy_out) && dy_out != dz && dy_out != ap->y && dy_out != dx_dz, DSNT_ERR_ALIGN,
+                 "%s: 16-byte alignment; dy_out must not alias dz or y (other workgroups read them again)", who);
+    KsApplyP q;
+    memset(&q, 0, sizeof(q));
+    if (partial) {
+        if (int e = bn_bwd_pro_fill(q.pro, who, partial, ntiles, dgamma, dbeta, accumulate_params, const_cast<float*>(ap->coef), p.M, p.Cin))
+            return e;
+    }
+    q.amax = reinterpret_cast<unsigned*>(dy_amax);
+    dgrad_apply_tap(g, q.cr, q.cs);
+    p.ap_y = ap->y; p.ap_scale = ap->scale; p.ap_mean = ap->mean; p.ap_invstd = ap->invstd; p.ap_coef = ap->coef; p.ap_out = dy_out;
+    p.mtiles = (p.M + 31) / 32; p.ntiles = (p.Cout + 31) / 32;
+    const int grid = p.mtiles * p.ntiles;
+    hipStream_t st = (hipStream_t)stream;
+    if (p.Cin % KS_CW == 0) DSNT_LAUNCH((conv_ksplit_apply_kernel<KS_CW>), dim3(grid), dim3(512), 0, st, p, q);
+    else DSNT_LAUNCH((conv_ksplit_apply_kernel<8>), dim3(grid), dim3(512), 0, st, p, q);
+    DSNT_CHECK_LAUNCH("dsnt_conv_dgrad_apply");
+}
diff --git a/dsnt-pose2d_amd/dsnt/_lib.py b/dsnt-pose2d_amd/dsnt/_lib.py
--- a/dsnt-pose2d_amd/dsnt/_lib.py
+++ b/dsnt-pose2d_amd/dsnt/_lib.py
@@ -104,6 +104,7 @@
     'dsnt_conv1x1_bwd_f16x3': [BP, P, AP, P, L, P, P, P, P, P, P, P, I, GP, P],
     'dsnt_conv1x1_fwd_ds_f16x3': [P, P, P, P, L, P, P, P, P, P, P, P, P, P, I, P, GP, GP, TP, P],
     'dsnt_conv_dgrad_f16x3_stream_apply': [P, AP, P, P, L, P, P, P, P, I, GP, BP, TP, P],
+    'dsnt_conv_dgrad_apply': [P, AP, P, P, P, I, P, P, I, P, P, P, GP, BP, P],
     'dsnt_wgrad_reduce_all': [P, I, I, P],
     'dsnt_conv_wgrad_group': [P, I, I, P],
     'dsnt_bn_stats': [P, P, L, I, P],
@@ -197,6 +198,7 @@
     'dsnt_conv_dgrad_strided_ok': (I, [GP]),
     'dsnt_conv_dgrad_strided_tiles': (I, [GP]),
     'dsnt_conv_fwd_pro_ok': (I, [GP, I, I]),
+    'dsnt_conv_dgrad_apply_ok': (I, [GP]),
     'dsnt_conv_wgrad_f16x3_splits': (I, [GP, I]),
     'dsnt_conv_wgrad_f16x3_ws_floats': (L, [GP, I]),
     'dsnt_conv_wgrad_ws_floats': (L, [GP]),
diff --git a/dsnt-pose2d_amd/dsnt/convop.py b/dsnt-pose2d_amd/dsnt/convop.py
--- a/dsnt-pose2d_amd/dsnt/convop.py
+++ b/dsnt-pose2d_amd/dsnt/convop.py
@@ -68,7 +68,7 @@
 
 class ConvOp:
     __slots__ = ('tape', 'src', 'x', 'y', 'p', 'g', 'res1', 'res2', 'name', 'normed', 'sc', 'sh', 'relu', 'need_input_grad', 'bucket',
-                 'x_amax', 'use6', 'use16', 'slot', 'slot_k', 'fuse1', 'fold3_ok', 'gd')
+                 'x_amax', 'use6', 'use16', 'slot', 'slot_k', 'fuse1', 'fold3_ok', 'foldk_ok', 'gd')
 
     def __init__(self, tape, src, p, res1, res2, name, need_input_grad):
         from .engine import Normed
@@ -81,7 +81,7 @@
         self.bucket = tape.cur_bucket
         self.y = None
         self.x_amax, self.use6, self.use16 = None, False, False
-        self.slot, self.slot_k, self.fuse1, self.fold3_ok, self.gd = None, None, False, False, None
+        self.slot, self.slot_k, self.fuse1, self.fold3_ok, self.foldk_ok, self.gd = None, None, False, False, False, None
 
     def operand_bound(self):
         bd = self.tape.bounds
@@ -198,7 +198,11 @@
             self.gd = ConvGeom(x.N, g.Ho, g.Wo, p.Cout, x.H, x.W, p.Cin, p.R, p.S, 1, p.dil * (p.R - 1) - p.pad, p.dil)
         self.fold3_ok = bool(t.fold3 and one_pass and plain and t.training and p.R == 3 and p.S == 3 and self.gd is not None and
                              self.use16 and y.M >= t.fold3_rows and use6(t, self.gd) and stream_ok(t, p, self.gd, None))
-        y.fold_ok = bool(self.fuse1 and plain) or self.fold3_ok
+        self.foldk_ok = bool(t.foldk and plain and t.training and self.need_input_grad and self.gd is not None and
+                             not self.fuse1 and not self.fold3_ok and not use6(t, self.gd) and
+                             t.lib.dsnt_conv_fwd_bm(C.byref(self.gd)) == 32 and t.lib.dsnt_conv_dgrad_apply_ok(C.byref(self.gd)))
+        y.fold_ok = bool(self.fuse1 and plain) or self.fold3_ok or self.foldk_ok
+        y.foldk = self.foldk_ok
 
     def backward(self):
         t, y = self.tape, self.y
@@ -206,7 +210,9 @@
         fused = self.fuse1 and t.bounds.dgrad_planes16 is not None
         fold3 = bool(self.fold3_ok and ap is not None and gy is None and t.bounds.dgrad_planes16 is not None and
                      self.need_input_grad and ap.bound is not None)
-        if ap is not None and (not fused or gy is not None) and not fold3:
+        foldk = bool(self.foldk_ok and ap is not None and ap.bound is None and gy is None and
+                     (self.x.foldk or not t.fold_ok(self.src)))
+        if ap is not None and (not fused or gy is not None) and not fold3 and not foldk:
             t.materialize_apply(y)
             ap, gy = None, y.grad
         assert gy is not None or ap is not None, 'no gradient reached conv output ' + self.name
@@ -218,6 +224,11 @@
         elif fold3:
             gy = y._grad = t.empty(y.N, y.H, y.W, y.C)
             y.grad_amax, y.pending_apply = ap.bound, None
+            self.dgrad(gy, ap)
+            wl, defer_res = self.wgrad(gy)
+        elif foldk:
+            gy = y._grad = t.empty(y.N, y.H, y.W, y.C)
+            y.grad_amax, y.pending_apply = (t.bounds.amax_slot() if t.use_f16x3 else None), None
             self.dgrad(gy, ap)
             wl, defer_res = self.wgrad(gy)
         else:
@@ -252,7 +263,7 @@
             grad = dict(g=dy, g_bound=gb)
         if self.normed:
             ab = bd.f16_bn_bound_bwd(src)
-            fold = t.fold_ok(src)
+            fold = t.fold_ok(src) and not x.foldk
             dz = self.dz_buffer(fold)
             dz_amax = bd.amax_slot() if fold else None
             part = t.scratch('bnpart', nsp * 2 * x.C).view(-1)
@@ -374,15 +385,26 @@
             self.dgrad_launch(d, buf, base if base is not None else (buf if acc else None), tail=tl)
             return
         fold = not d.native and t.fold_ok(src)
+        foldk = fold and x.foldk
         dz = self.dz_buffer(fold)
         tiles = t.lib.dsnt_conv_dgrad_strided_tiles(C.byref(self.g)) if d.native else stats_tiles(t, d.gd, d.d6)
-        part = t.scratch('bnpart', tiles * 2 * x.C).view(-1)
+        part = t.empty(tiles * 2 * x.C) if foldk else t.scratch('bnpart', tiles * 2 * x.C).view(-1)
         bnb = bn_epilogue(x, src)
         tl, dz_amax = None, None
-        if fold:
+        if fold and not foldk:
             dz_amax = t.bounds.amax_slot()
             tl = tail_at(dz_amax)
-        if ap is not None:
+        if ap is not None and ap.bound is None:
+            assert not (d.native or d.d6) and tl is None
+            name, bn = 'dsnt_conv_dgrad_apply', ap.n.bn
+            aps, _ = bn_apply(y, ap)
+            if ap.part is not None:
+                (pp, ptiles), pg, pb, acc_p = ap.part, bn.ggamma, bn.gbeta, t.bn_param_acc(bn)
+            else:
+                pp, ptiles, pg, pb, acc_p = None, 0, None, None, 0
+            t.b(name, ap.dz, aps, gy, y.grad_amax, pp, ptiles, pg, pb, acc_p, d.wd, dz, part, d.gd, bnb)
+            t.bwd.count(name, 4 * y.buf.numel())
+        elif ap is not None:
             assert d.d16 and d.d_stream and not d.native
             name = 'dsnt_conv_dgrad_f16x3_stream_apply'
             aps, applied = bn_apply(y, ap)
@@ -391,7 +413,7 @@
             self.use(e, 'dgrad', w=d.wd, w_bound=d.wbd, g_bound=ap.bound, g_apply=applied)
         else:
             self.dgrad_launch(d, dz, None, part, bnb, tl)
-        t._norm_backward(src, dz, reduced=(part, tiles), dz_amax=dz_amax)
+        t._norm_backward(src, dz, reduced=(part, tiles), dz_amax=dz_amax, foldk=foldk)
 
     def residual_grads(self, gy, wl, defer_res):
         t, y = self.tape, self.y
diff --git a/dsnt-pose2d_amd/dsnt/engine.py b/dsnt-pose2d_amd/dsnt/engine.py
--- a/dsnt-pose2d_amd/dsnt/engine.py
+++ b/dsnt-pose2d_amd/dsnt/engine.py
@@ -13,7 +13,7 @@
 
 
 class Act:
-    __slots__ = ('buf', 'N', 'H', 'W', 'C', '_grad', 'stats', 'name', 'grad_amax', 'amax_tail', 'fold_ok',
+    __slots__ = ('buf', 'N', 'H', 'W', 'C', '_grad', 'stats', 'name', 'grad_amax', 'amax_tail', 'fold_ok', 'foldk',
                  'pending_apply', 'uses', 'gives_away', 'is_branch', 'grad_shared', 'pending_add', 'base', 'base_amax')
 
     def __init__(self, buf, name=''):
@@ -25,6 +25,7 @@
         self.amax_tail = None
         self.grad_amax = None
         self.fold_ok = False
+        self.foldk = False
         self.pending_apply = None
         self.uses = 0
         self.gives_away = False
@@ -81,10 +82,10 @@
 
 
 class PendingApply:
-    __slots__ = ('dz', 'n', 'coef', 'bound', 'dz_amax')
-
-    def __init__(self, dz, n, coef, bound, dz_amax):
-        self.dz, self.n, self.coef, self.bound, self.dz_amax = dz, n, coef, bound, dz_amax
+    __slots__ = ('dz', 'n', 'coef', 'bound', 'dz_amax', 'part')
+
+    def __init__(self, dz, n, coef, bound, dz_amax, part=None):
+        self.dz, self.n, self.coef, self.bound, self.dz_amax, self.part = dz, n, coef, bound, dz_amax, part
 
 
 class Tape:
@@ -127,6 +128,7 @@
         self.fwd1 = 'fwd1' not in off
         self.fold3 = 'fold3' not in off
         self.fold3_rows = int(os.environ.get('DSNT_X_FOLD3_ROWS', '16384'))
+        self.foldk = 'foldk' not in off
         self.stem4 = 'stem4' not in off
         self.ds_fuse = 'dsfuse' not in off
         self.ds_fuse_rows = int(os.environ.get('DSNT_X_DS_FUSE_ROWS', '65536'))
@@ -359,16 +361,26 @@
 
     def fold_ok(self, n):
         x = n.x
-        return bool(self.bwd1 and x.fold_ok and x.grad is None and x.pending_apply is None)
+        return bool((self.bwd1 or x.foldk) and x.fold_ok and x.grad is None and x.pending_apply is None)
+
+    def bn_param_acc(self, bn):
+        acc_p = 1 if bn.uses > 0 else 0
+        bn.uses += 1
+        return acc_p
 
     def materialize_apply(self, x):
         ap, x.pending_apply = x.pending_apply, None
         n = ap.n
         buf, acc = self.grad_target(x, amax=True)
+        if ap.part is not None:
+            part, tiles = ap.part
+            self.b('dsnt_bn_act_bwd_apply_pro', ap.dz, x.buf, n.scale, n.shift, n.mean, n.invstd, part, tiles, n.bn.ggamma,
+                   n.bn.gbeta, self.bn_param_acc(n.bn), ap.coef, 0, buf, acc, x.M, n.bn.C, x.grad_amax)
+            return
         self.b_amax('dsnt_bn_act_bwd_apply', ap.dz, x.buf, n.scale, n.shift, n.mean, n.invstd, ap.coef, 0,
                     buf, acc, x.M, n.bn.C, amax=x.grad_amax)
 
-    def _norm_backward(self, n, da, reduced=None, finalised=False, dz_amax=None):
+    def _norm_backward(self, n, da, reduced=None, finalised=False, dz_amax=None, foldk=False):
         x, bn = n.x, n.bn
         coef = self.scratch('bncoef', 2 * bn.C)
         relu = 1 if n.relu else 0
@@ -380,6 +392,15 @@
             part = self.scratch('bnpart', tiles * 2 * bn.C).view(-1)
             self.b('dsnt_bn_act_bwd_reduce', da, x.buf, n.scale, n.shift, n.mean, n.invstd, relu, part,
                    x.M, bn.C)
+        if foldk:
+            assert reduced is not None and not finalised and x.grad is None and dz_amax is None and self.training
+            coef = self.empty(2 * bn.C)
+            if self.finalize_in_consumer(bn, tiles):
+                x.pending_apply = PendingApply(da, n, coef, None, None, part=(part, tiles))
+            else:
+                self.b('dsnt_bn_bwd_finalize', part, tiles, x.M, bn.C, bn.ggamma, bn.gbeta, self.bn_param_acc(bn), coef)
+                x.pending_apply = PendingApply(da, n, coef, None, None)
+            return
         if dz_amax is not None:
             assert reduced is not None and not finalised and x.grad is None
             acc_p = 1 if bn.uses > 0 else 0
@@ -439,7 +460,7 @@
         c.forward_ds(cd, want_stats)
         cd.plan_backward()
         c.plan_backward()
-        y.fold_ok = False
+        y.fold_ok = y.foldk = False
         self.on_backward(lambda: c.backward_ds(cd))
         return y
 
diff --git a/include/dsnt_hip.h b/include/dsnt_hip.h
--- a/include/dsnt_hip.h
+++ b/include/dsnt_hip.h
@@ -225,6 +225,11 @@
                                        const float* a_bound, float* dx_dz, float* stats_partial, int flags,
                                        const dsnt_conv_geom* g, const dsnt_bn_bwd_epilogue* bnb,
                                        const dsnt_out_bounds* tail, void* stream);
+int dsnt_conv_dgrad_apply_ok(const dsnt_conv_geom* g);
+int dsnt_conv_dgrad_apply(const float* dz, const dsnt_bn_bwd_apply* ap, float* dy_out, float* dy_amax,
+                          const float* partial, int ntiles, float* dgamma, float* dbeta, int accumulate_params,
+                          const float* wd, float* dx_dz, float* stats_partial, const dsnt_conv_geom* g,
+                          const dsnt_bn_bwd_epilogue* bnb, void* stream);
 
 int dsnt_encode_heatmaps(const float* target, float* out, int64_t rows, int h, int w, float sigma, void* stream);
 int dsnt_heatmap_mse_fwd(const float* hm, const float* target, float* per_row, int64_t rows, int h, int w,
```

Result: no change. 2975 images/sec (median of 3 runs) (+0.3%).
